# Mephisto405/WCMC

Measured on AMD Instinct MI355X. Metric: 128x128 MC patches/sec (train step), KPCN-Manifold, higher is better.
Workload: dtype bf16x321h

## Files before the change

### include/wcmc_hip.h

```cpp
#ifndef WCMC_HIP_H
#define WCMC_HIP_H

#include <stddef.h>
#include <stdint.h>

#ifdef __cplusplus
extern "C" {
#endif

#define WCMC_ABI_VERSION 2

enum wcmc_status {
  WCMC_OK = 0,
  WCMC_ERR_BAD_ARG = -1,
  WCMC_ERR_ALIGNMENT = -2,
  WCMC_ERR_WORKSPACE = -3,
  WCMC_ERR_LAUNCH = -4
};

enum wcmc_act { WCMC_ACT_LINEAR = 0, WCMC_ACT_RELU = 1, WCMC_ACT_LEAKY_RELU = 2 };

int wcmc_abi_version(void);
const char* wcmc_last_error(void);

int wcmc_to_nhwc(const float* src, int64_t ssn, int64_t ssc, int64_t ssh, int64_t ssw,
                 float* dst, int64_t dsn, int64_t dsh, int64_t dsw,
                 int N, int C, int H, int W, void* stream);
int wcmc_from_nhwc(const float* src, int64_t ssn, int64_t ssh, int64_t ssw,
                   float* dst, int64_t dsn, int64_t dsc, int64_t dsh, int64_t dsw,
                   int N, int C, int H, int W, void* stream);

size_t wcmc_conv2d_packed_elems(int rows, int kchan, int ks);
int wcmc_conv2d_pack_weight(const float* w_oihw, float* wp, int Cout, int Cin, int ks, int mode,
                            void* stream);

int wcmc_conv2d_igemm(const float* x, int64_t xsn, int64_t xsh, int64_t xsw,
                      int N, int H, int W, int Cin,
                      const float* wp, const float* bias,
                      float* y, int64_t ysn, int64_t ysh, int64_t ysw, int Cout,
                      int ks, int pad, int act, float slope,
                      const float* gate, int64_t gsn, int64_t gsh, int64_t gsw,
                      int gate_act, float gate_slope, void* stream);

size_t wcmc_conv2d_wgrad_workspace_bytes(int N, int Ho, int Wo, int Cout, int Cin, int ks);
int wcmc_conv2d_wgrad(const float* x, int64_t xsn, int64_t xsh, int64_t xsw,
                      int N, int H, int W, int Cin,
                      const float* dy, int64_t dsn, int64_t dsh, int64_t dsw, int Cout,
                      int ks, int pad, float* dw_oihw, float* db,
                      void* workspace, size_t workspace_bytes, void* stream);

int wcmc_split_from_nchw(const float* src, int64_t ssn, int64_t ssc, int64_t ssh, int64_t ssw, void* out_split, int N,
                         int C, int H, int W, void* stream);

size_t wcmc_split_elems(int N, int H, int W, int C);
int wcmc_split_bf16(const float* x, int64_t xsn, int64_t xsh, int64_t xsw, void* out_split,
                    int N, int H, int W, int C, void* stream);
int wcmc_split_gated_bf16(const float* dy, int64_t dsn, int64_t dsh, int64_t dsw, const float* post, int64_t psn,
                          int64_t psh, int64_t psw, int act, float slope, void* out_split, int N, int H, int W, int C,
                          void* stream);
int wcmc_cat_broadcast_split(const float* flat, int64_t fsn, int64_t fsh, int64_t fsw,
                             const float* prop, int64_t psn, int64_t psh, int64_t psw,
                             void* out_split, int B, int S, int H, int W, int C1, int C2, void* stream);
int wcmc_cat_upsample_split(const float* deep, int64_t dsn, int64_t dsh, int64_t dsw, const float* skip, int64_t ssn,
                            int64_t ssh, int64_t ssw, void* out_split, int N, int H, int W, int C1, int C2,
                            void* stream);

int wcmc_add_broadcast_split(const float* g, int64_t gsn, int64_t gsh, int64_t gsw,
                             const float* gm, int64_t msn, int64_t msh, int64_t msw, float scale,
                             void* out_split, int B, int S, int H, int W, int C, void* stream);
int wcmc_split_dy_colsum_bf16(const float* dy, int64_t dsn, int64_t dsh, int64_t dsw,
                              const float* post, int64_t psn, int64_t psh, int64_t psw, int act, float slope,
                              const float* gm, int64_t msn, int64_t msh, int64_t msw, int S, float scale,
                              void* out_split, float* colsum_partial, int N, int H, int W, int C, void* stream);
size_t wcmc_conv2d_packed_elems_bf16x3(int rows, int kchan, int ks, int mode);
int wcmc_conv2d_pack_weight_bf16x3(const float* w_oihw, void* wp, int Cout, int Cin, int ks, int mode,
                                   void* stream);
int wcmc_conv2d_pack_chain_bf16x3(int n_entries, const float* const* w, void* const* wp, const int* Cout,
                                  const int* Cin, const int* mode, int ks, void* stream);
int wcmc_conv2d_igemm_bf16x3(const void* x_split, int N, int H, int W, int Cin,
                             const void* wp, const float* bias,
                             float* y, int64_t ysn, int64_t ysh, int64_t ysw, void* y_split, int Cout,
                             int ks, int pad, int act, float slope,
                             const void* gate_split, int gate_act, float gate_slope,
                             float* colsum_partial, const void* gate_mask, void* mask_out, int terms, void* stream);
int wcmc_conv2d_out_f16_supported(int Cin, int Cout, int ks);
size_t wcmc_split_to_f16_elems(int N, int H, int W, int C);
int wcmc_split_to_f16(const void* x_split, int N, int H, int W, int C, void* out_f16, void* stream);
int wcmc_conv2d_out_f16(const void* x_f16, int N, int H, int W, int Cin, const void* wp_f16, const float* bias, float* y,
                        int64_t ysn, int64_t ysh, int64_t ysw, int Cout, int ks, int pad, void* stream);
int wcmc_conv1x1_pair_supported(int Cin, int Cout1, int Cout2);
int wcmc_conv1x1_pair_bf16x3(const void* x_split, int N, int H, int W, int Cin, const void* wp1, const float* bias1,
                             int Cout1, int act1, float slope1, void* y1_split, void* mask1, const void* gate_mask1,
                             int gate_act1, float gate_slope1, float* colsum1, const void* wp2, const float* bias2,
                             int Cout2, int act2, float slope2, float* y2, int64_t y2sn, int64_t y2sh, int64_t y2sw,
                             void* stream);
int wcmc_embed3_supported(int Cin, int C1, int C2, int C3);
size_t wcmc_embed3_bwd_workspace_bytes(void);
int wcmc_embed3_fwd(const void* x_split, int64_t M, int Cin, const void* wp0, const float* b0, const void* wp1,
                    const float* b1, const void* wp2, const float* b2, float* y, void* stream);
int wcmc_embed3_mean_supported(int S, int64_t HW);
int wcmc_embed3_mean_fwd(const void* x_split, int64_t M, int Cin, const void* wp0, const float* b0, const void* wp1,
                         const float* b1, const void* wp2, const float* b2, float* y, float* y_mean, int S, int64_t HW,
                         void* stream);
int wcmc_embed3_bwd(const void* x_split, int64_t M, int Cin, const void* wp0, const float* b0, const void* wp1,
                    const float* b1, const void* wt1, const void* wt2, const float* gy, int gy_pixel_stride,
                    const float* gm, int gm_pixel_stride, int S, int64_t HW, float gm_scale, float* dw0, float* db0,
                    float* dw1, float* db1, float* dw2, float* db2, void* workspace, size_t workspace_bytes, void* stream);
int wcmc_embed3_nchw_supported(int Cin, int64_t N, int64_t H, int64_t W, int64_t sn, int64_t sc, int64_t sh, int64_t sw);
int wcmc_embed3_mean_fwd_nchw(const float* x, int64_t x_sample_stride, int64_t x_channel_stride, int64_t M, int Cin,
                              const void* wp0, const float* b0, const void* wp1, const float* b1, const void* wp2,
                              const float* b2, float* y, float* y_mean, int S, int64_t HW, void* stream);
int wcmc_embed3_bwd_nchw(const float* x, int64_t x_sample_stride, int64_t x_channel_stride, int64_t M, int Cin, const void* wp0,
                         const float* b0, const void* wp1, const float* b1, const void* wt1, const void* wt2, const float* gy,
                         int gy_pixel_stride, const float* gm, int gm_pixel_stride, int S, int64_t HW, float gm_scale, float* dw0,
                         float* db0, float* dw1, float* db1, float* dw2, float* db2, void* workspace, size_t workspace_bytes,
                         void* stream);
int wcmc_final2_supported(int C1, int C2, int Chid, int outc, int64_t HW);
size_t wcmc_final2_bwd_workspace_bytes(void);
int wcmc_final2_fwd(const float* y, int y_pixel_stride, const float* prop, int prop_pixel_stride, int B, int S, int64_t HW,
                    const void* wp0, const float* b0, const void* wp1, const float* b1, int outc, float* out, void* stream);
int wcmc_final2_bwd(const float* y, int y_pixel_stride, const float* prop, int prop_pixel_stride, int B, int S, int64_t HW,
                    const void* wp0, const float* b0, const void* wp1, const float* b1, int outc, const void* wt0,
                    const void* wt1, const float* gout, float* dy, float* dprop, float* dw0, float* db0, float* dw1,
                    float* db1, void* workspace, size_t workspace_bytes, void* stream);
int wcmc_final2_fwd_save(const float* y, int y_pixel_stride, const float* prop, int prop_pixel_stride, int B, int S, int64_t HW,
                         const void* wp0, const float* b0, const void* wp1, const float* b1, int outc, float* out, void* h_hi,
                         void* stream);
int wcmc_final2_bwd_saved(const float* y, int y_pixel_stride, const float* prop, int prop_pixel_stride, int B, int S, int64_t HW,
                          const void* wp0, const float* b0, const void* wp1, const float* b1, int outc, const void* wt0,
                          const void* wt1, const float* gout, const float* out, const void* h_hi, float* dy, float* dprop,
                          float* dw0, float* db0, float* dw1, float* db1, void* workspace, size_t workspace_bytes, void* stream);
size_t wcmc_conv2d_igemm_colsum_elems(int N, int Ho, int Wo, int Cout);
int wcmc_colsum_finish(const float* partial, int N, int Ho, int Wo, int Cout, float* db, void* stream);
int wcmc_conv2d_launch_plan_bf16x3(int N, int H, int W, int Cin, int Cout, int ks, int pad, int terms, int split_out,
                                   int64_t ysn, int64_t ysh, int64_t ysw, int gate_tensor, int out_f16,
                                   char* cls, char* kernel, size_t len);
int wcmc_conv2d_wgrad_launch_plan_bf16x3(int N, int H, int W, int Cin, int Cout, int ks, int pad, int terms,
                                         char* cls, char* kernel, size_t len);
size_t wcmc_conv2d_wgrad_bf16x3_workspace_bytes(int N, int Ho, int Wo, int Cout, int Cin, int ks);
int wcmc_conv2d_wgrad_reduce_multi(int n, void* const* workspace, float* const* dw, float* const* db,
                                   const float* const* dy_colsum_partial, const int* N, const int* Ho, const int* Wo,
                                   const int* Cout, const int* Cin, const int* ks, int terms, void* stream);
int wcmc_conv2d_wgrad_bf16x3(const void* x_split, int N, int H, int W, int Cin,
                             const void* dy_split, int Cout, int ks, int pad, float* dw, float* db,
                             void* workspace, size_t workspace_bytes, int phase, const float* dy_colsum_partial,
                             int terms, void* stream);

int wcmc_act_backward(const float* dy, int64_t dsn, int64_t dsh, int64_t dsw,
                      const float* y, int64_t ysn, int64_t ysh, int64_t ysw,
                      float* dx, int64_t xsn, int64_t xsh, int64_t xsw,
                      int N, int H, int W, int C, int act, float slope, void* stream);

int wcmc_kernel_apply_fwd(const float* logits, int64_t lsn, int64_t lsh, int64_t lsw,
                          const float* data, int64_t dsn, int64_t dsc, int64_t dsh, int64_t dsw,
                          float* out, int64_t osn, int64_t osc, int64_t osh, int64_t osw,
                          float* lse, int N, int C, int h, int w, int k, void* stream);
int wcmc_kernel_apply_bwd(const float* logits, int64_t lsn, int64_t lsh, int64_t lsw,
                          const float* data, int64_t dsn, int64_t dsc, int64_t dsh, int64_t dsw,
                          const float* out, int64_t osn, int64_t osc, int64_t osh, int64_t osw,
                          const float* grad_out, int64_t gsn, int64_t gsc, int64_t gsh, int64_t gsw,
                          const float* lse,
                          float* d_logits, int64_t qsn, int64_t qsh, int64_t qsw,
                          float* d_data, int N, int C, int h, int w, int k, void* stream);

enum wcmc_splat_mode { WCMC_SPLAT_SOFTMAX = 0, WCMC_SPLAT_SHIFT = 1 };
size_t wcmc_kernel_splat_fwd_workspace_bytes(int N, int C, int h, int w, int k2);
int wcmc_kernel_splat_fwd(const float* logits, int64_t lsn, int64_t lsh, int64_t lsw,
                          const float* data, int64_t dsn, int64_t dsc, int64_t dsh, int64_t dsw,
                          float* sum_r, float* sum_w, float* lse, int mode, const float* shift,
                          int accumulate, void* workspace, size_t workspace_bytes,
                          int N, int C, int h, int w, int k2, void* stream);
int wcmc_kernel_splat_bwd(const float* logits, int64_t lsn, int64_t lsh, int64_t lsw,
                          const float* data, int64_t dsn, int64_t dsc, int64_t dsh, int64_t dsw,
                          const float* g_r, int64_t gsn, int64_t gsc, int64_t gsh, int64_t gsw,
                          const float* g_w, int64_t wsn, int64_t wsh, int64_t wsw,
                          const float* lse, int mode, const float* shift,
                          float* d_logits, int64_t qsn, int64_t qsh, int64_t qsw,
                          float* d_data, int N, int C, int h, int w, int k2, void* stream);
size_t wcmc_logit_max_workspace_bytes(int N);
int wcmc_logit_max(const float* logits, int64_t lsn, int64_t lsh, int64_t lsw, float* out,
                   void* workspace, size_t workspace_bytes, int N, int h, int w, int k2, void* stream);

int wcmc_recombine_fwd(const float* albedo, int64_t asn, int64_t asc, int64_t ash, int64_t asw,
                       const float* r_diffuse, int64_t dsn, int64_t dsc, int64_t dsh, int64_t dsw,
                       const float* r_specular, int64_t ssn, int64_t ssc, int64_t ssh, int64_t ssw,
                       float* out, int N, int C, int H, int W, void* stream);
int wcmc_recombine_bwd(const float* grad_out,
                       const float* albedo, int64_t asn, int64_t asc, int64_t ash, int64_t asw,
                       const float* r_specular, int64_t ssn, int64_t ssc, int64_t ssh, int64_t ssw,
                       float* d_diffuse, float* d_specular, int N, int C, int H, int W, void* stream);

size_t wcmc_image_loss_workspace_bytes(void);
int wcmc_image_loss_fwd(const float* x, int64_t xsn, int64_t xsc, int64_t xsh, int64_t xsw,
                        const float* ref, int64_t rsn, int64_t rsc, int64_t rsh, int64_t rsw, float eps,
                        float* l1_mean, float* relative_mse, void* workspace, size_t workspace_bytes,
                        int N, int C, int H, int W, void* stream);
int wcmc_l1_mean_bwd(const float* x, int64_t xsn, int64_t xsc, int64_t xsh, int64_t xsw,
                     const float* ref, int64_t rsn, int64_t rsc, int64_t rsh, int64_t rsw,
                     const float* grad_loss, float* dx, int N, int C, int H, int W, void* stream);

int wcmc_maxpool2_fwd(const float* x, int64_t xsn, int64_t xsh, int64_t xsw,
                      float* y, int64_t ysn, int64_t ysh, int64_t ysw,
                      int N, int H, int W, int C, void* stream);
int wcmc_maxpool2_bwd_add(const float* x, int64_t xsn, int64_t xsh, int64_t xsw, const float* dy, int64_t dsn, int64_t dsh,
                          int64_t dsw, const float* add, int64_t asn, int64_t ash, int64_t asw, float* dx, int64_t gsn,
                          int64_t gsh, int64_t gsw, int N, int H, int W, int C, void* stream);
int wcmc_maxpool2_bwd(const float* x, int64_t xsn, int64_t xsh, int64_t xsw,
                      const float* dy, int64_t dsn, int64_t dsh, int64_t dsw,
                      float* dx, int64_t gsn, int64_t gsh, int64_t gsw,
                      int N, int H, int W, int C, void* stream);
int wcmc_upsample2_fwd(const float* x, int64_t xsn, int64_t xsh, int64_t xsw,
                       float* y, int64_t ysn, int64_t ysh, int64_t ysw,
                       int N, int H, int W, int C, void* stream);
int wcmc_upsample2_bwd(const float* dy, int64_t dsn, int64_t dsh, int64_t dsw,
                       float* dx, int64_t xsn, int64_t xsh, int64_t xsw,
                       int N, int H, int W, int C, void* stream);

int wcmc_spp_reduce(const float* x, int64_t xsn, int64_t xsh, int64_t xsw,
                    float* y, int64_t ysn, int64_t ysh, int64_t ysw,
                    int B, int S, int H, int W, int C, float scale, void* stream);
int wcmc_spp_broadcast(const float* x, int64_t xsn, int64_t xsh, int64_t xsw,
                       float* y, int64_t ysn, int64_t ysh, int64_t ysw,
                       int B, int S, int H, int W, int C, float scale, int accumulate,
                       void* stream);

int wcmc_sample_cat_fwd(const float* feat, int64_t fsb, int64_t fss, int64_t fsc, int64_t fsh, int64_t fsw,
                        const float* p, int64_t psb, int64_t pss, int64_t psc, int64_t psh, int64_t psw, float* out,
                        int B, int S, int C, int Cp, int H, int W, void* stream);

int wcmc_pbuffer_cat_fwd(const float* base, int64_t bsn, int64_t bsc, int64_t bsh, int64_t bsw,
                         const float* p, int64_t psb, int64_t pss, int64_t psc, int64_t psh,
                         int64_t psw,
                         float* out, int64_t osn, int64_t osh, int64_t osw,
                         int B, int S, int Cb, int Cp, int H, int W, void* stream);
int wcmc_pbuffer_cat_bwd(const float* g, int64_t gsn, int64_t gsh, int64_t gsw,
                         float* dp, int64_t psb, int64_t pss, int64_t psc, int64_t psh,
                         int64_t psw,
                         int B, int S, int Cb, int Cp, int H, int W, void* stream);

size_t wcmc_feature_mse_workspace_bytes(int B, int S, int C, int h, int w);
int wcmc_feature_mse_fwd(const float* p, int64_t psb, int64_t pss, int64_t psc, int64_t psh,
                         int64_t psw,
                         const float* ref, int64_t rsb, int64_t rsc, int64_t rsh, int64_t rsw,
                         const int64_t* idx_patch, const int64_t* idx_batch,
                         float* loss, void* workspace, size_t workspace_bytes,
                         int B, int S, int C, int h, int w, void* stream);
int wcmc_feature_mse_bwd(const float* p, int64_t psb, int64_t pss, int64_t psc, int64_t psh,
                         int64_t psw,
                         const int64_t* idx_patch, const int64_t* idx_batch,
                         const float* grad_scale, float* dp,
                         void* workspace, size_t workspace_bytes,
                         int B, int S, int C, int h, int w, void* stream);

int wcmc_grs_fwd(const float* p, int64_t psb, int64_t pss, int64_t psc, int64_t psh, int64_t psw,
                 const float* ref, int64_t rsb, int64_t rsc, int64_t rsh, int64_t rsw,
                 const int64_t* idx_patch, const int64_t* idx_batch, float alpha,
                 float* loss, void* workspace, size_t workspace_bytes,
                 int B, int S, int C, int h, int w, void* stream);
int wcmc_grs_bwd(const float* p, int64_t psb, int64_t pss, int64_t psc, int64_t psh, int64_t psw,
                 const int64_t* idx_patch, const int64_t* idx_batch,
                 const float* grad_scale, float* dp,
                 void* workspace, size_t workspace_bytes,
                 int B, int S, int C, int h, int w, void* stream);

int wcmc_random_permutation(int64_t* out, int64_t n, uint64_t seed, void* stream);
uint64_t wcmc_permutation_key(uint64_t seed, uint64_t counter, int slot);
int wcmc_random_permutation_dev(int64_t* out, int64_t n, const uint64_t* state, int slot, void* stream);
int wcmc_step_counter_advance(uint64_t* state, void* stream);

int wcmc_image_loss2_fwd(int kind, const float* x, int64_t xsn, int64_t xsc, int64_t xsh, int64_t xsw, const float* ref,
                         int64_t rsn, int64_t rsc, int64_t rsh, int64_t rsw, float eps, float* loss, void* workspace,
                         size_t workspace_bytes, int N, int C, int H, int W, void* stream);
int wcmc_image_loss2_bwd(int kind, const float* x, int64_t xsn, int64_t xsc, int64_t xsh, int64_t xsw, const float* ref,
                         int64_t rsn, int64_t rsc, int64_t rsh, int64_t rsw, float eps, const float* grad_loss, float* dx,
                         int N, int C, int H, int W, void* stream);
size_t wcmc_grad_norm_clip_workspace_bytes(int n_tensors, const int64_t* numel);
int wcmc_grad_norm_clip(int n_tensors, float* const* grads, const int64_t* numel, float max_norm, float* norm_and_coef,
                        void* workspace, size_t workspace_bytes, void* stream);

int wcmc_weight_norm_fwd(int n_layers, const float* const* v, const float* const* g, float* const* w,
                         float* const* norm, const int* rows, const int* row_len, void* stream);
int wcmc_weight_norm_bwd(int n_layers, const float* const* dw, const float* const* v, const float* const* g,
                         const float* const* norm, float* const* dv, float* const* dg, const int* rows,
                         const int* row_len, void* stream);

int wcmc_clip_adam(float* param, float* grad, float* exp_avg, float* exp_avg_sq, int64_t n,
                   float clip, double lr, double beta1, double beta2, double eps, int step,
                   float grad_scale, const float* guard, void* stream);
void wcmc_clip_adam_hyper(double lr, double beta1, double beta2, double eps, int step, float* out7);
int wcmc_clip_adam_dev(float* param, float* grad, float* exp_avg, float* exp_avg_sq, int64_t n, float clip,
                       float grad_scale, const float* hyper7, const float* guard, void* stream);
int wcmc_step_guard(const float* const* losses, int n, float* ok, float* sums, float* flags, void* stream);
int wcmc_step_guard_local(const float* const* losses, int n, const float* ok, float* flags, float* flag_slot, void* stream);
int wcmc_step_guard_global(const float* const* losses, int n, const float* flag_slot, float* ok, float* sums, float* flags, void* stream);

int wcmc_preprocess_llpm(const float* raw, int64_t nsamples , int C, int max_depth, float* out,
                         void* stream);
size_t wcmc_preprocess_kpcn_workspace_bytes(int h, int w);
int wcmc_preprocess_kpcn(const float* raw, int h, int w, int s, int C, int max_depth, float* out,
                         void* workspace, size_t workspace_bytes, void* stream);
int wcmc_gradients(const float* buf, int h, int w, int c, float* out, void* stream);
int wcmc_preprocess_kpcn_begin(void* workspace, size_t workspace_bytes, int h, int w, void* stream);
int wcmc_preprocess_kpcn_rows(const float* raw_band, int h, int w, int row0, int rows, int s, int C, int max_depth, float* out,
                              void* workspace, size_t workspace_bytes, void* stream);
int wcmc_preprocess_kpcn_end(float* out, void* workspace, size_t workspace_bytes, int h, int w, int s, void* stream);

int wcmc_assemble_kpcn_patches(const float* kpcn, const float* llpm, const float* gt, const int* origins, int B, int H,
                               int W, int S, int P, float* diffuse_in, float* specular_in, float* diffuse_buffer,
                               float* specular_buffer, float* albedo, float* paths, float* target_diffuse,
                               float* target_specular, float* target_total, void* stream);

int wcmc_reflect_index(int i, int n);
size_t wcmc_importance_map_workspace_bytes(int H, int W, int C);
int wcmc_importance_map(const float* img, int H, int W, int C, float* out, void* workspace, size_t workspace_bytes,
                        void* stream);
size_t wcmc_sampling_prob_workspace_bytes(int H, int W, int patch);
int wcmc_sampling_prob(const float* raw, const float* gt, int H, int W, int S, int C, int max_depth, int patch, float* out,
                       void* workspace, size_t workspace_bytes, void* stream);
int wcmc_sanitize(float* x, int64_t n, void* stream);

int wcmc_preprocess_sbmc(const float* raw, int64_t nsamples , int C, int max_depth, float* out_s, float* out_p,
                         int tiled, void* stream);
int wcmc_assemble_sample_patches(const float* sbmc_s, const float* sbmc_p, const float* llpm, const float* gt,
                                 const int* origins, int B, int H, int W, int S, int P, int use_g_buf, int use_sbmc_buf,
                                 float* radiance, float* features, float* paths, float* target_image, void* stream);

size_t wcmc_preprocess_kpcn_prefix_workspace_bytes(int h, int w, int n_counts);
int wcmc_preprocess_kpcn_prefix(const float* raw, int h, int w, int S, int C, int max_depth, int s_lo, int s_hi, float* out,
                                void* workspace, size_t workspace_bytes, void* stream);
int wcmc_assemble_kpcn_patches_prefix(const float* kpcn, const float* llpm, const float* gt, const int* origins, int B, int H,
                                      int W, int S_total, int s, int P, float* diffuse_in, float* specular_in,
                                      float* diffuse_buffer, float* specular_buffer, float* albedo, float* paths,
                                      float* target_diffuse, float* target_specular, float* target_total, void* stream);
int wcmc_assemble_sample_patches_prefix(const float* sbmc_s, const float* sbmc_p, const float* llpm, const float* gt,
                                        const int* origins, int B, int H, int W, int S_total, int s, int P, int use_g_buf,
                                        int use_sbmc_buf, float* radiance, float* features, float* paths, float* target_image,
                                        void* stream);

int wcmc_assemble_kpcn_patches_aug(const float* kpcn, const float* llpm, const float* gt, const int* origins, const int* transforms,
                                   int B, int H, int W, int S_total, int s, int P, float* diffuse_in, float* specular_in,
                                   float* diffuse_buffer, float* specular_buffer, float* albedo, float* paths,
                                   float* target_diffuse, float* target_specular, float* target_total, void* stream);
int wcmc_assemble_sample_patches_aug(const float* sbmc_s, const float* sbmc_p, const float* llpm, const float* gt,
                                     const int* origins, const int* transforms, int B, int H, int W, int S_total, int s, int P,
                                     int use_g_buf, int use_sbmc_buf, float* radiance, float* features, float* paths,
                                     float* target_image, void* stream);

size_t wcmc_image_eval_workspace_bytes(int H, int W);
int wcmc_image_eval(const float* out, int64_t osh, int64_t osw, int64_t osc, const float* ipt, int64_t ish, int64_t isw,
                    int64_t isc, const float* tgt, int64_t tsh, int64_t tsw, int64_t tsc, const float* has_hit, int64_t hsh,
                    int64_t hsw, int64_t hsc, int H, int W, double eps, double* result, void* workspace,
                    size_t workspace_bytes, void* stream);
int wcmc_stitch_tiles(const float* rad, int64_t rsb, int64_t rsc, int64_t rsh, int64_t rsw, int ho, int wo,
                      const float* pbuf_a, const float* pbuf_b, int S, int C, int P, const int* coords, int B, int H, int W,
                      float* out_rad, float* out_pbuf_a, float* out_pbuf_b, void* stream);

int wcmc_assemble_kpcn_tiles(const float* kpcn, const float* llpm, const int* origins, int B, int H, int W, int S, int P, int pad,
                             float* diffuse_in, float* specular_in, float* diffuse_buffer, float* specular_buffer, float* albedo,
                             float* paths, void* stream);
int wcmc_finish_frame(const float* out_rad, const float* kpcn, const float* llpm, int H, int W, int S, float* out, float* ipt,
                      float* has_hit, unsigned char* preview_out, unsigned char* preview_ipt, void* stream);

int wcmc_assemble_sample_tiles(const float* sbmc_s, const float* sbmc_p, const float* llpm, const int* origins, int B, int H, int W,
                               int S, int P, int pad, int use_g_buf, int use_sbmc_buf, float* radiance, float* features,
                               float* paths, void* stream);
int wcmc_finish_sample_frame(const float* out_rad, const float* sbmc_s, const float* llpm, int H, int W, int S, float* out,
                             float* ipt, float* has_hit, unsigned char* preview_out, unsigned char* preview_ipt, void* stream);

size_t wcmc_pbuffer_filter_workspace_bytes(int S, int C, int H, int W);
int wcmc_pbuffer_filter(const float* image, int64_t ish, int64_t isw, int64_t isc,
                        const float* p_buffer, int64_t pss, int64_t psc, int64_t psh, int64_t psw,
                        const void* mask, int mask_bytes, float* out, float* wsum, void* workspace, size_t workspace_bytes,
                        int H, int W, int S, int C, int Cr, int R, int f, float bandwidth, float eps, int passes, void* stream);

#ifdef __cplusplus
}
#endif
#endif
```

### wcmc_amd/_lib.py

```python
import ctypes
import os

_HERE = os.path.dirname(os.path.abspath(__file__))
LIB_PATH = os.path.join(_HERE, "libwcmc_hip.so")
if os.environ.get("WCMC_DEBUG_LIB") == "1":
    LIB_PATH = os.path.join(_HERE, "libwcmc_hip_debug.so")
if os.environ.get("WCMC_LIB_AB"):
    LIB_PATH = os.path.join(_HERE, os.path.basename(os.environ["WCMC_LIB_AB"]))

_c = ctypes
P, I, L, F, D, Z = _c.c_void_p, _c.c_int, _c.c_int64, _c.c_float, _c.c_double, _c.c_size_t

SIGNATURES = {
    "wcmc_abi_version": (I, []),
    "wcmc_last_error": (_c.c_char_p, []),
    "wcmc_to_nhwc": (I, [P, L, L, L, L, P, L, L, L, I, I, I, I, P]),
    "wcmc_from_nhwc": (I, [P, L, L, L, P, L, L, L, L, I, I, I, I, P]),
    "wcmc_conv2d_packed_elems": (Z, [I, I, I]),
    "wcmc_conv2d_pack_weight": (I, [P, P, I, I, I, I, P]),
    "wcmc_conv2d_igemm": (I, [P, L, L, L, I, I, I, I, P, P, P, L, L, L, I, I, I, I, F,
                              P, L, L, L, I, F, P]),
    "wcmc_conv2d_wgrad_workspace_bytes": (Z, [I, I, I, I, I, I]),
    "wcmc_conv2d_wgrad": (I, [P, L, L, L, I, I, I, I, P, L, L, L, I, I, I, P, P, P, Z, P]),
    "wcmc_split_elems": (Z, [I, I, I, I]),
    "wcmc_split_bf16": (I, [P, L, L, L, P, I, I, I, I, P]),
    "wcmc_split_from_nchw": (I, [P, L, L, L, L, P, I, I, I, I, P]),
    "wcmc_split_gated_bf16": (I, [P, L, L, L, P, L, L, L, I, F, P, I, I, I, I, P]),
    "wcmc_cat_broadcast_split": (I, [P, L, L, L, P, L, L, L, P, I, I, I, I, I, I, P]),
    "wcmc_cat_upsample_split": (I, [P, L, L, L, P, L, L, L, P, I, I, I, I, I, P]),
    "wcmc_add_broadcast_split": (I, [P, L, L, L, P, L, L, L, F, P, I, I, I, I, I, P]),
    "wcmc_split_dy_colsum_bf16": (I, [P, L, L, L, P, L, L, L, I, F, P, L, L, L, I, F, P, P, I, I, I, I, P]),
    "wcmc_conv2d_packed_elems_bf16x3": (Z, [I, I, I, I]),
    "wcmc_conv2d_pack_weight_bf16x3": (I, [P, P, I, I, I, I, P]),
    "wcmc_conv2d_pack_chain_bf16x3": (I, [I, P, P, P, P, P, I, P]),
    "wcmc_conv2d_igemm_bf16x3": (I, [P, I, I, I, I, P, P, P, L, L, L, P, I, I, I, I, F, P, I, F, P, P, P, I, P]),
    "wcmc_conv2d_out_f16_supported": (I, [I, I, I]),
    "wcmc_split_to_f16_elems": (Z, [I, I, I, I]),
    "wcmc_split_to_f16": (I, [P, I, I, I, I, P, P]),
    "wcmc_conv2d_out_f16": (I, [P, I, I, I, I, P, P, P, L, L, L, I, I, I, P]),
    "wcmc_conv1x1_pair_supported": (I, [I, I, I]),
    "wcmc_conv1x1_pair_bf16x3": (I, [P, I, I, I, I, P, P, I, I, F, P, P, P, I, F, P, P, P, I, I, F, P, L, L, L, P]),
    "wcmc_conv2d_igemm_colsum_elems": (Z, [I, I, I, I]),
    "wcmc_colsum_finish": (I, [P, I, I, I, I, P, P]),
    "wcmc_conv2d_launch_plan_bf16x3": (I, [I, I, I, I, I, I, I, I, I, L, L, L, I, I, _c.c_char_p, _c.c_char_p, Z]),
    "wcmc_conv2d_wgrad_launch_plan_bf16x3": (I, [I, I, I, I, I, I, I, I, _c.c_char_p, _c.c_char_p, Z]),
    "wcmc_conv2d_wgrad_bf16x3_workspace_bytes": (Z, [I, I, I, I, I, I]),
    "wcmc_conv2d_wgrad_reduce_multi": (I, [I, P, P, P, P, P, P, P, P, P, P, I, P]),
    "wcmc_conv2d_wgrad_bf16x3": (I, [P, I, I, I, I, P, I, I, I, P, P, P, Z, I, P, I, P]),
    "wcmc_act_backward": (I, [P, L, L, L, P, L, L, L, P, L, L, L, I, I, I, I, I, F, P]),
    "wcmc_kernel_apply_fwd": (I, [P, L, L, L, P, L, L, L, L, P, L, L, L, L, P, I, I, I, I, I, P]),
    "wcmc_kernel_apply_bwd": (I, [P, L, L, L, P, L, L, L, L, P, L, L, L, L, P, L, L, L, L, P,
                                  P, L, L, L, P, I, I, I, I, I, P]),
    "wcmc_kernel_splat_fwd_workspace_bytes": (Z, [I, I, I, I, I]),
    "wcmc_kernel_splat_fwd": (I, [P, L, L, L, P, L, L, L, L, P, P, P, I, P, I, P, Z, I, I, I, I, I, P]),
    "wcmc_kernel_splat_bwd": (I, [P, L, L, L, P, L, L, L, L, P, L, L, L, L, P, L, L, L, P, I, P,
                                  P, L, L, L, P, I, I, I, I, I, P]),
    "wcmc_logit_max_workspace_bytes": (Z, [I]),
    "wcmc_logit_max": (I, [P, L, L, L, P, P, Z, I, I, I, I, P]),
    "wcmc_recombine_fwd": (I, [P, L, L, L, L, P, L, L, L, L, P, L, L, L, L, P, I, I, I, I, P]),
    "wcmc_image_loss_workspace_bytes": (Z, []),
    "wcmc_image_loss_fwd": (I, [P, L, L, L, L, P, L, L, L, L, F, P, P, P, Z, I, I, I, I, P]),
    "wcmc_l1_mean_bwd": (I, [P, L, L, L, L, P, L, L, L, L, P, P, I, I, I, I, P]),
    "wcmc_recombine_bwd": (I, [P, P, L, L, L, L, P, L, L, L, L, P, P, I, I, I, I, P]),
    "wcmc_maxpool2_fwd": (I, [P, L, L, L, P, L, L, L, I, I, I, I, P]),
    "wcmc_maxpool2_bwd": (I, [P, L, L, L, P, L, L, L, P, L, L, L, I, I, I, I, P]),
    "wcmc_maxpool2_bwd_add": (I, [P, L, L, L, P, L, L, L, P, L, L, L, P, L, L, L, I, I, I, I, P]),
    "wcmc_upsample2_fwd": (I, [P, L, L, L, P, L, L, L, I, I, I, I, P]),
    "wcmc_upsample2_bwd": (I, [P, L, L, L, P, L, L, L, I, I, I, I, P]),
    "wcmc_sample_cat_fwd": (I, [P, L, L, L, L, L, P, L, L, L, L, L, P, I, I, I, I, I, I, P]),
    "wcmc_spp_reduce": (I, [P, L, L, L, P, L, L, L, I, I, I, I, I, F, P]),
    "wcmc_spp_broadcast": (I, [P, L, L, L, P, L, L, L, I, I, I, I, I, F, I, P]),
    "wcmc_pbuffer_cat_fwd": (I, [P, L, L, L, L, P, L, L, L, L, L, P, L, L, L, I, I, I, I, I, I, P]),
    "wcmc_pbuffer_cat_bwd": (I, [P, L, L, L, P, L, L, L, L, L, I, I, I, I, I, I, P]),
    "wcmc_feature_mse_workspace_bytes": (Z, [I, I, I, I, I]),
    "wcmc_feature_mse_fwd": (I, [P, L, L, L, L, L, P, L, L, L, L, P, P, P, P, Z, I, I, I, I, I, P]),
    "wcmc_feature_mse_bwd": (I, [P, L, L, L, L, L, P, P, P, P, P, Z, I, I, I, I, I, P]),
    "wcmc_grs_fwd": (I, [P, L, L, L, L, L, P, L, L, L, L, P, P, F, P, P, Z, I, I, I, I, I, P]),
    "wcmc_grs_bwd": (I, [P, L, L, L, L, L, P, P, P, P, P, Z, I, I, I, I, I, P]),
    "wcmc_random_permutation": (I, [P, L, ctypes.c_uint64, P]),
    "wcmc_permutation_key": (ctypes.c_uint64, [ctypes.c_uint64, ctypes.c_uint64, I]),
    "wcmc_random_permutation_dev": (I, [P, L, P, I, P]),
    "wcmc_step_counter_advance": (I, [P, P]),
    "wcmc_final2_supported": (I, [I, I, I, I, L]),
    "wcmc_final2_bwd_workspace_bytes": (Z, []),
    "wcmc_final2_fwd": (I, [P, I, P, I, I, I, L, P, P, P, P, I, P, P]),
    "wcmc_final2_bwd": (I, [P, I, P, I, I, I, L, P, P, P, P, I, P, P, P, P, P, P, P, P, P, P, Z, P]),
    "wcmc_final2_fwd_save": (I, [P, I, P, I, I, I, L, P, P, P, P, I, P, P, P]),
    "wcmc_final2_bwd_saved": (I, [P, I, P, I, I, I, L, P, P, P, P, I, P, P, P, P, P, P, P, P, P, P, P, P, Z, P]),
    "wcmc_embed3_supported": (I, [I, I, I, I]),
    "wcmc_embed3_bwd_workspace_bytes": (Z, []),
    "wcmc_embed3_fwd": (I, [P, L, I, P, P, P, P, P, P, P, P]),
    "wcmc_embed3_mean_supported": (I, [I, L]),
    "wcmc_embed3_mean_fwd": (I, [P, L, I, P, P, P, P, P, P, P, P, I, L, P]),
    "wcmc_embed3_bwd": (I, [P, L, I, P, P, P, P, P, P, P, I, P, I, I, L, F, P, P, P, P, P, P, P, Z, P]),
    "wcmc_embed3_nchw_supported": (I, [I, L, L, L, L, L, L, L]),
    "wcmc_embed3_mean_fwd_nchw": (I, [P, L, L, L, I, P, P, P, P, P, P, P, P, I, L, P]),
    "wcmc_embed3_bwd_nchw": (I, [P, L, L, L, I, P, P, P, P, P, P, P, I, P, I, I, L, F, P, P, P, P, P, P, P, Z, P]),
    "wcmc_image_loss2_fwd": (I, [I, P, L, L, L, L, P, L, L, L, L, F, P, P, Z, I, I, I, I, P]),
    "wcmc_image_loss2_bwd": (I, [I, P, L, L, L, L, P, L, L, L, L, F, P, P, I, I, I, I, P]),
    "wcmc_grad_norm_clip_workspace_bytes": (Z, [I, P]),
    "wcmc_grad_norm_clip": (I, [I, P, P, F, P, P, Z, P]),
    "wcmc_weight_norm_fwd": (I, [I, P, P, P, P, P, P, P]),
    "wcmc_weight_norm_bwd": (I, [I, P, P, P, P, P, P, P, P, P]),
    "wcmc_clip_adam": (I, [P, P, P, P, L, F, D, D, D, D, I, F, P, P]),
    "wcmc_clip_adam_hyper": (None, [D, D, D, D, I, P]),
    "wcmc_clip_adam_dev": (I, [P, P, P, P, L, F, F, P, P, P]),
    "wcmc_step_guard": (I, [P, I, P, P, P, P]),
    "wcmc_step_guard_local": (I, [P, I, P, P, P, P]),
    "wcmc_step_guard_global": (I, [P, I, P, P, P, P, P]),
    "wcmc_preprocess_llpm": (I, [P, L, I, I, P, P]),
    "wcmc_preprocess_kpcn_workspace_bytes": (Z, [I, I]),
    "wcmc_preprocess_kpcn": (I, [P, I, I, I, I, I, P, P, Z, P]),
    "wcmc_preprocess_kpcn_begin": (I, [P, Z, I, I, P]),
    "wcmc_preprocess_kpcn_rows": (I, [P, I, I, I, I, I, I, I, P, P, Z, P]),
    "wcmc_preprocess_kpcn_end": (I, [P, P, Z, I, I, I, P]),
    "wcmc_gradients": (I, [P, I, I, I, P, P]),
    "wcmc_assemble_kpcn_patches": (I, [P, P, P, P, I, I, I, I, I, P, P, P, P, P, P, P, P, P, P]),
    "wcmc_reflect_index": (I, [I, I]),
    "wcmc_importance_map_workspace_bytes": (Z, [I, I, I]),
    "wcmc_importance_map": (I, [P, I, I, I, P, P, Z, P]),
    "wcmc_sampling_prob_workspace_bytes": (Z, [I, I, I]),
    "wcmc_sampling_prob": (I, [P, P, I, I, I, I, I, I, P, P, Z, P]),
    "wcmc_sanitize": (I, [P, L, P]),
    "wcmc_preprocess_sbmc": (I, [P, L, I, I, P, P, I, P]),
    "wcmc_assemble_sample_patches": (I, [P, P, P, P, P, I, I, I, I, I, I, I, P, P, P, P, P]),
    "wcmc_preprocess_kpcn_prefix_workspace_bytes": (Z, [I, I, I]),
    "wcmc_preprocess_kpcn_prefix": (I, [P, I, I, I, I, I, I, I, P, P, Z, P]),
    "wcmc_assemble_kpcn_patches_prefix": (I, [P, P, P, P, I, I, I, I, I, I, P, P, P, P, P, P, P, P, P, P]),
    "wcmc_assemble_sample_patches_prefix": (I, [P, P, P, P, P, I, I, I, I, I, I, I, I, P, P, P, P, P]),
    "wcmc_assemble_kpcn_patches_aug": (I, [P, P, P, P, P, I, I, I, I, I, I, P, P, P, P, P, P, P, P, P, P]),
    "wcmc_assemble_sample_patches_aug": (I, [P, P, P, P, P, P, I, I, I, I, I, I, I, I, P, P, P, P, P]),
    "wcmc_image_eval_workspace_bytes": (Z, [I, I]),
    "wcmc_image_eval": (I, [P, L, L, L, P, L, L, L, P, L, L, L, P, L, L, L, I, I, D, P, P, Z, P]),
    "wcmc_stitch_tiles": (I, [P, L, L, L, L, I, I, P, P, I, I, I, P, I, I, I, P, P, P, P]),
    "wcmc_assemble_kpcn_tiles": (I, [P, P, P, I, I, I, I, I, I, P, P, P, P, P, P, P]),
    "wcmc_finish_frame": (I, [P, P, P, I, I, I, P, P, P, P, P, P]),
    "wcmc_assemble_sample_tiles": (I, [P, P, P, P, I, I, I, I, I, I, I, I, P, P, P, P]),
    "wcmc_finish_sample_frame": (I, [P, P, P, I, I, I, P, P, P, P, P, P]),
    "wcmc_pbuffer_filter_workspace_bytes": (Z, [I, I, I, I]),
    "wcmc_pbuffer_filter": (I, [P, L, L, L, P, L, L, L, L, P, I, P, P, P, Z, I, I, I, I, I, I, I, F, F, I, P]),
}

_lib = None


def lib():
    global _lib
    if _lib is None:
        if not os.path.isfile(LIB_PATH):
            raise RuntimeError(
                "wcmc_amd: %s is missing -- the HIP hot path has not been built "
                "(make -C wcmc_amd/csrc). There is no CPU fallback." % LIB_PATH)
        h = ctypes.CDLL(LIB_PATH)
        for name, (res, args) in SIGNATURES.items():
            fn = getattr(h, name)
            fn.restype, fn.argtypes = res, args
        if h.wcmc_abi_version() != 2:
            raise RuntimeError("wcmc_amd: ABI version mismatch in %s" % LIB_PATH)
        _lib = h
    return _lib


def check(rc, what=""):
    if rc != 0:
        msg = lib().wcmc_last_error().decode("utf-8", "replace")
        raise RuntimeError("wcmc_hip %s failed (%d): %s" % (what, rc, msg))
```

### wcmc_amd/csrc/bf16x3_common.h

```cpp
#pragma once
#include "common.h"

namespace wcmc {

typedef __bf16 bf16x8 __attribute__((ext_vector_type(8)));
typedef unsigned short u16;
typedef short s16x4 __attribute__((ext_vector_type(4)));

__device__ __forceinline__ u16 f2bf(float x) { return __builtin_bit_cast(u16, (__bf16)x); }
__device__ __forceinline__ float bf2f(u16 h) { return __builtin_bit_cast(float, (unsigned)h << 16); }
__device__ __forceinline__ void split1(float x, u16& hi, u16& lo) {
  hi = f2bf(x);
  lo = f2bf(x - bf2f(hi));
}

typedef _Float16 xf16x8 __attribute__((ext_vector_type(8)));

constexpr int XBM = 128;
constexpr int XKC = 32;
constexpr int XROW = 32;
constexpr unsigned XOOB = 0x80000000u;

typedef unsigned int u32x4 __attribute__((ext_vector_type(4)));
typedef unsigned u32x2 __attribute__((ext_vector_type(2)));

typedef short xs16x2 __attribute__((ext_vector_type(2)));
__device__ __forceinline__ unsigned positive_pair(unsigned w) {
  const xs16x2 z = {0, 0};
  const xs16x2 c = __builtin_elementwise_max(__builtin_bit_cast(xs16x2, w), z);
  return ((__builtin_bit_cast(unsigned, c) + 0x7fff7fffu) >> 15) & 0x00010001u;
}
__device__ __forceinline__ unsigned char positive_mask8(const u32x4 v) {
  const unsigned x = positive_pair(v[0]) | (positive_pair(v[1]) << 2) | (positive_pair(v[2]) << 4) | (positive_pair(v[3]) << 6);
  return (unsigned char)((x | (x >> 15)) & 0xffu);
}

typedef __bf16 xbf16x2 __attribute__((ext_vector_type(2)));
typedef float xf32x2 __attribute__((ext_vector_type(2)));
__device__ __forceinline__ void x_split2(float a, float b, unsigned& hi2, unsigned& lo2) {
  const xf32x2 v = {a, b};
  hi2 = __builtin_bit_cast(unsigned, __builtin_convertvector(v, xbf16x2));
  const xf32x2 back = {__builtin_bit_cast(float, hi2 << 16), __builtin_bit_cast(float, hi2 & 0xffff0000u)};
  lo2 = __builtin_bit_cast(unsigned, __builtin_convertvector(v - back, xbf16x2));
}
struct XAct { float ns; bool zero; };
__device__ __forceinline__ XAct x_act(int act, float slope) {
  return XAct{act == WCMC_ACT_LEAKY_RELU ? slope : 1.f, act == WCMC_ACT_RELU};
}
__device__ __forceinline__ float x_act_apply(float v, XAct a) { return v > 0.f ? v : (a.zero ? 0.f : v * a.ns); }

__device__ __forceinline__ void x_epi_quad(const f32x4 a4, const float (&b)[4], bool ok, XAct ak, int gkind, u32x2 g2, int co,
                                           float gate_off, float (&v)[4]) {
#pragma unroll
  for (int e = 0; e < 4; ++e) {
    const float t = a4[e] + b[e];
    const float neg = ak.zero ? 0.f : t * ak.ns;
    const float r = t > 0.f ? t : neg;
    v[e] = ok ? r : 0.f;
  }
  if (gkind == 1) {
    const unsigned g[4] = {g2.x << 16, g2.x & 0xffff0000u, g2.y << 16, g2.y & 0xffff0000u};
#pragma unroll
    for (int e = 0; e < 4; ++e) v[e] = __builtin_bit_cast(float, g[e]) > 0.f ? v[e] : v[e] * gate_off;
  } else if (gkind == 2) {
    const unsigned bits = g2.x >> (co & 7);
#pragma unroll
    for (int e = 0; e < 4; ++e) v[e] = ((bits >> e) & 1u) ? v[e] : v[e] * gate_off;
  }
}

struct XIgemmParams {
  const u16* x; int N, H, W, Cin, Cpi;
  const u16* wp; const float* bias;
  float* yf; int64_t ysn, ysh, ysw;
  u16* ys; int Cpo;
  int Ho, Wo, Cout;
  const u16* gate; int gate_act; float gate_slope;
  const unsigned char* gate_mask;
  unsigned char* mask_out;
  int ks, pad, act; float slope;
  int Kp, Kt, Np;
  int64_t M;
  unsigned x_bytes, wp_bytes;
  float* colsum;
  int G;
  int CS, nslabs, SPS, PXS, tilesX, tilesY;
  int CSl, SPSl;
  int rows16;
  int stripX, stripY;
  int ap;
  int wplanes;
  int f16;
  unsigned y_bytes, m_bytes;
  const u16* wp2; const float* bias2; float* y2; int64_t y2sn, y2sh, y2sw;
  int Cout2, act2, Kt2; float slope2; unsigned wp2_bytes, y2_bytes;
};

struct XWgradParams {
  const u16* x; int N, H, W, Cin, Cpi;
  const u16* dy; int Ho, Wo, Cout, Cpo;
  int ks, pad;
  float* slabs; int S; int64_t M, pix_per_split;
  int Np, Cq, coBlocks, ciBlocks;
  unsigned x_bytes, dy_bytes;
  int xps, yps;
};
struct XWRowsParams {
  const u16* x; int N, H, W, Cpi;
  const u16* dy; int Ho, Wo, Cpo;
  int pad;
  float* slabs; int S, rps, R;
  float* dbg;
  int prio;
  int Np, Cq, coBlocks, ciBlocks;
  unsigned x_bytes, dy_bytes;
  int xps, yps;
};
constexpr int xwr_stride(int ch) { return ((ch / 16) | 1) * 16; }
static size_t xwr_lds_bytes_rt(int ks, int tm, int nw, int pl = 2) {
  const int nvec = pl * 64 * (xwr_stride(tm * 16) / 8) + pl * (64 + ks - 1) * (xwr_stride(nw * 16) / 8);
  const int ni = (nvec + nw * 64 - 1) / (nw * 64);
  const size_t stage = (size_t)2 * ni * nw * 64 * 16, red = (size_t)tm * 16 * (nw * 16 + 4) * sizeof(float);
  return stage > red ? stage : red;
}

__device__ __forceinline__ void pw_barrier() {
  asm volatile("s_waitcnt lgkmcnt(0)" ::: "memory");
  __builtin_amdgcn_s_barrier();
  asm volatile("" ::: "memory");
}

int x_env_on(const char* name);

struct XIgemmPlan { int nt, padded, dbuf; };
struct XHaloPlan { int nt, th, nb, ap, tilesY; size_t lds; };
struct XHalo64Plan { int nt, nb, pt, pxst, ap, wp, f16;
                     int tilesX, tilesY, rows16, stripX, stripY; size_t lds; };
struct XHalo3Plan { int ap, spt; };
struct XPwPlan { int ntw, u; };
struct XWRowsPlan { int ks, tm, nw, pl, rows8, xe; };
XIgemmPlan x_plan_igemm(int nt, const XIgemmParams& p);
int launch_xigemm(const XIgemmPlan& g, const XIgemmParams& p, hipStream_t stream);
bool x_halo_is64(const XIgemmParams& p);
int x_plan_halo(int nt, const XIgemmParams& p, XHaloPlan* h);
int launch_xhalo(const XHaloPlan& h, const XIgemmParams& p, hipStream_t stream);
XHalo64Plan x_plan_halo64(int nt, const XIgemmParams& p);
int launch_xhalo64(const XHalo64Plan& h, const XIgemmParams& p, hipStream_t stream);
bool x_halo3_ok(const XIgemmParams& p);
XHalo3Plan x_plan_halo3(const XIgemmParams& p);
int launch_xhalo3(const XHalo3Plan& h, const XIgemmParams& p, hipStream_t stream);
bool x_plan_pw(const XIgemmParams& p, XPwPlan* w);
int launch_xpw(XIgemmParams& p, const XPwPlan& w, hipStream_t stream);
int launch_xpw_pair(int kind, const XIgemmParams& p, hipStream_t stream);
int launch_xwgrad(int tm, int planes, const XWgradParams& p, hipStream_t stream);
XWRowsPlan x_plan_wgrad_rows(int ks, int tm, int nw, int planes);
int launch_xwgrad_rows(const XWRowsPlan& r, const XWRowsParams& p, hipStream_t stream);

}
```

### wcmc_amd/csrc/bf16x3_halo64.hip

```cpp
#include "bf16x3_common.h"

namespace wcmc {

template <int NT, int NB, int PT = 4, int DBG = 0, int PXST = 0, int AP = 2, int WP = 2, int F16 = 0>
__global__ __launch_bounds__(256, 2) void conv_halo64_bf16x3_kernel(XIgemmParams p0) {
  static_assert(WP == 2 || AP == 1, "one weight plane only together with one pixel plane");
  static_assert(!F16 || (AP == 1 && WP == 1), "fp16 operands: one plane each");
  XIgemmParams p = p0;
  if (PXST) { p.PXS = PXST; p.ks = 5; }
  constexpr int BN = NT * 16, TH = 4 * PT, TW = 16, NTHR = 256, NWV = 4;
  constexpr int NG = (PT + 1) / 2;
  extern __shared__ __attribute__((aligned(16))) u16 smem16[];
  constexpr int B_LO = BN * XROW + 32, B_ELEMS = 2 * BN * XROW + 64;
  const int HWd = TW + p.ks - 1, HHt = TH + p.ks - 1, HP = HWd * HHt;
  char* const halo = reinterpret_cast<char*>(smem16);
  u16* const bsm = smem16 + ((HP * p.PXS + 127) & ~127) / 2;

  const int tid = threadIdx.x, lane = tid & 63, wave = __builtin_amdgcn_readfirstlane(tid >> 6);
  unsigned long long st_rt[7] = {0, 0, 0, 0, 0, 0, 0};
  auto rstamp = [&](int i) {
    if (DBG & 64) {
      unsigned long long t;
      __builtin_amdgcn_sched_barrier(0);
      asm volatile("s_memrealtime %0\n\ts_waitcnt lgkmcnt(0)" : "=s"(t)::"memory");
      __builtin_amdgcn_sched_barrier(0);
      st_rt[i] = t;
    }
  };
  rstamp(0);
  int tile;
  {
    const int nb = gridDim.x, q = nb >> 3, r = nb & 7, xcd = blockIdx.x & 7, k = blockIdx.x >> 3;
    tile = (xcd < r ? xcd * (q + 1) : r * (q + 1) + (xcd - r) * q) + k;
  }
  const int nmain = p.tilesX * p.tilesY;
  const int tpi = nmain + (PT == 4 ? p.stripX * p.stripY : 0);
  const int img = tile / tpi, trem0 = tile - img * tpi;
  const bool tr = PT == 4 && trem0 >= nmain;
  const int trem = tr ? trem0 - nmain : trem0;
  const int tcols = tr ? p.stripX : p.tilesX;
  const int trow = trem / tcols;
  const int ptc = tr ? 3 : (PT == 4 && trow >= p.rows16) ? 3 : PT;
  const int oy0 = tr ? trow * 16 : PT == 4 ? (trow < p.rows16 ? trow * 16 : p.rows16 * 16 + (trow - p.rows16) * 12) : trow * TH;
  const int ox0 = tr ? p.tilesX * TW + (trem - trow * tcols) * 12 : (trem - trow * tcols) * TW;
  const int n0 = blockIdx.y * BN;

  const __amdgpu_buffer_rsrc_t xr = __builtin_amdgcn_make_buffer_rsrc((void*)p.x, 0, (int)p.x_bytes, 0x00020000);
  const __amdgpu_buffer_rsrc_t wr = __builtin_amdgcn_make_buffer_rsrc((void*)p.wp, 0, (int)p.wp_bytes, 0x00020000);
  const int pixb = (F16 ? 2 : 4) * p.Cpi;

  const int VP = p.PXS / 16;
  const int hvecs = HWd * (4 * ptc + p.ks - 1) * VP;
  const float invVP = 1.0f / (float)VP, invHW = 1.0f / (float)HWd;
  constexpr int NHV = PXST ? (((TH + 4) * (TW + 4) * (PXST / 16) + 63) / 64 + NWV - 1) / NWV : 0;
  const int CSlh = p.CSl < 8 ? 8 : p.CSl;
  unsigned hoff[NHV ? NHV : 1], hoffl[NHV ? NHV : 1];
  if (PXST) {
#pragma unroll
    for (int kq = 0; kq < NHV; ++kq) {
      const int v = (wave + NWV * kq) * 64 + lane;
      hoff[kq] = XOOB; hoffl[kq] = XOOB;
      if (v < hvecs) {
        const int px = (int)(((float)v + 0.5f) * invVP), part = v - px * VP;
        const int hy = (int)(((float)px + 0.5f) * invHW), hx = px - hy * HWd;
        const int iy = oy0 - p.pad + (tr ? hx : hy), ix = ox0 - p.pad + (tr ? hy : hx);
        if ((unsigned)iy < (unsigned)p.H && (unsigned)ix < (unsigned)p.W) {
          const unsigned pbase = (unsigned)(((img * p.H + iy) * p.W + ix) * pixb);
          if (AP == 1) {
            if (part < p.CS / 8 && (p.nslabs - 2) * p.CS + part * 8 < p.Cpi) hoff[kq] = pbase + (unsigned)(part * 16);
            if (part < CSlh / 8 && (p.nslabs - 1) * p.CS + part * 8 < p.Cpi) hoffl[kq] = pbase + (unsigned)(part * 16);
          } else {
          {
            const int V = p.CS / 4, plane = part >= (V >> 1), vec = part - plane * (V >> 1);
            if (part < V && (p.nslabs - 2) * p.CS + vec * 8 < p.Cpi) hoff[kq] = pbase + (unsigned)(plane * 2 * p.Cpi + vec * 16);
          }
          {
            const int V = CSlh / 4, plane = part >= (V >> 1), vec = part - plane * (V >> 1);
            if (part < V && (p.nslabs - 1) * p.CS + vec * 8 < p.Cpi) hoffl[kq] = pbase + (unsigned)(plane * 2 * p.Cpi + vec * 16);
          }
          }
        }
      }
    }
  }
  auto dma_halo = [&](int slab) {
    if (PXST) {
      const unsigned so = (unsigned)(slab * p.CS * 2);
      const bool lastslab = slab == p.nslabs - 1;
#pragma unroll
      for (int kq = 0; kq < NHV; ++kq) {
        const int ii = wave + NWV * kq;
        if (ii * 64 < hvecs) {
          const unsigned off = (lastslab ? hoffl[kq] : hoff[kq]) + so;
          if (ii * 64 + lane < hvecs)
            __builtin_amdgcn_raw_ptr_buffer_load_lds(xr, (__attribute__((address_space(3))) void*)(halo + ii * 1024), 16, off, 0, 0, 0);
        }
      }
      return;
    }
    const int V = (slab == p.nslabs - 1 ? CSlh : p.CS) / (AP == 1 ? 8 : 4);
    for (int ii = wave; ii * 64 < hvecs; ii += NWV) {
      const int v = ii * 64 + lane;
      if (v < hvecs) {
        const int px = (int)(((float)v + 0.5f) * invVP), part = v - px * VP;
        const int hy = (int)(((float)px + 0.5f) * invHW), hx = px - hy * HWd;
        const int iy = oy0 - p.pad + (tr ? hx : hy), ix = ox0 - p.pad + (tr ? hy : hx);
        const int plane = AP == 1 ? 0 : part >= (V >> 1), vec = part - plane * (V >> 1);
        const int ch = slab * p.CS + vec * 8;
        unsigned off = XOOB;
        if (part < V && (unsigned)iy < (unsigned)p.H && (unsigned)ix < (unsigned)p.W && ch < p.Cpi)
          off = (unsigned)(((img * p.H + iy) * p.W + ix) * pixb + plane * 2 * p.Cpi + ch * 2);
        __builtin_amdgcn_raw_ptr_buffer_load_lds(xr, (__attribute__((address_space(3))) void*)(halo + ii * 1024), 16, off, 0, 0, 0);
      }
    }
  };

  const int nstages = p.Kt / XKC;
  constexpr int NGMAX = (NT + NWV - 1) / NWV;
  const int ngroups = wave < NT ? (NT - wave + NWV - 1) / NWV : 0;
  unsigned dbase[NGMAX], dbase2[NGMAX];
#pragma unroll
  for (int q = 0; q < NGMAX; ++q) {
    const int drow = 16 * (wave + q * NWV) + (lane >> 2);
    const int dvq = (lane & 3) ^ ((drow >> 1) & 3);
    dbase[q] = (q < ngroups && n0 + drow < p.Np) ? (unsigned)(((n0 + drow) * 2 * p.Kt + dvq * 8) * 2) : XOOB;
    dbase2[q] = dbase[q] >= XOOB ? XOOB : dbase[q] + (unsigned)(p.Kt * 2);
  }
  auto dma_b = [&](int g, int buf) {
    const unsigned sg = g < nstages ? (unsigned)(g * XKC * 2) : 0x40000000u;
#pragma unroll
    for (int q = 0; q < NGMAX; ++q) {
      if (q < ngroups) {
        const unsigned off = dbase[q] + sg;
        const unsigned off2 = dbase2[q] + sg;
        u16* d = bsm + buf * B_ELEMS + 16 * (wave + q * NWV) * XROW;
        __builtin_amdgcn_raw_ptr_buffer_load_lds(wr, (__attribute__((address_space(3))) void*)d, 16, off, 0, 0, 0);
        if (WP == 2) __builtin_amdgcn_raw_ptr_buffer_load_lds(wr, (__attribute__((address_space(3))) void*)(d + B_LO), 16, off2, 0, 0, 0);
      }
    }
  };

  f32x4 acc[NT][PT];
#pragma unroll
  for (int j = 0; j < NT; ++j)
#pragma unroll
    for (int i = 0; i < PT; ++i) acc[j][i] = f32x4{0.f, 0.f, 0.f, 0.f};

  const int frow = lane & 15, kg = lane >> 4;
  const int fslot = (kg ^ ((frow >> 1) & 3)) * 8;
  const int abase0 = (wave * HWd + frow) * p.PXS, dA = NWV * HWd * p.PXS;
  int cs_cur, sps_cur, lo_off, tps, coff, tdx, tdy;
  bool cs4 = false;
  const int sMx = tr ? HWd * p.PXS : p.PXS, sMy = tr ? p.PXS : HWd * p.PXS;
  int toff = 0, dstep = 0;
  const int wrapc = sMy - p.ks * sMx;
  auto slab_begin = [&](int slab) {
    cs_cur = slab == p.nslabs - 1 ? p.CSl : p.CS;
    sps_cur = slab == p.nslabs - 1 ? p.SPSl : (p.SPS & 0xff);
    cs4 = cs_cur == 4;
    lo_off = (cs4 ? 8 : cs_cur) * 2;
    tps = 32 / cs_cur;
    coff = cs4 ? 0 : ((kg * 8) & (cs_cur - 1)) * 2;
    tdy = 0; tdx = cs_cur == 32 ? 0 : cs_cur == 16 ? (kg >> 1) : cs4 ? 2 * kg : kg;
    if (tdx >= p.ks) { tdx -= p.ks; ++tdy; }
    toff = tdy * sMy + tdx * sMx + coff;
    dstep = tps * sMx;
  };
  bf16x8 ah[PT], al[PT], wh[NT], wl[NT];
  auto a_off = [&]() { return tdy < p.ks ? toff : coff; };
  auto a_off2 = [&]() {
    const bool wrap = tdx + 1 >= p.ks;
    const int y = tdy + (wrap ? 1 : 0);
    return y < p.ks ? toff + sMx + (wrap ? wrapc : 0) : 0;
  };
  auto a_advance = [&]() {
    tdx += tps; toff += dstep;
    if (tdx >= p.ks) { tdx -= p.ks; ++tdy; toff += wrapc; }
    if (cs4 && tdx >= p.ks) { tdx -= p.ks; ++tdy; toff += wrapc; }
  };
  auto read_a1 = [&](int i, int aoff, int aoff2) {
    const char* pa = halo + abase0 + aoff;
    if (cs4) {
      const char* pb = halo + abase0 + aoff2;
      const u32x2 a0 = *reinterpret_cast<const u32x2*>(pa + i * dA), a1 = *reinterpret_cast<const u32x2*>(pb + i * dA);
      ah[i] = __builtin_bit_cast(bf16x8, u32x4{a0.x, a0.y, a1.x, a1.y});
      if (AP == 2) {
        const u32x2 l0 = *reinterpret_cast<const u32x2*>(pa + lo_off + i * dA), l1 = *reinterpret_cast<const u32x2*>(pb + lo_off + i * dA);
        al[i] = __builtin_bit_cast(bf16x8, u32x4{l0.x, l0.y, l1.x, l1.y});
      }
      return;
    }
    ah[i] = *reinterpret_cast<const bf16x8*>(pa + i * dA);
    if (AP == 2) al[i] = *reinterpret_cast<const bf16x8*>(pa + lo_off + i * dA);
  };
  const u16* const bfrag = bsm + frow * XROW + fslot;
  auto read_b = [&](int buf, int j) {
    wh[j] = *reinterpret_cast<const bf16x8*>(bfrag + buf * B_ELEMS + j * 16 * XROW);
    if (WP == 2) wl[j] = *reinterpret_cast<const bf16x8*>(bfrag + buf * B_ELEMS + B_LO + j * 16 * XROW);
  };

#pragma unroll
  for (int b = 0; b < NB; ++b) dma_b(b, b);
  dma_halo(0);
  slab_begin(0);
  asm volatile("s_waitcnt vmcnt(0)" ::: "memory");
  __syncthreads();
  {
    const int aoff = a_off(), aoff2 = cs4 ? a_off2() : 0;
#pragma unroll
    for (int i = 0; i < PT; ++i)
      if (i < ptc) read_a1(i, aoff, aoff2);
    a_advance();
  }
#pragma unroll
  for (int j = 0; j < NT; ++j) read_b(0, j);
  int s_in = 0, slab = 0, bcur = 0;
  const int wgpar = (blockIdx.x >> 8) & 1;
  const bool prio_on = p.SPS & 0x100;
  rstamp(1);
  for (int g = 0; g < nstages; ++g) {
    const int b1 = bcur + 1 == NB ? 0 : bcur + 1;
    if (NGMAX == 1 || ngroups < 2) asm volatile("s_waitcnt vmcnt(%0)" ::"n"(WP * (NB - 2)) : "memory");
    else asm volatile("s_waitcnt vmcnt(%0)" ::"n"(2 * WP * (NB - 2)) : "memory");
    pw_barrier();
    if (prio_on) { if ((g ^ wgpar) & 1) __builtin_amdgcn_s_setprio(1); else __builtin_amdgcn_s_setprio(0); }
    if (!(DBG & 2)) dma_b(g + NB, bcur);
    bcur = b1;
    const bool last_of_slab = (s_in + 1 == sps_cur);
    if (last_of_slab && slab + 1 < p.nslabs && !(DBG & 4)) dma_halo(slab + 1);
    const int aoff = a_off(), aoff2 = cs4 ? a_off2() : 0;
    __builtin_amdgcn_sched_barrier(0);
#pragma unroll
    for (int j = 0; j < NT; ++j) {
#pragma unroll
      for (int i = 0; i < PT; ++i) {
        if (i >= ptc) continue;
        if (!(DBG & 1)) {
          if (WP == 2) acc[j][i] = __builtin_amdgcn_mfma_f32_16x16x32_bf16(wl[j], ah[i], acc[j][i], 0, 0, 0);
          if (AP == 2) acc[j][i] = __builtin_amdgcn_mfma_f32_16x16x32_bf16(wh[j], al[i], acc[j][i], 0, 0, 0);
          if (F16) acc[j][i] = __builtin_amdgcn_mfma_f32_16x16x32_f16(__builtin_bit_cast(xf16x8, wh[j]), __builtin_bit_cast(xf16x8, ah[i]), acc[j][i], 0, 0, 0);
          else acc[j][i] = __builtin_amdgcn_mfma_f32_16x16x32_bf16(wh[j], ah[i], acc[j][i], 0, 0, 0);
        }
        if (j == NT - 1 && !last_of_slab && !(DBG & 8)) read_a1(i, aoff, aoff2);
      }
      if (!(DBG & 8)) read_b(b1, j);
      __builtin_amdgcn_sched_barrier(0);
    }
    if (!last_of_slab) {
      a_advance();
      ++s_in;
    } else {
      s_in = 0;
      ++slab;
      slab_begin(slab < p.nslabs ? slab : p.nslabs - 1);
      asm volatile("s_waitcnt vmcnt(0)" ::: "memory");
      __syncthreads();
      const int a2 = a_off(), a22 = cs4 ? a_off2() : 0;
#pragma unroll
      for (int i = 0; i < PT; ++i)
        if (i < ptc) read_a1(i, a2, a22);
      a_advance();
    }
  }
  __builtin_amdgcn_s_setprio(0);
  rstamp(2);
  if ((DBG & 32) && !(DBG & 64)) {
    float keep = 0.f;
#pragma unroll
    for (int j = 0; j < NT; ++j)
#pragma unroll
      for (int i = 0; i < PT; ++i) keep += acc[j][i][0] + acc[j][i][1] + acc[j][i][2] + acc[j][i][3];
    if (keep == 12345.678f && p.ys) p.ys[0] = 1;
    return;
  }
  const int fq = kg * 4;
  float bv[NT][4];
  {
    const __amdgpu_buffer_rsrc_t brs =
        __builtin_amdgcn_make_buffer_rsrc((void*)(p.bias ? (const void*)p.bias : (const void*)p.wp), 0, p.bias ? p.Cout * 4 : 0, 0x00020000);
#pragma unroll
    for (int j = 0; j < NT; ++j)
#pragma unroll
      for (int e = 0; e < 4; ++e)
        bv[j][e] = __builtin_bit_cast(float, __builtin_amdgcn_raw_buffer_load_b32(brs, (n0 + j * 16 + fq + e) * 4, 0, 0));
  }
  const bool use_gate = p.ys && p.gate, use_mask = p.ys && !p.gate && p.gate_mask && p.gate_act != WCMC_ACT_LINEAR;
  u32x2 gv[PT][NT];
  bool okp[PT]; int64_t mp[PT];
#pragma unroll
  for (int i = 0; i < PT; ++i) {
    const int oy = tr ? oy0 + frow : oy0 + wave + NWV * i, ox = tr ? ox0 + wave + NWV * i : ox0 + frow;
    okp[i] = i < ptc && oy < p.Ho && ox < p.Wo;
    mp[i] = ((int64_t)img * p.Ho + oy) * p.Wo + ox;
  }
  if (use_gate) {
    const int64_t gbytes = (int64_t)p.N * p.Ho * p.Wo * 4 * p.Cpo;
    const __amdgpu_buffer_rsrc_t grs = __builtin_amdgcn_make_buffer_rsrc((void*)p.gate, 0, (int)(gbytes < 0x7fffffff ? gbytes : 0x7fffffff), 0x00020000);
#pragma unroll
    for (int i = 0; i < PT; ++i)
#pragma unroll
      for (int j = 0; j < NT; ++j) {
        const int co = n0 + j * 16 + fq;
        gv[i][j] = __builtin_amdgcn_raw_buffer_load_b64(grs, (okp[i] && co < p.Cpo) ? (unsigned)((mp[i] * 2 * p.Cpo + co) * 2) : XOOB, 0, 0);
      }
  } else if (use_mask) {
    const int64_t mbytes = (int64_t)p.N * p.Ho * p.Wo * (p.Cpo >> 3);
    const __amdgpu_buffer_rsrc_t mrs = __builtin_amdgcn_make_buffer_rsrc((void*)p.gate_mask, 0, (int)mbytes, 0x00020000);
#pragma unroll
    for (int i = 0; i < PT; ++i)
#pragma unroll
      for (int j = 0; j < NT; ++j) {
        const int co = n0 + j * 16 + fq;
        gv[i][j].x = (unsigned)__builtin_amdgcn_raw_buffer_load_b8(mrs, (okp[i] && co < p.Cpo) ? (unsigned)(mp[i] * (p.Cpo >> 3) + (co >> 3)) : XOOB, 0, 0);
      }
  }
  const XAct ak = x_act(p.act, p.slope);
  const float gate_off = p.gate_act == WCMC_ACT_RELU ? 0.f : p.gate_act == WCMC_ACT_LEAKY_RELU ? p.gate_slope : 1.f;
  const int gkind = use_gate ? 1 : use_mask ? 2 : 0;
  asm volatile("s_waitcnt vmcnt(0)" ::: "memory");
  __syncthreads();
  rstamp(3);

  auto pix_of = [&](int h, int pr, int& oy, int& ox) {
    const int i = 2 * h + ((pr >> 4) & 1);
    if (tr) { oy = oy0 + (pr & 15); ox = ox0 + (pr >> 5) + NWV * i; }
    else { oy = oy0 + (pr >> 5) + NWV * i; ox = ox0 + (pr & 15); }
    return i < ptc && oy < p.Ho && ox < p.Wo;
  };
  if (p.ys) {
    constexpr int OLD = 2 * BN + 8;
    u16* so = smem16;
    constexpr int CW = BN <= 16 ? 16 : BN <= 32 ? 32 : BN <= 64 ? 64 : 128, RG = NTHR / CW;
    const int cc = tid % CW, rg = tid / CW;
    float csum = 0.f;
#pragma unroll
    for (int h = 0; h < NG; ++h) {
      if (h) __syncthreads();
#pragma unroll
      for (int il = 0; il < 2; ++il) {
        const int pr = wave * 32 + il * 16 + frow;
#pragma unroll
        for (int j = 0; j < NT; ++j) {
          const int co = n0 + j * 16 + fq;
          unsigned h01 = 0, l01 = 0, h23 = 0, l23 = 0;
          if (2 * h + il < PT) {
            constexpr int dummy = 0; (void)dummy;
            float v[4];
            const int ti = 2 * h + il < PT ? 2 * h + il : 0;
            x_epi_quad(acc[j][ti], bv[j], okp[ti], ak, gkind, gv[ti][j], co, gate_off, v);
            x_split2(v[0], v[1], h01, l01);
            x_split2(v[2], v[3], h23, l23);
          }
          *reinterpret_cast<uint2*>(so + pr * OLD + j * 16 + fq) = make_uint2(h01, h23);
          *reinterpret_cast<uint2*>(so + pr * OLD + BN + j * 16 + fq) = make_uint2(l01, l23);
        }
      }
      __syncthreads();
      if (h == 0) rstamp(4);
      constexpr int VPP = BN / 8;
      for (int v = tid; v < 128 * 2 * VPP; v += NTHR) {
        const int pr = v / (2 * VPP), q = v - pr * (2 * VPP);
        const int plane = q >= VPP, vec = q - plane * VPP;
        const int co = n0 + vec * 8;
        int oy, ox;
        if (pix_of(h, pr, oy, ox) && co < p.Cpo) {
          const int64_t m = ((int64_t)img * p.Ho + oy) * p.Wo + ox;
          const u32x4 hv = *reinterpret_cast<const u32x4*>(so + pr * OLD + plane * BN + vec * 8);
          *reinterpret_cast<u32x4*>(p.ys + m * 2 * p.Cpo + plane * p.Cpo + co) = hv;
          if (p.mask_out && plane == 0) p.mask_out[m * (p.Cpo >> 3) + (co >> 3)] = positive_mask8(hv);
        }
      }
      if (h == 0) rstamp(5);
      if (p.colsum && cc < BN)
        for (int r = rg; r < 128; r += RG) csum += bf2f(so[r * OLD + cc]) + bf2f(so[r * OLD + BN + cc]);
    }
    if (p.colsum && !(DBG & 64)) {
      __syncthreads();
      float* red = reinterpret_cast<float*>(so);
      if (rg > 0 && cc < BN) red[(rg - 1) * BN + cc] = csum;
      __syncthreads();
      if (rg == 0 && cc < BN && n0 + cc < p.Np) {
        for (int q = 0; q < RG - 1; ++q) csum += red[q * BN + cc];
        p.colsum[(int64_t)tile * p.Np + n0 + cc] = csum;
        if (tile == 0 && n0 + cc == 0) reinterpret_cast<int*>(p.colsum)[(int64_t)p.G * p.Np] = (int)gridDim.x;
      }
    }
  } else {
    constexpr int OLD = BN + 4;
    float* so = reinterpret_cast<float*>(smem16);
#pragma unroll
    for (int h = 0; h < NG; ++h) {
      if (h) __syncthreads();
#pragma unroll
      for (int il = 0; il < 2; ++il) {
        const int pr = wave * 32 + il * 16 + frow;
#pragma unroll
        for (int j = 0; j < NT; ++j) {
          const int co = n0 + j * 16 + fq;
          const f32x4 a4 = acc[j][2 * h + il < PT ? 2 * h + il : 0];
          float v[4];
          x_epi_quad(a4, bv[j], true, ak, 0, u32x2{0u, 0u}, co, 1.f, v);
          *reinterpret_cast<float4*>(so + pr * OLD + j * 16 + fq) = make_float4(v[0], v[1], v[2], v[3]);
        }
      }
      __syncthreads();
      constexpr int VPP = BN / 4;
      for (int v = tid; v < 128 * VPP; v += NTHR) {
        const int pr = v / VPP, vec = v - pr * VPP;
        const int co = n0 + vec * 4;
        int oy, ox;
        if (pix_of(h, pr, oy, ox) && co < p.Cpo)
          *reinterpret_cast<float4*>(p.yf + (int64_t)img * p.ysn + (int64_t)oy * p.ysh + (int64_t)ox * p.ysw + co) =
              *reinterpret_cast<const float4*>(so + pr * OLD + vec * 4);
      }
    }
  }
  if (DBG & 64) {
    asm volatile("s_waitcnt vmcnt(0)" ::: "memory");
    rstamp(6);
    if (lane == 0) {
      unsigned long long* o = reinterpret_cast<unsigned long long*>(p.colsum) + ((int64_t)tile * NWV + wave) * 14;
      for (int i = 0; i < 7; ++i) o[6 + i] = st_rt[i];
      unsigned hw, xcc;
      asm volatile("s_getreg_b32 %0, hwreg(HW_REG_HW_ID)" : "=s"(hw));
      asm volatile("s_getreg_b32 %0, hwreg(HW_REG_XCC_ID)" : "=s"(xcc));
      o[13] = hw | ((unsigned long long)xcc << 32);
    }
  }
}

static size_t xh64_halo_bytes(int th, const XIgemmParams& p) { return (size_t)(((th + p.ks - 1) * (16 + p.ks - 1) * p.PXS + 127) & ~127); }
static size_t xh64_bstage_bytes(int nt) { return (size_t)(2 * nt * 16 * XROW + 64) * sizeof(u16); }

XHalo64Plan x_plan_halo64(int nt, const XIgemmParams& p) {
  XHalo64Plan h;
  h.nt = nt;
  const int gy = (p.Np / 16 + nt - 1) / nt;
  auto rounds = [&](int th) { return ((int64_t)p.N * p.tilesX * ((p.Ho + th - 1) / th) * gy + 511) / 512 * th; };
  bool pt3 = p.PXS == 160 || (x_env_on("WCMC_HALO64_PT3") && rounds(12) < rounds(16));
  h.rows16 = 1 << 20; h.stripX = h.stripY = 0; h.tilesX = p.tilesX;
  const char* mixe = ab_env("WCMC_HALO64_MIX");
  const bool mix12 = !(mixe && mixe[0] == '1');
  const char* nomix = ab_env("WCMC_HALO64_NOMIX");
  if (p.PXS != 160 && p.Ho % 16 != 0 && (p.Ho % 12 != 0 || mix12) && x_env_on("WCMC_HALO64_MIX") && !(nomix && atoi(nomix) == p.Ho)) {
    for (int b = 1; 12 * b < p.Ho; ++b)
      if ((p.Ho - 12 * b) % 16 == 0) { h.rows16 = (p.Ho - 12 * b) / 16; pt3 = false; break; }
  }
  const bool mixed = h.rows16 != (1 << 20);
  const int th = pt3 ? 12 : 16;
  h.tilesY = mixed ? h.rows16 + (p.Ho - 16 * h.rows16) / 12 : (p.Ho + th - 1) / th;
  const size_t halo = xh64_halo_bytes(th, p), bstage = xh64_bstage_bytes(nt);
  const size_t out = p.ys ? (size_t)128 * (2 * nt * 16 + 8) * sizeof(u16) : (size_t)128 * (nt * 16 + 4) * sizeof(float);
  const char* nbe = ab_env("WCMC_HALO_NB");
  h.nb = (p.ap == 1 || (!(nbe && nbe[0] == '2') && halo + 3 * bstage <= 80 * 1024)) ? 3 : 2;
  h.pt = pt3 ? 3 : 4;
  if (!pt3 && p.ks == 5 && p.Wo % 16 != 0 && p.Wo % 4 == 0 && x_env_on("WCMC_HALO64_STRIP")) {
    for (int b = 1; b <= 3; ++b)
      if (12 * b < p.Wo && (p.Wo - 12 * b) % 16 == 0) { h.stripX = b; h.tilesX = (p.Wo - 12 * b) / 16; h.stripY = (p.Ho + 15) / 16; break; }
  }
  const size_t main_ = halo + h.nb * bstage;
  h.lds = main_ > out ? main_ : out;
  const bool hi = h.nb == 3 && p.ap == 1;
  h.wp = (hi && nt == 7 && p.wplanes == 1) ? 1 : 2;
  h.f16 = (h.wp == 1 && p.f16) ? 1 : 0;
  h.ap = (hi && (nt == 7 || nt == 1)) ? 1 : 2;
  h.pxst = h.ap == 1 ? 80 : (p.ks == 5 && p.PXS == 80 && h.nb == 3) ? 80 : (p.ks == 5 && p.PXS == 160 && h.nb == 2 && pt3) ? 160 : 0;
  return h;
}

template <int NT, int NB, int PT, int PXST, int AP = 2, int WP = 2, int F16 = 0>
static int launch_xhalo64c(const XHalo64Plan& h, const XIgemmParams& p, hipStream_t stream) {
  WCMC_REQUIRE(h.nt == NT && h.nb == NB && h.pt == PT && h.pxst == PXST && h.ap == AP && h.wp == WP && h.f16 == F16, WCMC_ERR_LAUNCH,
               "conv2d_igemm_bf16x3(halo, 64 pixels per wave): no instance for the plan");
  static LdsAttr attr;
  if (set_max_lds(reinterpret_cast<const void*>(&conv_halo64_bf16x3_kernel<NT, NB, PT, 0, PXST, AP, WP, F16>), h.lds, attr) != hipSuccess) return WCMC_ERR_LAUNCH;
  const dim3 grid((unsigned)(p.N * (p.tilesX * p.tilesY + (PT == 4 ? p.stripX * p.stripY : 0))), (unsigned)((p.Np / 16 + NT - 1) / NT));
  hipLaunchKernelGGL((conv_halo64_bf16x3_kernel<NT, NB, PT, 0, PXST, AP, WP, F16>), grid, dim3(256), h.lds, stream, p);
  return check_launch("conv2d_igemm_bf16x3(halo, 64 pixels per wave)");
}
template <int NT, int NB, int PT>
static int launch_xhalo64b(const XHalo64Plan& h, const XIgemmParams& p, hipStream_t stream) {
  if constexpr (NT == 7 && NB == 3) {
    if (h.f16) return launch_xhalo64c<NT, NB, PT, 80, 1, 1, 1>(h, p, stream);
    if (h.wp == 1) return launch_xhalo64c<NT, NB, PT, 80, 1, 1>(h, p, stream);
  }
  if constexpr ((NT == 7 || NT == 1) && NB == 3) {
    if (h.ap == 1) return launch_xhalo64c<NT, NB, PT, 80, 1>(h, p, stream);
  }
  if (h.pxst == 80) return launch_xhalo64c<NT, NB, PT, NB == 3 ? 80 : 0>(h, p, stream);
  if (h.pxst == 160) return launch_xhalo64c<NT, NB, PT, (NB == 2 && PT == 3) ? 160 : 0>(h, p, stream);
  return launch_xhalo64c<NT, NB, PT, 0>(h, p, stream);
}
template <int NT>
static int launch_xhalo64(const XHalo64Plan& h, const XIgemmParams& p0, hipStream_t stream) {
  XIgemmParams p = p0;
  p.SPS |= 0x100;
  p.rows16 = h.rows16; p.tilesY = h.tilesY; p.stripX = p.stripY = 0;
#ifdef WCMC_DEBUG_BUILD
  if (NT == 7 && h.pt == 4 && p.PXS == 80 && p.ks == 5) {
    const char* e = ab_env("WCMC_DEBUG_ABLATE");
    const int ab = e ? atoi(e) : 0;
    if (ab) {
      auto kfn = ab == 1 ? &conv_halo64_bf16x3_kernel<7, 3, 4, 1, 80> : ab == 2 ? &conv_halo64_bf16x3_kernel<7, 3, 4, 2, 80>
                 : ab == 4 ? &conv_halo64_bf16x3_kernel<7, 3, 4, 4, 80> : ab == 8 ? &conv_halo64_bf16x3_kernel<7, 3, 4, 8, 80>
                 : ab == 10 ? &conv_halo64_bf16x3_kernel<7, 3, 4, 10, 80> : ab == 14 ? &conv_halo64_bf16x3_kernel<7, 3, 4, 14, 80>
                 : ab == 32 ? &conv_halo64_bf16x3_kernel<7, 3, 4, 32, 80> : ab == 46 ? &conv_halo64_bf16x3_kernel<7, 3, 4, 46, 80>
                 : &conv_halo64_bf16x3_kernel<7, 3, 4, 64, 80>;
      (void)hipFuncSetAttribute(reinterpret_cast<const void*>(kfn), hipFuncAttributeMaxDynamicSharedMemorySize, 80 * 1024);
      const dim3 grid((unsigned)(p.N * p.tilesX * p.tilesY), (unsigned)((p.Np / 16 + NT - 1) / NT));
      hipLaunchKernelGGL(kfn, grid, dim3(256), xh64_halo_bytes(16, p) + 3 * xh64_bstage_bytes(NT), stream, p);
      return check_launch("conv2d_igemm_bf16x3(halo64, debug)");
    }
  }
#endif
  p.tilesX = h.tilesX; p.stripX = h.stripX; p.stripY = h.stripY;
  if (h.pt == 3) return h.nb == 3 ? launch_xhalo64b<NT, 3, 3>(h, p, stream) : launch_xhalo64b<NT, 2, 3>(h, p, stream);
  return h.nb == 3 ? launch_xhalo64b<NT, 3, 4>(h, p, stream) : launch_xhalo64b<NT, 2, 4>(h, p, stream);
}
int launch_xhalo64(const XHalo64Plan& h, const XIgemmParams& p, hipStream_t stream) {
  switch (h.nt) {
    case 7: return launch_xhalo64<7>(h, p, stream);
    case 4: return launch_xhalo64<4>(h, p, stream);
    case 2: return launch_xhalo64<2>(h, p, stream);
    default: return launch_xhalo64<1>(h, p, stream);
  }
}

}
```

### wcmc_amd/csrc/conv_bf16x3.hip

```cpp
#include <stdlib.h>

#include "bf16x3_common.h"
#include "conv_common.h"

namespace wcmc {

__global__ void split_kernel(const float* __restrict__ x, int64_t xsn, int64_t xsh, int64_t xsw,
                             u16* __restrict__ out, int H, int W, int C, int Cp, int64_t total,
                             const float* __restrict__ post = nullptr, int64_t psn = 0, int64_t psh = 0, int64_t psw = 0,
                             int act = 0, float slope = 0.f) {
  const int V = Cp / 8;
  for (int64_t idx = (int64_t)blockIdx.x * blockDim.x + threadIdx.x; idx < total;
       idx += (int64_t)gridDim.x * blockDim.x) {
    const NhwvIndex ix_ = decode_nhwv(idx, total, H, W, V);
    const int v = ix_.v, xx = ix_.x, y = ix_.y, n = ix_.n;
    const float* src = x + n * xsn + y * xsh + xx * xsw + v * 8;
    float f[8];
    const int c0 = v * 8;
    if (c0 + 8 <= C) {
      const float4 a = *reinterpret_cast<const float4*>(src), b = *reinterpret_cast<const float4*>(src + 4);
      f[0] = a.x; f[1] = a.y; f[2] = a.z; f[3] = a.w; f[4] = b.x; f[5] = b.y; f[6] = b.z; f[7] = b.w;
    } else {
#pragma unroll
      for (int e = 0; e < 8; ++e) f[e] = (c0 + e < C) ? src[e] : 0.f;
    }
    if (post) {
      const float* ps = post + n * psn + y * psh + xx * psw + c0;
#pragma unroll
      for (int e = 0; e < 8; ++e)
        if (c0 + e < C) f[e] *= act_gate(ps[e], act, slope);
    }
    u16 hi[8], lo[8];
#pragma unroll
    for (int e = 0; e < 8; ++e) split1(f[e], hi[e], lo[e]);
    u16* o = out + (((int64_t)n * H + y) * W + xx) * 2 * Cp + c0;
    *reinterpret_cast<uint4*>(o) = *reinterpret_cast<const uint4*>(hi);
    *reinterpret_cast<uint4*>(o + Cp) = *reinterpret_cast<const uint4*>(lo);
  }
}

__device__ __forceinline__ u16 f2h_sat(float v) {
  v = v > 65504.f ? 65504.f : (v < -65504.f ? -65504.f : v);
  return __builtin_bit_cast(u16, (_Float16)v);
}
__global__ __launch_bounds__(256) void split_to_f16_kernel(const u16* __restrict__ xs, u16* __restrict__ out, int Cp, int64_t total) {
  const int V = Cp / 8;
  for (int64_t idx = (int64_t)blockIdx.x * blockDim.x + threadIdx.x; idx < total; idx += (int64_t)gridDim.x * blockDim.x) {
    const int v = (int)(idx % V); const int64_t px = idx / V;
    const uint4 h = *reinterpret_cast<const uint4*>(xs + px * 2 * Cp + v * 8), l = *reinterpret_cast<const uint4*>(xs + px * 2 * Cp + Cp + v * 8);
    const unsigned hw[4] = {h.x, h.y, h.z, h.w}, lw[4] = {l.x, l.y, l.z, l.w};
    u16 o[8];
#pragma unroll
    for (int e = 0; e < 4; ++e) {
      const float a = __builtin_bit_cast(float, hw[e] << 16) + __builtin_bit_cast(float, lw[e] << 16);
      const float b = __builtin_bit_cast(float, hw[e] & 0xffff0000u) + __builtin_bit_cast(float, lw[e] & 0xffff0000u);
      o[2 * e] = f2h_sat(a); o[2 * e + 1] = f2h_sat(b);
    }
    *reinterpret_cast<uint4*>(out + px * Cp + v * 8) = *reinterpret_cast<const uint4*>(o);
  }
}

__global__ __launch_bounds__(256) void nchw_split_kernel(const float* __restrict__ src, int64_t ssn, int64_t ssc, int64_t ssh,
                                                         int64_t ssw, u16* __restrict__ out, int C, int Cp, int H, int W) {
  __shared__ float tile[64][65];
  const int xt = blockIdx.x * 64, y = blockIdx.y % H, n = blockIdx.y / H;
  const int lane = threadIdx.x & 63, grp = threadIdx.x >> 6;
  for (int c = grp; c < Cp; c += 4) {
    const int x = xt + lane;
    tile[c][lane] = (c < C && x < W) ? src[(int64_t)n * ssn + (int64_t)c * ssc + (int64_t)y * ssh + (int64_t)x * ssw] : 0.f;
  }
  __syncthreads();
  const int V = Cp / 8;
  for (int i = threadIdx.x; i < 64 * V; i += 256) {
    const int px = i / V, v = i - px * V, x = xt + px;
    if (x >= W) continue;
    u16 hi[8], lo[8];
#pragma unroll
    for (int e = 0; e < 8; ++e) split1(tile[v * 8 + e][px], hi[e], lo[e]);
    u16* o = out + (((int64_t)n * H + y) * W + x) * 2 * Cp + v * 8;
    *reinterpret_cast<uint4*>(o) = *reinterpret_cast<const uint4*>(hi);
    *reinterpret_cast<uint4*>(o + Cp) = *reinterpret_cast<const uint4*>(lo);
  }
}

__global__ void cat_broadcast_split_kernel(const float* __restrict__ flat, int64_t fsn, int64_t fsh, int64_t fsw,
                                           const float* __restrict__ prop, int64_t psn, int64_t psh, int64_t psw,
                                           u16* __restrict__ out, int S, int H, int W, int C1, int C2, int Cp,
                                           int64_t total, int up = 0) {
  const int V = Cp / 8;
  for (int64_t idx = (int64_t)blockIdx.x * blockDim.x + threadIdx.x; idx < total;
       idx += (int64_t)gridDim.x * blockDim.x) {
    const NhwvIndex ix_ = decode_nhwv(idx, total, H, W, V);
    const int v = ix_.v, xx = ix_.x, y = ix_.y, n = ix_.n;
    const int c0 = v * 8;
    float f[8];
    if (c0 < C1 && up) {
      const int hh = H >> 1, wh = W >> 1, iy = y >> 1, ix = xx >> 1;
      const int ny = (y & 1) ? min(iy + 1, hh - 1) : max(iy - 1, 0);
      const int nx = (xx & 1) ? min(ix + 1, wh - 1) : max(ix - 1, 0);
      const float* b0 = flat + n * fsn + c0;
      const float* p00 = b0 + iy * fsh + ix * fsw;
      const float* p01 = b0 + iy * fsh + nx * fsw;
      const float* p10 = b0 + ny * fsh + ix * fsw;
      const float* p11 = b0 + ny * fsh + nx * fsw;
      __attribute__((aligned(16))) float t00[8], t01[8], t10[8], t11[8];
      *reinterpret_cast<float4*>(t00) = *reinterpret_cast<const float4*>(p00); *reinterpret_cast<float4*>(t00 + 4) = *reinterpret_cast<const float4*>(p00 + 4);
      *reinterpret_cast<float4*>(t01) = *reinterpret_cast<const float4*>(p01); *reinterpret_cast<float4*>(t01 + 4) = *reinterpret_cast<const float4*>(p01 + 4);
      *reinterpret_cast<float4*>(t10) = *reinterpret_cast<const float4*>(p10); *reinterpret_cast<float4*>(t10 + 4) = *reinterpret_cast<const float4*>(p10 + 4);
      *reinterpret_cast<float4*>(t11) = *reinterpret_cast<const float4*>(p11); *reinterpret_cast<float4*>(t11 + 4) = *reinterpret_cast<const float4*>(p11 + 4);
#pragma unroll
      for (int e = 0; e < 8; ++e) {
        float r = 0.5625f * t00[e];
        r = fmaf(0.1875f, t01[e], r);
        r = fmaf(0.1875f, t10[e], r);
        r = fmaf(0.0625f, t11[e], r);
        f[e] = r;
      }
    } else if (c0 < C1) {
      const float* src = flat + n * fsn + y * fsh + xx * fsw + c0;
      const float4 a = *reinterpret_cast<const float4*>(src), b = *reinterpret_cast<const float4*>(src + 4);
      f[0] = a.x; f[1] = a.y; f[2] = a.z; f[3] = a.w; f[4] = b.x; f[5] = b.y; f[6] = b.z; f[7] = b.w;
    } else {
      const float* src = prop + (n / S) * psn + y * psh + xx * psw + (c0 - C1);
      if (c0 - C1 + 8 <= C2) {
        const float4 a = *reinterpret_cast<const float4*>(src), b = *reinterpret_cast<const float4*>(src + 4);
        f[0] = a.x; f[1] = a.y; f[2] = a.z; f[3] = a.w; f[4] = b.x; f[5] = b.y; f[6] = b.z; f[7] = b.w;
      } else {
#pragma unroll
        for (int e = 0; e < 8; ++e) f[e] = (c0 - C1 + e < C2) ? src[e] : 0.f;
      }
    }
    u16 hi[8], lo[8];
#pragma unroll
    for (int e = 0; e < 8; ++e) split1(f[e], hi[e], lo[e]);
    u16* o = out + (((int64_t)n * H + y) * W + xx) * 2 * Cp + c0;
    *reinterpret_cast<uint4*>(o) = *reinterpret_cast<const uint4*>(hi);
    *reinterpret_cast<uint4*>(o + Cp) = *reinterpret_cast<const uint4*>(lo);
  }
}

__global__ void add_broadcast_split_kernel(const float* __restrict__ g, int64_t gsn, int64_t gsh, int64_t gsw,
                                           const float* __restrict__ gm, int64_t msn, int64_t msh, int64_t msw,
                                           float scale, u16* __restrict__ out, int S, int H, int W, int C, int Cp,
                                           int64_t total) {
  const int V = Cp / 8;
  for (int64_t idx = (int64_t)blockIdx.x * blockDim.x + threadIdx.x; idx < total;
       idx += (int64_t)gridDim.x * blockDim.x) {
    const NhwvIndex ix_ = decode_nhwv(idx, total, H, W, V);
    const int v = ix_.v, xx = ix_.x, y = ix_.y, n = ix_.n;
    const int c0 = v * 8;
    float f[8];
    if (c0 + 8 <= C) {
#pragma unroll
      for (int e = 0; e < 8; ++e) f[e] = 0.f;
      if (g) {
        const float* q = g + n * gsn + y * gsh + xx * gsw + c0;
        const float4 a = *reinterpret_cast<const float4*>(q), b = *reinterpret_cast<const float4*>(q + 4);
        f[0] = a.x; f[1] = a.y; f[2] = a.z; f[3] = a.w; f[4] = b.x; f[5] = b.y; f[6] = b.z; f[7] = b.w;
      }
      if (gm) {
        const float* q = gm + (n / S) * msn + y * msh + xx * msw + c0;
        const float4 a = *reinterpret_cast<const float4*>(q), b = *reinterpret_cast<const float4*>(q + 4);
        f[0] += a.x * scale; f[1] += a.y * scale; f[2] += a.z * scale; f[3] += a.w * scale;
        f[4] += b.x * scale; f[5] += b.y * scale; f[6] += b.z * scale; f[7] += b.w * scale;
      }
    } else {
#pragma unroll
      for (int e = 0; e < 8; ++e) {
        float a = 0.f;
        if (c0 + e < C) {
          if (g) a = g[n * gsn + y * gsh + xx * gsw + c0 + e];
          if (gm) a += gm[(n / S) * msn + y * msh + xx * msw + c0 + e] * scale;
        }
        f[e] = a;
      }
    }
    u16 hi[8], lo[8];
#pragma unroll
    for (int e = 0; e < 8; ++e) split1(f[e], hi[e], lo[e]);
    u16* o = out + (((int64_t)n * H + y) * W + xx) * 2 * Cp + c0;
    *reinterpret_cast<uint4*>(o) = *reinterpret_cast<const uint4*>(hi);
    *reinterpret_cast<uint4*>(o + Cp) = *reinterpret_cast<const uint4*>(lo);
  }
}

__global__ __launch_bounds__(256) void split_dy_colsum_kernel(const float* __restrict__ dy, int64_t dsn, int64_t dsh, int64_t dsw,
                                                              const float* __restrict__ post, int64_t psn, int64_t psh, int64_t psw,
                                                              int act, float slope, const float* __restrict__ gm, int64_t msn,
                                                              int64_t msh, int64_t msw, int S, float scale, u16* __restrict__ out,
                                                              int H, int W, int C, int Cp, int64_t M, int64_t per_block,
                                                              float* __restrict__ partial, int Np, int Gmax) {
  extern __shared__ __attribute__((aligned(16))) float smem[];
  const int V = Cp / 8, PL = 256 / V;
  const int v = threadIdx.x % V, pl = threadIdx.x / V;
  const int64_t p0 = (int64_t)blockIdx.x * per_block, p1 = min(M, p0 + per_block);
  const int c0 = v * 8;
  float acc[8] = {0.f, 0.f, 0.f, 0.f, 0.f, 0.f, 0.f, 0.f};
  if (pl < PL) {
    int xx, y, n;
    { const int64_t q0 = p0 + pl; xx = (int)(q0 % W); const int64_t t = q0 / W; y = (int)(t % H); n = (int)(t / H); }
    for (int64_t q = p0 + pl; q < p1; q += PL, xx += PL) {
      while (xx >= W) { xx -= W; if (++y == H) { y = 0; ++n; } }
      float f[8];
#pragma unroll
      for (int e = 0; e < 8; ++e) f[e] = 0.f;
      const bool whole = c0 + 8 <= C;
      if (dy) {
        const float* src = dy + n * dsn + y * dsh + xx * dsw + c0;
        if (whole) {
          const float4 a = *reinterpret_cast<const float4*>(src), b = *reinterpret_cast<const float4*>(src + 4);
          f[0] = a.x; f[1] = a.y; f[2] = a.z; f[3] = a.w; f[4] = b.x; f[5] = b.y; f[6] = b.z; f[7] = b.w;
        } else {
#pragma unroll
          for (int e = 0; e < 8; ++e) if (c0 + e < C) f[e] = src[e];
        }
      }
      if (gm) {
        const float* src = gm + (n / S) * msn + y * msh + xx * msw + c0;
        if (whole) {
          const float4 a = *reinterpret_cast<const float4*>(src), b = *reinterpret_cast<const float4*>(src + 4);
          f[0] += a.x * scale; f[1] += a.y * scale; f[2] += a.z * scale; f[3] += a.w * scale;
          f[4] += b.x * scale; f[5] += b.y * scale; f[6] += b.z * scale; f[7] += b.w * scale;
        } else {
#pragma unroll
          for (int e = 0; e < 8; ++e) if (c0 + e < C) f[e] += src[e] * scale;
        }
      }
      if (post) {
        const float* ps = post + n * psn + y * psh + xx * psw + c0;
        if (whole) {
          const float4 a = *reinterpret_cast<const float4*>(ps), b = *reinterpret_cast<const float4*>(ps + 4);
          const float g[8] = {a.x, a.y, a.z, a.w, b.x, b.y, b.z, b.w};
#pragma unroll
          for (int e = 0; e < 8; ++e) f[e] *= act_gate(g[e], act, slope);
        } else {
#pragma unroll
          for (int e = 0; e < 8; ++e)
            if (c0 + e < C) f[e] *= act_gate(ps[e], act, slope);
        }
      }
      u16 hi[8], lo[8];
#pragma unroll
      for (int e = 0; e < 8; ++e) {
        split1(f[e], hi[e], lo[e]);
        acc[e] += bf2f(hi[e]) + bf2f(lo[e]);
      }
      u16* o = out + q * 2 * Cp + c0;
      *reinterpret_cast<uint4*>(o) = *reinterpret_cast<const uint4*>(hi);
      *reinterpret_cast<uint4*>(o + Cp) = *reinterpret_cast<const uint4*>(lo);
    }
#pragma unroll
    for (int e = 0; e < 8; ++e) smem[(pl * V + v) * 8 + e] = acc[e];
  }
  __syncthreads();
  if (pl == 0) {
    for (int q = 1; q < PL; ++q)
#pragma unroll
      for (int e = 0; e < 8; ++e) acc[e] += smem[(q * V + v) * 8 + e];
#pragma unroll
    for (int e = 0; e < 8; ++e)
      if (c0 + e < Np) partial[(int64_t)blockIdx.x * Np + c0 + e] = (c0 + e < C) ? acc[e] : 0.f;
  }
  if (threadIdx.x < Np - Cp) partial[(int64_t)blockIdx.x * Np + Cp + threadIdx.x] = 0.f;
  if (blockIdx.x == 0 && threadIdx.x == 0) reinterpret_cast<int*>(partial)[(int64_t)Gmax * Np] = (int)gridDim.x;
}

__global__ void pack_weight_split_kernel(const float* __restrict__ w, u16* __restrict__ wp, int Cout, int Cin,
                                         int ks, int mode, int rows, int Np, int CS, int Ks, int Kt, int nslabs, int CSl, int f16) {
  const int64_t idx = (int64_t)blockIdx.x * blockDim.x + threadIdx.x;
  if (idx >= (int64_t)Np * Kt) return;
  const int n = (int)(idx / Kt), k = (int)(idx - (int64_t)n * Kt);
  int slab = k / Ks;
  if (slab > nslabs - 1) slab = nslabs - 1;
  const int kk = k - slab * Ks;
  const int cs = slab == nslabs - 1 ? CSl : CS;
  const int tap = kk / cs, cl = kk - tap * cs;
  const int c = slab * CS + cl;
  const int taps = ks * ks;
  const int kchan = mode == 0 ? Cin : Cout;
  float v = 0.f;
  if (n < rows && tap < taps && c < kchan) {
    if (mode == 0) v = w[((int64_t)n * Cin + c) * taps + tap];
    else           v = w[((int64_t)c * Cin + n) * taps + (taps - 1 - tap)];
  }
  u16 hi, lo;
  split1(v, hi, lo);
  if (f16) { hi = f2h_sat(v); lo = 0; }
  wp[((int64_t)n * 2) * Kt + k] = hi;
  wp[((int64_t)n * 2 + 1) * Kt + k] = lo;
}

int x_env_on(const char* name) {
  const char* e = ab_env(name);
  return (e && e[0] == '0') ? 0 : 1;
}
struct XKPlan { bool halo; int Kp, CS, nslabs, Ks, Kt, PXS, CSl, Ksl, ap; };
static int x_pick_nt(int tiles);
static bool x_last4(int kchan, int CS, int nslabs) {
  const int left = kchan - (nslabs - 1) * CS;
  return nslabs >= 2 && left >= 1 && left <= 4 && x_env_on("WCMC_HALO64_L4");
}
static XKPlan x_plan_k(int kchan, int ks, int ap_req = 2, int rows = 0) {
  const int enable = x_env_on("WCMC_IGEMM_HALO");
  XKPlan q;
  q.ap = 2;
  q.Kp = round_up(kchan, 8);
  q.halo = enable && ks >= 3 && ks <= 5 && q.Kp >= 32;
  const int nt_rows = rows > 0 ? x_pick_nt(round_up(rows, 16) / 16) : 0;
  if (ap_req == 1 && q.halo && ks == 5 && x_env_on("WCMC_HALO64") && (nt_rows == 7 || nt_rows == 1) &&
      q.Kp % 32 != 24 && x_env_on("WCMC_DGRAD_AP1")) {
    q.ap = 1;
    q.nslabs = (q.Kp + 31) / 32;
    q.CS = 32; q.CSl = q.Kp - (q.nslabs - 1) * 32;
    if (x_last4(kchan, q.CS, q.nslabs)) q.CSl = 4;
    q.PXS = 80;
    q.Ks = round_up(ks * ks * q.CS, 32); q.Ksl = round_up(ks * ks * q.CSl, 32);
    q.Kt = (q.nslabs - 1) * q.Ks + q.Ksl;
    return q;
  }
  if (ap_req == 1 && q.halo && ks == 3 && rows > 0 && x_pick_nt(round_up(rows, 16) / 16) >= 4 && x_env_on("WCMC_DGRAD_AP1")) {
    q.ap = 1;
    q.nslabs = (q.Kp + 127) / 128;
    q.CS = round_up((q.Kp + q.nslabs - 1) / q.nslabs, 8);
    q.PXS = q.CS <= 112 ? 224 : 288;
    q.Ks = round_up(ks * ks * q.CS, 32);
    q.CSl = q.Kp - (q.nslabs - 1) * q.CS;
    if (q.CSl < 32) q.CSl = q.CS;
    q.Ksl = round_up(ks * ks * q.CSl, 32);
    q.Kt = (q.nslabs - 1) * q.Ks + q.Ksl;
    return q;
  }
  if (q.halo && ks == 5 && x_env_on("WCMC_HALO64")) {
    if (q.Kp >= 256 && q.Kp % 32 == 0 && x_env_on("WCMC_HALO64_CS32")) {
      q.nslabs = q.Kp / 32;
      q.CS = q.CSl = 32;
      q.PXS = 160;
      q.Ks = q.Ksl = round_up(ks * ks * 32, 32);
      q.Kt = q.nslabs * q.Ks;
      return q;
    }
    q.nslabs = (q.Kp + 15) / 16;
    q.CS = 16; q.CSl = q.Kp - (q.nslabs - 1) * 16;
    if (x_last4(kchan, q.CS, q.nslabs)) q.CSl = 4;
    q.PXS = 80;
    q.Ks = round_up(ks * ks * q.CS, 32); q.Ksl = round_up(ks * ks * q.CSl, 32);
    q.Kt = (q.nslabs - 1) * q.Ks + q.Ksl;
    return q;
  }
  const int th8 = x_env_on("WCMC_HALO_TH8_5X5");
  if (q.halo && th8 && ks == 5 && (q.Kp % 32 == 0 || q.Kp % 32 == 8)) {
    q.nslabs = q.Kp / 32;
    q.CS = 32; q.CSl = q.Kp - (q.nslabs - 1) * 32;
    q.PXS = 160;
    q.Ks = round_up(ks * ks * q.CS, 32); q.Ksl = round_up(ks * ks * q.CSl, 32);
    q.Kt = (q.nslabs - 1) * q.Ks + q.Ksl;
    return q;
  }
  if (q.halo) {
    q.nslabs = (q.Kp + 63) / 64;
    q.CS = round_up((q.Kp + q.nslabs - 1) / q.nslabs, 8);
    q.PXS = q.CS <= 56 ? 224 : 288;
    q.Ks = round_up(ks * ks * q.CS, 32);
    q.CSl = q.Kp - (q.nslabs - 1) * q.CS;
    if (q.CSl < 32) q.CSl = q.CS;
    q.Ksl = round_up(ks * ks * q.CSl, 32);
  } else {
    q.nslabs = 1; q.CS = q.Kp; q.PXS = 0;
    q.Ks = round_up(ks * ks * q.Kp, 32);
    q.CSl = q.CS; q.Ksl = q.Ks;
  }
  q.Kt = (q.nslabs - 1) * q.Ks + q.Ksl;
  return q;
}
constexpr int XPACK_MAX = 32;
struct XPackEntry { const float* w; u16* wp; int Cout, Cin, mode, rows, Np, CS, Ks, Kt, nslabs, CSl; unsigned block0; int f16; };
struct XPackTable { XPackEntry e[XPACK_MAX]; int n, ks; };
__global__ __launch_bounds__(256) void pack_weight_split_multi_kernel(XPackTable t) {
  int k = 0;
#pragma unroll 1
  for (int i = 1; i < t.n; ++i)
    if (blockIdx.x >= t.e[i].block0) k = i;
  const XPackEntry& q = t.e[k];
  const int64_t idx = (int64_t)(blockIdx.x - q.block0) * blockDim.x + threadIdx.x;
  if (idx >= (int64_t)q.Np * q.Kt) return;
  const int n = (int)(idx / q.Kt), kk0 = (int)(idx - (int64_t)n * q.Kt);
  int slab = kk0 / q.Ks;
  if (slab > q.nslabs - 1) slab = q.nslabs - 1;
  const int kk = kk0 - slab * q.Ks;
  const int cs = slab == q.nslabs - 1 ? q.CSl : q.CS;
  const int tap = kk / cs, cl = kk - tap * cs;
  const int c = slab * q.CS + cl;
  const int taps = t.ks * t.ks;
  const int kchan = q.mode == 0 ? q.Cin : q.Cout;
  float v = 0.f;
  if (n < q.rows && tap < taps && c < kchan) {
    if (q.mode == 0) v = q.w[((int64_t)n * q.Cin + c) * taps + tap];
    else             v = q.w[((int64_t)c * q.Cin + n) * taps + (taps - 1 - tap)];
  }
  u16 hi, lo;
  split1(v, hi, lo);
  if (q.f16) { hi = f2h_sat(v); lo = 0; }
  q.wp[((int64_t)n * 2) * q.Kt + kk0] = hi;
  q.wp[((int64_t)n * 2 + 1) * q.Kt + kk0] = lo;
}

static int x_colsum_rows(int N, int Ho, int Wo) {
  const int64_t gl = ceil_div64((int64_t)N * Ho * Wo, 128);
  const int64_t gh = (int64_t)N * ((Ho + 7) / 8) * ((Wo + 15) / 16);
  return (int)(gl > gh ? gl : gh);
}

__global__ __launch_bounds__(256) void colsum_split_kernel(const u16* __restrict__ dy, int Cp, int C, int64_t M,
                                                            int64_t per_block, float* __restrict__ partial) {
  extern __shared__ __attribute__((aligned(16))) float smem[];
  const int V = Cp / 8;
  const int PL = 256 / V;
  const int v = threadIdx.x % V, pl = threadIdx.x / V;
  const int64_t p0 = (int64_t)blockIdx.x * per_block, p1 = min(M, p0 + per_block);
  float acc[8] = {0.f, 0.f, 0.f, 0.f, 0.f, 0.f, 0.f, 0.f};
  if (pl < PL) {
    for (int64_t q = p0 + pl; q < p1; q += PL) {
      const u16* r = dy + q * 2 * Cp + v * 8;
      const uint4 h = *reinterpret_cast<const uint4*>(r), l = *reinterpret_cast<const uint4*>(r + Cp);
      const unsigned hw[4] = {h.x, h.y, h.z, h.w}, lw[4] = {l.x, l.y, l.z, l.w};
#pragma unroll
      for (int e = 0; e < 4; ++e) {
        acc[2 * e] += __builtin_bit_cast(float, hw[e] << 16) + __builtin_bit_cast(float, lw[e] << 16);
        acc[2 * e + 1] += __builtin_bit_cast(float, hw[e] & 0xffff0000u) + __builtin_bit_cast(float, lw[e] & 0xffff0000u);
      }
    }
#pragma unroll
    for (int e = 0; e < 8; ++e) smem[(pl * V + v) * 8 + e] = acc[e];
  }
  __syncthreads();
  if (pl == 0) {
    for (int q = 1; q < PL; ++q)
#pragma unroll
      for (int e = 0; e < 8; ++e) acc[e] += smem[(q * V + v) * 8 + e];
#pragma unroll
    for (int e = 0; e < 8; ++e)
      if (v * 8 + e < C) partial[(int64_t)blockIdx.x * C + v * 8 + e] = acc[e];
  }
}

static int x_pick_nt(int tiles) {
  const int cand[4] = {7, 4, 2, 1};
  int best = 1, best_cost = 1 << 30;
  for (int i = 0; i < 4; ++i) {
    const int nt = cand[i];
    const int cost = ((tiles + nt - 1) / nt) * (nt + 2);
    if (cost < best_cost) { best_cost = cost; best = nt; }
  }
  return best;
}

struct XWgradPlan { int rows, rps, R, rTM, rNW; int TM, coBlocks, ciBlocks, S, Np, Cq, G; int64_t pix_per_split, per_block; size_t slab_elems, bytes; };
static XWgradPlan x_plan_wgrad(int N, int Ho, int Wo, int Cout, int Cin, int ks, int terms = 3) {
  XWgradPlan pl;
  pl.Np = round_up(Cout, 16); pl.Cq = round_up(Cin, 16);
  const int coT = pl.Np / 16, ciT = pl.Cq / 16;
  pl.TM = (coT % 7 == 0) ? 7 : 4;
  pl.coBlocks = (coT + pl.TM - 1) / pl.TM;
  pl.ciBlocks = (ciT + 3) / 4;
  const int64_t M = (int64_t)N * Ho * Wo;
  const int taps = ks * ks;
  const int rows_on = x_env_on("WCMC_WGRAD_ROWS");
  pl.R = N * Ho; pl.rps = 0; pl.rows = 0; pl.rTM = pl.rNW = 0;
  if (rows_on && (ks == 5 || ks == 3 || (ks == 1 && x_env_on("WCMC_WGRAD_ROWS_1X1"))) && (int64_t)N * Ho >= 64) {
    int tm = 0, nw = 0;
    if (ks == 5) { tm = coT % 7 == 0 ? 7 : 0; nw = ciT % 7 == 0 ? 7 : ciT == 3 ? 3 : 0; }
    else if (ks == 1) {
      if (coT == 8 && ciT == 8) { tm = 8; nw = 8; }
    }
    else if (ks == 3) {
      const int wide = x_env_on("WCMC_WGRAD_ROWS_3X3");
      const char* e44 = ab_env("WCMC_WGRAD_44");
      if (coT % 8 == 0 && ciT % 8 == 0 && (ciT >= 16 || wide) && !(e44 && e44[0] == '1')) { tm = 8; nw = 8; }
      else if (wide && coT % 4 == 0 && ciT % 4 == 0) { tm = 4; nw = 4; }
    }
    if (tm && nw) {
      pl.rows = 1; pl.rTM = tm; pl.rNW = nw;
      pl.coBlocks = coT / tm; pl.ciBlocks = ciT / nw;
      const size_t lds = xwr_lds_bytes_rt(ks, tm, nw, terms == 1 ? 1 : 2);
      int wpc = (int)((160 * 1024) / lds);
      int wcap = nw <= 4 ? 2 : 1;
      { const char* e = ab_env("WCMC_WGRAD_WCAP"); if (e && nw <= 4) wcap = atoi(e); }
      int sdiv = 1;
      { const char* e = ab_env("WCMC_WGRAD_SDIV"); if (e) sdiv = atoi(e); }
      if (wpc > wcap) wpc = wcap;
      if (wpc < 1) wpc = 1;
      int S = 8 * ((32 * wpc) / ks) / (pl.coBlocks * pl.ciBlocks) / sdiv;
      if (S > pl.R / 4) S = pl.R / 4;
      if (S < 1) S = 1;
      pl.rps = (pl.R + S - 1) / S;
      pl.S = (pl.R + pl.rps - 1) / pl.rps;
      pl.pix_per_split = 0;
    }
  }
  const int64_t tiles = (int64_t)taps * pl.coBlocks * pl.ciBlocks;
  int64_t S = (ks == 1 ? 512 : 1024) / tiles;
  const int64_t maxS = M / 512 > 0 ? M / 512 : 1;
  if (S > maxS) S = maxS;
  if (S < 1) S = 1;
  if (!pl.rows) {
    pl.pix_per_split = ceil_div64(ceil_div64(M, S), 64) * 64;
    pl.S = (int)ceil_div64(M, pl.pix_per_split);
  }
  pl.slab_elems = (size_t)pl.S * taps * pl.Np * pl.Cq;
  pl.G = (int)(M / 64 > 0 ? (M / 64 < 1024 ? M / 64 : 1024) : 1);
  pl.per_block = ceil_div64(M, pl.G);
  pl.G = (int)ceil_div64(M, pl.per_block);
  pl.bytes = (pl.slab_elems + (size_t)pl.G * Cout) * sizeof(float);
  return pl;
}

}

using namespace wcmc;

extern "C" size_t wcmc_split_elems(int N, int H, int W, int C) {
  if (N <= 0 || H <= 0 || W <= 0 || C <= 0) return 0;
  return (size_t)N * H * W * 2 * round_up(C, 8);
}

extern "C" int wcmc_split_bf16(const float* x, int64_t xsn, int64_t xsh, int64_t xsw, void* out, int N, int H, int W,
                               int C, void* stream) {
  WCMC_REQUIRE(N > 0 && H > 0 && W > 0 && C > 0 && out, WCMC_ERR_BAD_ARG, "split_bf16: bad argument");
  WCMC_REQUIRE(nhwc_view_ok(x, xsn, xsh, xsw, C) && aligned16(out), WCMC_ERR_ALIGNMENT,
               "split_bf16: x violates the NHWC-view contract (or out unaligned)");
  const int Cp = round_up(C, 8);
  const int64_t total = (int64_t)N * H * W * (Cp / 8);
  const int64_t blocks = ceil_div64(total, 256);
  hipLaunchKernelGGL(split_kernel, dim3((unsigned)(blocks < 16384 ? blocks : 16384)), dim3(256), 0, (hipStream_t)stream,
                     x, xsn, xsh, xsw, (u16*)out, H, W, C, Cp, total, (const float*)nullptr, (int64_t)0, (int64_t)0,
                     (int64_t)0, 0, 0.f);
  return check_launch("split_bf16");
}

extern "C" int wcmc_split_gated_bf16(const float* dy, int64_t xsn, int64_t xsh, int64_t xsw, const float* post, int64_t psn,
                                     int64_t psh, int64_t psw, int act, float slope, void* out, int N, int H, int W, int C,
                                     void* stream) {
  WCMC_REQUIRE(N > 0 && H > 0 && W > 0 && C > 0 && out, WCMC_ERR_BAD_ARG, "split_gated_bf16: bad argument");
  WCMC_REQUIRE(nhwc_view_ok(dy, xsn, xsh, xsw, C) && nhwc_view_ok(post, psn, psh, psw, C) && aligned16(out),
               WCMC_ERR_ALIGNMENT, "split_gated_bf16: dy / post violate the NHWC-view contract (or out unaligned)");
  const int Cp = round_up(C, 8);
  const int64_t total = (int64_t)N * H * W * (Cp / 8);
  const int64_t blocks = ceil_div64(total, 256);
  hipLaunchKernelGGL(split_kernel, dim3((unsigned)(blocks < 16384 ? blocks : 16384)), dim3(256), 0, (hipStream_t)stream,
                     dy, xsn, xsh, xsw, (u16*)out, H, W, C, Cp, total, post, psn, psh, psw, act, slope);
  return check_launch("split_gated_bf16");
}

extern "C" int wcmc_split_from_nchw(const float* src, int64_t ssn, int64_t ssc, int64_t ssh, int64_t ssw, void* out_split,
                                    int N, int C, int H, int W, void* stream) {
  WCMC_REQUIRE(src && out_split && N > 0 && C > 0 && C <= 64 && H > 0 && W > 0, WCMC_ERR_BAD_ARG,
               "split_from_nchw: bad argument (at most 64 channels)");
  WCMC_REQUIRE(aligned16(out_split), WCMC_ERR_ALIGNMENT, "split_from_nchw: out must be 16-byte aligned");
  WCMC_REQUIRE((int64_t)N * H <= 65535, WCMC_ERR_BAD_ARG, "split_from_nchw: N*H > 65535");
  hipLaunchKernelGGL(nchw_split_kernel, dim3((unsigned)((W + 63) / 64), (unsigned)(N * H)), dim3(256), 0,
                     (hipStream_t)stream, src, ssn, ssc, ssh, ssw, (u16*)out_split, C, round_up(C, 8), H, W);
  return check_launch("split_from_nchw");
}

extern "C" int wcmc_cat_broadcast_split(const float* flat, int64_t fsn, int64_t fsh, int64_t fsw, const float* prop,
                                       int64_t psn, int64_t psh, int64_t psw, void* out_split, int B, int S, int H,
                                       int W, int C1, int C2, void* stream) {
  WCMC_REQUIRE(flat && prop && out_split && B > 0 && S > 0 && H > 0 && W > 0 && C1 > 0 && C2 > 0, WCMC_ERR_BAD_ARG,
               "cat_broadcast_split: bad argument");
  WCMC_REQUIRE(C1 % 8 == 0, WCMC_ERR_BAD_ARG, "cat_broadcast_split: the first operand needs a multiple of 8 channels");
  WCMC_REQUIRE(nhwc_view_ok(flat, fsn, fsh, fsw, C1) && nhwc_view_ok(prop, psn, psh, psw, C2) && aligned16(out_split),
               WCMC_ERR_ALIGNMENT, "cat_broadcast_split: a view violates the NHWC-view contract");
  const int Cp = round_up(C1 + C2, 8);
  const int64_t total = (int64_t)B * S * H * W * (Cp / 8);
  const int64_t blocks = ceil_div64(total, 256);
  hipLaunchKernelGGL(cat_broadcast_split_kernel, dim3((unsigned)(blocks > 65535 ? 65535 : blocks)), dim3(256), 0,
                     (hipStream_t)stream, flat, fsn, fsh, fsw, prop, psn, psh, psw, (u16*)out_split, S, H, W, C1, C2, Cp,
                     total, 0);
  return check_launch("cat_broadcast_split");
}

extern "C" int wcmc_cat_upsample_split(const float* deep, int64_t dsn, int64_t dsh, int64_t dsw, const float* skip,
                                       int64_t ssn, int64_t ssh, int64_t ssw, void* out_split, int N, int H, int W, int C1,
                                       int C2, void* stream) {
  WCMC_REQUIRE(deep && skip && out_split && N > 0 && H > 1 && W > 1 && (H % 2) == 0 && (W % 2) == 0 && C1 > 0 && C2 > 0,
               WCMC_ERR_BAD_ARG, "cat_upsample_split: bad argument (H and W are the fine, even, geometry)");
  WCMC_REQUIRE(C1 % 8 == 0, WCMC_ERR_BAD_ARG, "cat_upsample_split: the upsampled operand needs a multiple of 8 channels");
  WCMC_REQUIRE(nhwc_view_ok(deep, dsn, dsh, dsw, C1) && nhwc_view_ok(skip, ssn, ssh, ssw, C2) && aligned16(out_split),
               WCMC_ERR_ALIGNMENT, "cat_upsample_split: a view violates the NHWC-view contract");
  const int Cp = round_up(C1 + C2, 8);
  const int64_t total = (int64_t)N * H * W * (Cp / 8);
  const int64_t blocks = ceil_div64(total, 256);
  hipLaunchKernelGGL(cat_broadcast_split_kernel, dim3((unsigned)(blocks > 65535 ? 65535 : blocks)), dim3(256), 0,
                     (hipStream_t)stream, deep, dsn, dsh, dsw, skip, ssn, ssh, ssw, (u16*)out_split, 1, H, W, C1, C2, Cp,
                     total, 1);
  return check_launch("cat_upsample_split");
}

extern "C" int wcmc_add_broadcast_split(const float* g, int64_t gsn, int64_t gsh, int64_t gsw, const float* gm,
                                       int64_t msn, int64_t msh, int64_t msw, float scale, void* out_split, int B,
                                       int S, int H, int W, int C, void* stream) {
  WCMC_REQUIRE((g || gm) && out_split && B > 0 && S > 0 && H > 0 && W > 0 && C > 0, WCMC_ERR_BAD_ARG,
               "add_broadcast_split: bad argument");
  WCMC_REQUIRE((!g || nhwc_view_ok(g, gsn, gsh, gsw, C)) && (!gm || nhwc_view_ok(gm, msn, msh, msw, C)) &&
                   aligned16(out_split),
               WCMC_ERR_ALIGNMENT, "add_broadcast_split: a view violates the NHWC-view contract");
  const int Cp = round_up(C, 8);
  const int64_t total = (int64_t)B * S * H * W * (Cp / 8);
  const int64_t blocks = ceil_div64(total, 256);
  hipLaunchKernelGGL(add_broadcast_split_kernel, dim3((unsigned)(blocks > 65535 ? 65535 : blocks)), dim3(256), 0,
                     (hipStream_t)stream, g, gsn, gsh, gsw, gm, msn, msh, msw, scale, (u16*)out_split, S, H, W, C, Cp,
                     total);
  return check_launch("add_broadcast_split");
}

extern "C" int wcmc_split_dy_colsum_bf16(const float* dy, int64_t dsn, int64_t dsh, int64_t dsw, const float* post, int64_t psn,
                                         int64_t psh, int64_t psw, int act, float slope, const float* gm, int64_t msn,
                                         int64_t msh, int64_t msw, int S, float scale, void* out_split, float* colsum_partial,
                                         int N, int H, int W, int C, void* stream) {
  WCMC_REQUIRE((dy || gm) && out_split && colsum_partial && N > 0 && S > 0 && H > 0 && W > 0 && C > 0 && C <= 2048,
               WCMC_ERR_BAD_ARG, "split_dy_colsum_bf16: bad argument");
  WCMC_REQUIRE(!gm || N % S == 0, WCMC_ERR_BAD_ARG, "split_dy_colsum_bf16: N must be a multiple of S");
  WCMC_REQUIRE((!dy || nhwc_view_ok(dy, dsn, dsh, dsw, C)) && (!post || nhwc_view_ok(post, psn, psh, psw, C)) &&
                   (!gm || nhwc_view_ok(gm, msn, msh, msw, C)) && aligned16(out_split),
               WCMC_ERR_ALIGNMENT, "split_dy_colsum_bf16: a view violates the NHWC-view contract (or out unaligned)");
  const int Cp = round_up(C, 8), Np = round_up(C, 16);
  const int64_t M = (int64_t)N * H * W;
  const int Gmax = x_colsum_rows(N, H, W);
  int blocks = Gmax < 1024 ? Gmax : 1024;
  const int64_t per_block = ceil_div64(M, blocks);
  blocks = (int)ceil_div64(M, per_block);
  hipLaunchKernelGGL(split_dy_colsum_kernel, dim3((unsigned)blocks), dim3(256), (size_t)256 * 8 * sizeof(float),
                     (hipStream_t)stream, dy, dsn, dsh, dsw, post, psn, psh, psw, act, slope, gm, msn, msh, msw, S, scale,
                     (u16*)out_split, H, W, C, Cp, M, per_block, colsum_partial, Np, Gmax);
  return check_launch("split_dy_colsum_bf16");
}

static inline int x_mode_ap(int mode) { return mode >= 2 ? 1 : 2; }
static inline bool x_mode_fwd(int mode) { return mode == 0 || mode == 3 || mode == 4; }
extern "C" size_t wcmc_conv2d_packed_elems_bf16x3(int rows, int kchan, int ks, int mode) {
  if (rows <= 0 || kchan <= 0 || ks <= 0 || mode < 0 || mode > 4) return 0;
  return (size_t)round_up(rows, 16) * 2 * x_plan_k(kchan, ks, x_mode_ap(mode), rows).Kt;
}

extern "C" int wcmc_conv2d_pack_weight_bf16x3(const float* w, void* wp, int Cout, int Cin, int ks, int mode,
                                              void* stream) {
  WCMC_REQUIRE(w && wp && Cout > 0 && Cin > 0 && ks > 0 && mode >= 0 && mode <= 4, WCMC_ERR_BAD_ARG,
               "conv2d_pack_weight_bf16x3: bad argument");
  const int rows = x_mode_fwd(mode) ? Cout : Cin, kchan = x_mode_fwd(mode) ? Cin : Cout;
  const int Np = round_up(rows, 16);
  const XKPlan q = x_plan_k(kchan, ks, x_mode_ap(mode), rows);
  const int64_t total = (int64_t)Np * q.Kt;
  hipLaunchKernelGGL(pack_weight_split_kernel, dim3((unsigned)ceil_div64(total, 256)), dim3(256), 0,
                     (hipStream_t)stream, w, (u16*)wp, Cout, Cin, ks, x_mode_fwd(mode) ? 0 : 1, rows, Np, q.CS, q.Ks, q.Kt, q.nslabs, q.CSl, mode == 4 ? 1 : 0);
  return check_launch("conv2d_pack_weight_bf16x3");
}

extern "C" int wcmc_conv2d_pack_chain_bf16x3(int n_entries, const float* const* w, void* const* wp, const int* Cout,
                                             const int* Cin, const int* mode, int ks, void* stream) {
  WCMC_REQUIRE(n_entries > 0 && n_entries <= XPACK_MAX && w && wp && Cout && Cin && mode && ks > 0, WCMC_ERR_BAD_ARG,
               "conv2d_pack_chain_bf16x3: bad argument (at most %d entries)", XPACK_MAX);
  XPackTable t;
  t.n = n_entries; t.ks = ks;
  unsigned blocks = 0;
  for (int i = 0; i < n_entries; ++i) {
    WCMC_REQUIRE(w[i] && wp[i] && Cout[i] > 0 && Cin[i] > 0 && mode[i] >= 0 && mode[i] <= 4, WCMC_ERR_BAD_ARG,
                 "conv2d_pack_chain_bf16x3: bad entry %d", i);
    XPackEntry& e = t.e[i];
    e.w = w[i]; e.wp = (u16*)wp[i]; e.Cout = Cout[i]; e.Cin = Cin[i]; e.mode = x_mode_fwd(mode[i]) ? 0 : 1;
    e.f16 = mode[i] == 4 ? 1 : 0;
    e.rows = x_mode_fwd(mode[i]) ? Cout[i] : Cin[i];
    const int kchan = x_mode_fwd(mode[i]) ? Cin[i] : Cout[i];
    e.Np = round_up(e.rows, 16);
    const XKPlan q = x_plan_k(kchan, ks, x_mode_ap(mode[i]), e.rows);
    e.CS = q.CS; e.Ks = q.Ks; e.Kt = q.Kt; e.nslabs = q.nslabs; e.CSl = q.CSl;
    e.block0 = blocks;
    blocks += (unsigned)ceil_div64((int64_t)e.Np * q.Kt, 256);
  }
  hipLaunchKernelGGL(pack_weight_split_multi_kernel, dim3(blocks), dim3(256), 0, (hipStream_t)stream, t);
  return check_launch("conv2d_pack_chain_bf16x3");
}

extern "C" int wcmc_conv2d_wgrad_reduce_multi(int n, void* const* workspace, float* const* dw, float* const* db,
                                              const float* const* dy_colsum_partial, const int* N, const int* Ho, const int* Wo,
                                              const int* Cout, const int* Cin, const int* ks, int terms, void* stream) {
  WCMC_REQUIRE(n > 0 && n <= WRM_MAX && workspace && dw && db && dy_colsum_partial && N && Ho && Wo && Cout && Cin && ks &&
               (terms == 1 || terms == 3), WCMC_ERR_BAD_ARG, "conv2d_wgrad_reduce_multi: bad argument (1..%d layers)", WRM_MAX);
  WRMTable t;
  t.n = n;
  unsigned blocks = 0;
  size_t lds = 0;
  for (int i = 0; i < n; ++i) {
    WCMC_REQUIRE(workspace[i] && dw[i] && N[i] > 0 && Ho[i] > 0 && Wo[i] > 0 && Cout[i] > 0 && Cin[i] > 0 && ks[i] > 0 && ks[i] <= 7,
                 WCMC_ERR_BAD_ARG, "conv2d_wgrad_reduce_multi: bad layer %d", i);
    WCMC_REQUIRE(!db[i] || dy_colsum_partial[i], WCMC_ERR_BAD_ARG,
                 "conv2d_wgrad_reduce_multi: layer %d wants a bias gradient without the column sums of dy", i);
    const XWgradPlan pl = x_plan_wgrad(N[i], Ho[i], Wo[i], Cout[i], Cin[i], ks[i], terms);
    WRMEntry& e = t.e[i];
    const bool fuse_db = db[i] != nullptr;
    e.slabs = (const float*)workspace[i]; e.dw = dw[i]; e.cs_partial = fuse_db ? dy_colsum_partial[i] : nullptr; e.db = db[i];
    e.S = pl.S; e.taps = ks[i] * ks[i]; e.Cout = Cout[i]; e.Cin = Cin[i]; e.Np = pl.Np; e.Cq = pl.Cq;
    e.cs_gmax = x_colsum_rows(N[i], Ho[i], Wo[i]); e.cs_ld = round_up(Cout[i], 16);
    e.gx = (Cin[i] + WR_CI - 1) / WR_CI;
    e.block0 = blocks;
    blocks += (unsigned)e.gx * (unsigned)(Cout[i] + (fuse_db ? (Cout[i] + 63) / 64 : 0));
    size_t l = (size_t)WR_CI * (e.taps + 1) * sizeof(float) + 256 * sizeof(float);
    if (fuse_db && l < (size_t)16 * 64 * sizeof(float)) l = (size_t)16 * 64 * sizeof(float);
    if (l > lds) lds = l;
  }
  hipLaunchKernelGGL(wgrad_reduce_multi_kernel, dim3(blocks), dim3(256), lds, (hipStream_t)stream, t);
  return check_launch("conv2d_wgrad_reduce_multi");
}

static bool x_out_f16_plan(int Cin, int Cout, int ks, XKPlan* q) {
  if (ks != 5 || Cin <= 0 || Cout <= 0) return false;
  *q = x_plan_k(Cin, ks, 1, Cout);
  return q->ap == 1 && q->halo && q->PXS == 80 && x_pick_nt(round_up(Cout, 16) / 16) == 7;
}
extern "C" int wcmc_conv2d_out_f16_supported(int Cin, int Cout, int ks) {
  XKPlan q;
  return x_out_f16_plan(Cin, Cout, ks, &q) ? 1 : 0;
}
extern "C" size_t wcmc_split_to_f16_elems(int N, int H, int W, int C) {
  return (N > 0 && H > 0 && W > 0 && C > 0) ? (size_t)N * H * W * round_up(C, 8) : 0;
}
extern "C" int wcmc_split_to_f16(const void* x_split, int N, int H, int W, int C, void* out_f16, void* stream) {
  WCMC_REQUIRE(x_split && out_f16 && N > 0 && H > 0 && W > 0 && C > 0, WCMC_ERR_BAD_ARG, "split_to_f16: bad argument");
  WCMC_REQUIRE(aligned16(x_split) && aligned16(out_f16), WCMC_ERR_ALIGNMENT, "split_to_f16: buffers must be 16-byte aligned");
  const int Cp = round_up(C, 8);
  const int64_t total = (int64_t)N * H * W * (Cp / 8);
  const int64_t blocks = ceil_div64(total, 256);
  hipLaunchKernelGGL(split_to_f16_kernel, dim3((unsigned)(blocks < 16384 ? blocks : 16384)), dim3(256), 0, (hipStream_t)stream,
                     (const u16*)x_split, (u16*)out_f16, Cp, total);
  return check_launch("split_to_f16");
}

static int x_igemm_shape(XIgemmParams& p, const char* who, int N, int H, int W, int Cin, int Cout, int ks, int pad, int terms,
                         bool split_out, int64_t ysn, int64_t ysh, int64_t ysw, bool gated, bool f16) {
  WCMC_REQUIRE(N > 0 && H > 0 && W > 0 && Cin > 0 && Cout > 0 && ks > 0 && pad >= 0, WCMC_ERR_BAD_ARG, "%s: bad argument", who);
  WCMC_REQUIRE(terms >= 1 && terms <= 3, WCMC_ERR_BAD_ARG,
               "%s: terms must be 3, 2 (x hi plane only; wp packed with mode 2 / 3) or 1 (hi planes of x and W only)", who);
  const int Ho = H + 2 * pad - ks + 1, Wo = W + 2 * pad - ks + 1;
  WCMC_REQUIRE(Ho > 0 && Wo > 0, WCMC_ERR_BAD_ARG, "%s: empty output", who);
  WCMC_REQUIRE(!gated || split_out, WCMC_ERR_BAD_ARG, "%s: a gate / a mask requires the split output geometry", who);
  XKPlan q;
  if (f16)
    WCMC_REQUIRE(x_out_f16_plan(Cin, Cout, ks, &q), WCMC_ERR_BAD_ARG,
                 "%s: no fp16 instance for this shape (ask wcmc_conv2d_out_f16_supported; 5x5, cout blocks of seven tiles)", who);
  else
    q = x_plan_k(Cin, ks, terms <= 2 ? 1 : 2, Cout);
  p = XIgemmParams{};
  p.N = N; p.H = H; p.W = W; p.Cin = Cin; p.Cpi = round_up(Cin, 8);
  p.ysn = ysn; p.ysh = ysh; p.ysw = ysw;
  p.Cpo = split_out ? round_up(Cout, 8) : round_up(Cout, 4);
  p.Ho = Ho; p.Wo = Wo; p.Cout = Cout;
  p.ks = ks; p.pad = pad;
  p.ap = f16 ? 1 : q.ap;
  p.wplanes = (f16 || (terms == 1 && q.ap == 1 && ks == 5 && q.PXS == 80 && x_pick_nt(round_up(Cout, 16) / 16) == 7)) ? 1 : 2;
  p.f16 = f16 ? 1 : 0;
  p.Kp = p.Cpi; p.Kt = q.Kt; p.Np = round_up(Cout, 16);
  p.CS = q.CS; p.nslabs = q.nslabs; p.SPS = q.Ks / 32; p.PXS = q.halo ? q.PXS : 0;
  p.CSl = q.CSl; p.SPSl = q.Ksl / 32;
  p.tilesY = (Ho + 15) / 16; p.tilesX = (Wo + 15) / 16;
  p.G = x_colsum_rows(N, Ho, Wo);
  p.M = (int64_t)N * Ho * Wo;
  const size_t xb = (f16 ? (size_t)N * H * W * p.Cpi : wcmc_split_elems(N, H, W, Cin)) * sizeof(u16), wb = (size_t)p.Np * 2 * p.Kt * sizeof(u16);
  WCMC_REQUIRE(xb < 0x7ff00000u && wb < 0x7ff00000u, WCMC_ERR_BAD_ARG, "%s: operand larger than 2 GiB (split the batch)", who);
  WCMC_REQUIRE(!q.halo || wb < 0x40000000u, WCMC_ERR_BAD_ARG, "%s: packed weights of 1 GiB or more", who);
  p.x_bytes = (unsigned)xb; p.wp_bytes = (unsigned)wb;
  return 0;
}
struct XConvPlan {
  enum { PW, HALO3, IGEMM, HALO, HALO64 } family;
  XPwPlan pw; XHalo3Plan h3; XIgemmPlan ig; XHaloPlan halo; XHalo64Plan h64;
};
static int x_plan_conv(const XIgemmParams& p, XConvPlan* c) {
  const int nt = x_pick_nt(p.Np / 16);
  if (x_plan_pw(p, &c->pw)) c->family = XConvPlan::PW;
  else if (x_halo3_ok(p)) { c->family = XConvPlan::HALO3; c->h3 = x_plan_halo3(p); }
  else if (!p.PXS) { c->family = XConvPlan::IGEMM; c->ig = x_plan_igemm(nt, p); }
  else if (x_halo_is64(p)) { c->family = XConvPlan::HALO64; c->h64 = x_plan_halo64(nt, p); }
  else { c->family = XConvPlan::HALO; return x_plan_halo(nt, p, &c->halo); }
  return 0;
}
static int x_launch_conv(const XConvPlan& c, XIgemmParams& p, hipStream_t st) {
  switch (c.family) {
    case XConvPlan::PW: return launch_xpw(p, c.pw, st);
    case XConvPlan::HALO3: return launch_xhalo3(c.h3, p, st);
    case XConvPlan::IGEMM: return launch_xigemm(c.ig, p, st);
    case XConvPlan::HALO64: return launch_xhalo64(c.h64, p, st);
    default: return launch_xhalo(c.halo, p, st);
  }
}
static int x_name_conv(const XConvPlan& c, const XIgemmParams& p, char* cls, char* kernel, size_t len) {
  const char* k = "conv_igemm";
  int kn = 0, cn = 0;
  switch (c.family) {
    case XConvPlan::PW:
      k = "conv_pw";
      kn = snprintf(kernel, len, "conv_pw_bf16x3_kernel<%d, %d, %s, 0>", c.pw.ntw, c.pw.u, p.ys ? "true" : "false");
      break;
    case XConvPlan::HALO3:
      k = c.h3.ap == 2 ? "conv_halo3" : "conv_halo3_x2";
      kn = snprintf(kernel, len, "conv_halo3_bf16x3_kernel<%d, %d, 2, 0>", c.h3.ap, c.h3.spt);
      break;
    case XConvPlan::IGEMM:
      kn = snprintf(kernel, len, "conv_igemm_bf16x3_kernel<%d, %s, %s, 0>", c.ig.nt, c.ig.padded ? "true" : "false", c.ig.dbuf ? "true" : "false");
      break;
    case XConvPlan::HALO:
      if (c.halo.nt == 7 && c.halo.th == 8 && c.halo.ap == 2) k = "conv_halo7";
      kn = snprintf(kernel, len, "conv_halo_bf16x3_kernel<%d, %d, 16, 0, %d, %d>", c.halo.nt, c.halo.th, c.halo.nb, c.halo.ap);
      break;
    case XConvPlan::HALO64: {
      const XHalo64Plan& h = c.h64;
      if (h.nt == 7 && h.nb == 2 && h.pt == 3 && h.pxst == 160) k = "conv_halo64_cs32";
      else if (h.nt == 7 && h.nb == 3 && h.pxst == 80) {
        cn = snprintf(cls, len, "conv_halo64_pt%d%s", h.pt, h.f16 ? "_h1" : h.wp == 1 ? "_x1" : h.ap == 1 ? "_x2" : "");
        k = nullptr;
      }
      kn = snprintf(kernel, len, "conv_halo64_bf16x3_kernel<%d, %d, %d, 0, %d, %d, %d, %d>", h.nt, h.nb, h.pt, h.pxst, h.ap, h.wp, h.f16);
      break;
    }
  }
  if (k) cn = snprintf(cls, len, "%s", k);
  return cn > kn ? cn : kn;
}

extern "C" int wcmc_conv2d_launch_plan_bf16x3(int N, int H, int W, int Cin, int Cout, int ks, int pad, int terms, int split_out,
                                              int64_t ysn, int64_t ysh, int64_t ysw, int gate_tensor, int out_f16,
                                              char* cls, char* kernel, size_t len) {
  const char* who = "conv2d_launch_plan_bf16x3";
  WCMC_REQUIRE(cls && kernel && len > 0, WCMC_ERR_BAD_ARG, "%s: bad argument", who);
  WCMC_REQUIRE(!out_f16 || (!split_out && !gate_tensor), WCMC_ERR_BAD_ARG, "%s: the fp16 launch writes an fp32 view, un-gated", who);
  XIgemmParams p;
  if (const int rc = x_igemm_shape(p, who, N, H, W, Cin, Cout, ks, pad, out_f16 ? 1 : terms, split_out != 0, ysn, ysh, ysw,
                                   gate_tensor != 0, out_f16 != 0)) return rc;
  static const u16 given = 0;
  if (split_out) p.ys = const_cast<u16*>(&given); else p.yf = reinterpret_cast<float*>(const_cast<u16*>(&given));
  if (gate_tensor) p.gate = &given;
  XConvPlan c;
  if (const int rc = x_plan_conv(p, &c)) return rc;
  WCMC_REQUIRE((size_t)x_name_conv(c, p, cls, kernel, len) < len, WCMC_ERR_BAD_ARG, "%s: buffers of %zu bytes are too short", who, len);
  return 0;
}

extern "C" int wcmc_conv2d_igemm_bf16x3(const void* x_split, int N, int H, int W, int Cin, const void* wp,
                                        const float* bias, float* y, int64_t ysn, int64_t ysh, int64_t ysw,
                                        void* y_split, int Cout, int ks, int pad, int act, float slope,
                                        const void* gate_split, int gate_act, float gate_slope,
                                        float* colsum_partial, const void* gate_mask, void* mask_out,
                                        int terms, void* stream) {
  const char* who = "conv2d_igemm_bf16x3";
  WCMC_REQUIRE(x_split && wp, WCMC_ERR_BAD_ARG, "%s: bad argument", who);
  WCMC_REQUIRE(!colsum_partial || y_split, WCMC_ERR_BAD_ARG,
               "conv2d_igemm_bf16x3: column sums are produced with the split output only");
  WCMC_REQUIRE((y != nullptr) != (y_split != nullptr), WCMC_ERR_BAD_ARG,
               "conv2d_igemm_bf16x3: exactly one of y (fp32 view) and y_split must be given");
  XIgemmParams p;
  if (const int rc = x_igemm_shape(p, who, N, H, W, Cin, Cout, ks, pad, terms, y_split != nullptr, ysn, ysh, ysw,
                                   gate_split || gate_mask || mask_out, false)) return rc;
  WCMC_REQUIRE(aligned16(x_split) && aligned16(wp) && (!y_split || aligned16(y_split)) &&
                   (!gate_split || aligned16(gate_split)),
               WCMC_ERR_ALIGNMENT, "conv2d_igemm_bf16x3: split buffers must be 16-byte aligned");
  WCMC_REQUIRE(!y || nhwc_view_ok(y, ysn, ysh, ysw, Cout), WCMC_ERR_ALIGNMENT,
               "conv2d_igemm_bf16x3: y violates the NHWC-view contract");
  WCMC_REQUIRE(!(gate_split && gate_mask), WCMC_ERR_BAD_ARG, "conv2d_igemm_bf16x3: gate_split and gate_mask are exclusive");
  p.x = (const u16*)x_split; p.wp = (const u16*)wp; p.bias = bias;
  p.yf = y; p.ys = (u16*)y_split;
  p.gate = (const u16*)gate_split; p.gate_act = gate_act; p.gate_slope = gate_slope;
  p.gate_mask = (const unsigned char*)gate_mask; p.mask_out = (unsigned char*)mask_out;
  p.act = act; p.slope = slope;
  p.colsum = colsum_partial;
#ifdef WCMC_DEBUG_BUILD
  {
    static int dbg = -1;
    if (dbg < 0) { const char* e = ab_env("WCMC_DEBUG_DROP"); dbg = e ? atoi(e) : 0; }
    if (dbg & 1) p.x_bytes = 0;
    if (dbg & 2) p.wp_bytes = 0;
  }
#endif
  XConvPlan c;
  if (const int rc = x_plan_conv(p, &c)) return rc;
  return x_launch_conv(c, p, (hipStream_t)stream);
}

extern "C" int wcmc_conv2d_out_f16(const void* x_f16, int N, int H, int W, int Cin, const void* wp_f16, const float* bias, float* y,
                                   int64_t ysn, int64_t ysh, int64_t ysw, int Cout, int ks, int pad, void* stream) {
  const char* who = "conv2d_out_f16";
  WCMC_REQUIRE(x_f16 && wp_f16 && y, WCMC_ERR_BAD_ARG, "%s: bad argument", who);
  XIgemmParams p;
  if (const int rc = x_igemm_shape(p, who, N, H, W, Cin, Cout, ks, pad, 1, false, ysn, ysh, ysw, false, true)) return rc;
  WCMC_REQUIRE(aligned16(x_f16) && aligned16(wp_f16) && nhwc_view_ok(y, ysn, ysh, ysw, Cout), WCMC_ERR_ALIGNMENT,
               "conv2d_out_f16: unaligned operand or y violates the NHWC-view contract");
  p.x = (const u16*)x_f16; p.wp = (const u16*)wp_f16; p.bias = bias; p.yf = y;
  p.gate_act = WCMC_ACT_LINEAR; p.act = WCMC_ACT_LINEAR;
  XConvPlan c;
  if (const int rc = x_plan_conv(p, &c)) return rc;
  return x_launch_conv(c, p, (hipStream_t)stream);
}

static bool x_pair_enabled() {
  const char* e = ab_env("WCMC_IGEMM_PW");
  const char* t = ab_env("WCMC_PW_TAIL");
  return !(e && e[0] == '0') && !(t && t[0] == '0');
}
static int x_pair_kind(int Cin, int Cout1, int Cout2) {
  const int cpi = round_up(Cin, 8);
  if (cpi == 128 && Cout1 == 128 && Cout2 >= 1 && Cout2 <= 4) return 1;
  if (cpi == 8 && Cout1 == 128 && Cout2 == 128) return 2;
  if (cpi == 64 && Cout1 == 64 && Cout2 == 64) return 3;
  return 0;
}

extern "C" int wcmc_conv1x1_pair_supported(int Cin, int Cout1, int Cout2) {
  return x_pair_enabled() && x_pair_kind(Cin, Cout1, Cout2) != 0;
}

extern "C" int wcmc_conv1x1_pair_bf16x3(const void* x_split, int N, int H, int W, int Cin, const void* wp1,
                                        const float* bias1, int Cout1, int act1, float slope1, void* y1_split,
                                        void* mask1, const void* gate_mask1, int gate_act1, float gate_slope1,
                                        float* colsum1, const void* wp2, const float* bias2, int Cout2, int act2,
                                        float slope2, float* y2, int64_t y2sn, int64_t y2sh, int64_t y2sw, void* stream) {
  WCMC_REQUIRE(N > 0 && H > 0 && W > 0 && x_split && wp1 && wp2 && y1_split && y2, WCMC_ERR_BAD_ARG,
               "conv1x1_pair_bf16x3: bad argument");
  const int kind = x_pair_enabled() ? x_pair_kind(Cin, Cout1, Cout2) : 0;
  WCMC_REQUIRE(kind != 0, WCMC_ERR_BAD_ARG, "conv1x1_pair_bf16x3: no fused instance for %d -> %d -> %d channels", Cin,
               Cout1, Cout2);
  WCMC_REQUIRE(aligned16(x_split) && aligned16(wp1) && aligned16(wp2) && aligned16(y1_split), WCMC_ERR_ALIGNMENT,
               "conv1x1_pair_bf16x3: split buffers must be 16-byte aligned");
  WCMC_REQUIRE(nhwc_view_ok(y2, y2sn, y2sh, y2sw, Cout2), WCMC_ERR_ALIGNMENT, "conv1x1_pair_bf16x3: y2 violates the NHWC-view contract");
  XIgemmParams p;
  p.x = (const u16*)x_split; p.N = N; p.H = H; p.W = W; p.Cin = Cin; p.Cpi = round_up(Cin, 8);
  p.wp = (const u16*)wp1; p.bias = bias1;
  p.yf = nullptr; p.ysn = p.ysh = p.ysw = 0;
  p.ys = (u16*)y1_split; p.Cpo = round_up(Cout1, 8);
  p.Ho = H; p.Wo = W; p.Cout = Cout1;
  p.gate = nullptr; p.gate_act = gate_act1; p.gate_slope = gate_slope1; p.gate_mask = (const unsigned char*)gate_mask1;
  p.mask_out = (unsigned char*)mask1;
  p.ks = 1; p.pad = 0; p.act = act1; p.slope = slope1;
  p.Kp = p.Cpi; p.Kt = round_up(p.Cpi, 32); p.Np = round_up(Cout1, 16);
  p.CS = p.Kp; p.nslabs = 1; p.SPS = p.Kt / 32; p.PXS = 0; p.CSl = p.CS; p.SPSl = p.SPS; p.ap = 2; p.wplanes = 2; p.f16 = 0;
  p.tilesY = p.tilesX = 0; p.G = x_colsum_rows(N, H, W); p.colsum = colsum1;
  p.M = (int64_t)N * H * W;
  const int cp2 = round_up(Cout2, 4);
  const int64_t xb = p.M * 4 * p.Cpi, yb = p.M * 4 * p.Np;
  const int64_t y2b = ((int64_t)(N - 1) * y2sn + (int64_t)(H - 1) * y2sh + (int64_t)(W - 1) * y2sw + cp2) * 4;
  WCMC_REQUIRE(xb < 0x7ff00000LL && yb < 0x7ff00000LL && y2b < 0x7ff00000LL && y2sn >= 0 && y2sh >= 0 && y2sw >= cp2,
               WCMC_ERR_BAD_ARG, "conv1x1_pair_bf16x3: operand larger than 2 GiB (split the batch)");
  p.x_bytes = (unsigned)xb; p.wp_bytes = (unsigned)((size_t)p.Np * 2 * p.Kt * sizeof(u16));
  p.y_bytes = (unsigned)yb; p.m_bytes = (unsigned)(p.M * (p.Np / 8));
  p.wp2 = (const u16*)wp2; p.bias2 = bias2; p.y2 = y2; p.y2sn = y2sn; p.y2sh = y2sh; p.y2sw = y2sw;
  p.Cout2 = Cout2; p.act2 = act2; p.slope2 = slope2; p.Kt2 = p.Np;
  p.wp2_bytes = (unsigned)((size_t)round_up(Cout2, 16) * 2 * p.Kt2 * sizeof(u16)); p.y2_bytes = (unsigned)y2b;
  hipStream_t st = (hipStream_t)stream;
  return launch_xpw_pair(kind, p, st);
}

extern "C" size_t wcmc_conv2d_igemm_colsum_elems(int N, int Ho, int Wo, int Cout) {
  if (N <= 0 || Ho <= 0 || Wo <= 0 || Cout <= 0) return 0;
  return (size_t)x_colsum_rows(N, Ho, Wo) * round_up(Cout, 16) + 4;
}

extern "C" int wcmc_colsum_finish(const float* partial, int N, int Ho, int Wo, int Cout, float* db, void* stream) {
  WCMC_REQUIRE(partial && db && N > 0 && Ho > 0 && Wo > 0 && Cout > 0, WCMC_ERR_BAD_ARG, "colsum_finish: bad argument");
  const int G = x_colsum_rows(N, Ho, Wo), Np = round_up(Cout, 16);
  hipLaunchKernelGGL(colsum_final_strided_kernel, dim3((unsigned)((Cout + 63) / 64)), dim3(1024), 0,
                     (hipStream_t)stream, partial, G, Np, Cout, db);
  return check_launch("colsum_finish");
}

extern "C" size_t wcmc_conv2d_wgrad_bf16x3_workspace_bytes(int N, int Ho, int Wo, int Cout, int Cin, int ks) {
  if (N <= 0 || Ho <= 0 || Wo <= 0 || Cout <= 0 || Cin <= 0 || ks <= 0) return 0;
  const size_t b3 = x_plan_wgrad(N, Ho, Wo, Cout, Cin, ks, 3).bytes, b1 = x_plan_wgrad(N, Ho, Wo, Cout, Cin, ks, 1).bytes;
  return b3 > b1 ? b3 : b1;
}

static int x_wgrad_shape(XWgradParams& p, XWgradPlan& pl, const char* who, int N, int H, int W, int Cin, int Cout, int ks, int pad, int terms) {
  WCMC_REQUIRE(N > 0 && H > 0 && W > 0 && Cin > 0 && Cout > 0 && ks > 0 && pad >= 0, WCMC_ERR_BAD_ARG, "%s: bad argument", who);
  WCMC_REQUIRE(terms == 3 || terms == 1, WCMC_ERR_BAD_ARG, "%s: terms must be 3 (hi*hi + hi*lo + lo*hi) or 1 (the hi planes only)", who);
  const int Ho = H + 2 * pad - ks + 1, Wo = W + 2 * pad - ks + 1;
  WCMC_REQUIRE(Ho > 0 && Wo > 0, WCMC_ERR_BAD_ARG, "%s: empty output", who);
  pl = x_plan_wgrad(N, Ho, Wo, Cout, Cin, ks, terms);
  p = XWgradParams{};
  p.N = N; p.H = H; p.W = W; p.Cin = Cin; p.Cpi = round_up(Cin, 8);
  p.Ho = Ho; p.Wo = Wo; p.Cout = Cout; p.Cpo = round_up(Cout, 8);
  p.ks = ks; p.pad = pad; p.S = pl.S; p.M = (int64_t)N * Ho * Wo;
  p.pix_per_split = pl.pix_per_split; p.Np = pl.Np; p.Cq = pl.Cq; p.coBlocks = pl.coBlocks; p.ciBlocks = pl.ciBlocks;
  const size_t xb = wcmc_split_elems(N, H, W, Cin) * sizeof(u16), yb = wcmc_split_elems(N, Ho, Wo, Cout) * sizeof(u16);
  WCMC_REQUIRE(xb < 0x7ff00000u && yb < 0x7ff00000u, WCMC_ERR_BAD_ARG, "%s: operand larger than 2 GiB (split the batch)", who);
  p.x_bytes = (unsigned)xb; p.dy_bytes = (unsigned)yb;
  p.xps = 4 * p.Cpi; p.yps = 4 * p.Cpo;
  return 0;
}

extern "C" int wcmc_conv2d_wgrad_launch_plan_bf16x3(int N, int H, int W, int Cin, int Cout, int ks, int pad, int terms,
                                                    char* cls, char* kernel, size_t len) {
  const char* who = "conv2d_wgrad_launch_plan_bf16x3";
  WCMC_REQUIRE(cls && kernel && len > 0, WCMC_ERR_BAD_ARG, "%s: bad argument", who);
  XWgradParams p;
  XWgradPlan pl;
  if (const int rc = x_wgrad_shape(p, pl, who, N, H, W, Cin, Cout, ks, pad, terms)) return rc;
  const XWRowsPlan r = x_plan_wgrad_rows(ks, pl.rTM, pl.rNW, terms == 1 ? 1 : 2);
  const int cn = snprintf(cls, len, "%s", (pl.rows && ks == 5 && pl.rTM == 7 && pl.rNW == 7) ? "conv_wgrad_rows" : "conv_wgrad");
  const int kn = pl.rows && r.rows8 ? snprintf(kernel, len, "conv_wgrad_rows8_bf16x3_kernel<0, %d, %d>", r.xe, r.pl)
                 : pl.rows ? snprintf(kernel, len, "conv_wgrad_rows_bf16x3_kernel<%d, %d, %d, 0, %d>", r.ks, r.tm, r.nw, r.pl)
                           : snprintf(kernel, len, "conv_wgrad_bf16x3_kernel<%d, %d>", pl.TM, r.pl);
  WCMC_REQUIRE((size_t)(cn > kn ? cn : kn) < len, WCMC_ERR_BAD_ARG, "%s: buffers of %zu bytes are too short", who, len);
  return 0;
}

extern "C" int wcmc_conv2d_wgrad_bf16x3(const void* x_split, int N, int H, int W, int Cin, const void* dy_split,
                                        int Cout, int ks, int pad, float* dw, float* db, void* workspace,
                                        size_t workspace_bytes, int phase, const float* dy_colsum_partial, int terms,
                                        void* stream) {
  const char* who = "conv2d_wgrad_bf16x3";
  WCMC_REQUIRE(dw && workspace && x_split && dy_split, WCMC_ERR_BAD_ARG, "%s: bad argument", who);
  XWgradParams p;
  XWgradPlan pl;
  if (const int rc = x_wgrad_shape(p, pl, who, N, H, W, Cin, Cout, ks, pad, terms)) return rc;
  const int Ho = p.Ho, Wo = p.Wo;
  WCMC_REQUIRE(aligned16(x_split) && aligned16(dy_split), WCMC_ERR_ALIGNMENT,
               "conv2d_wgrad_bf16x3: split buffers must be 16-byte aligned");
  WCMC_REQUIRE(workspace_bytes >= pl.bytes && aligned16(workspace), WCMC_ERR_WORKSPACE,
               "conv2d_wgrad_bf16x3: workspace %zu < %zu bytes (or unaligned)", workspace_bytes, pl.bytes);
  WCMC_REQUIRE(phase >= 0 && phase <= 2, WCMC_ERR_BAD_ARG, "conv2d_wgrad_bf16x3: phase must be 0, 1 or 2");
  hipStream_t st = (hipStream_t)stream;
  p.x = (const u16*)x_split; p.dy = (const u16*)dy_split; p.slabs = (float*)workspace;
  int rc = 0;
  if (phase != 2 && pl.rows) {
    XWRowsParams q;
    q.x = p.x; q.N = N; q.H = H; q.W = W; q.Cpi = p.Cpi; q.dy = p.dy; q.Ho = Ho; q.Wo = Wo; q.Cpo = p.Cpo;
    q.dbg = (float*)workspace + pl.slab_elems;
    { const char* e = ab_env("WCMC_WGRAD_ROWS8_PRIO"); q.prio = e ? atoi(e) : 8; if (q.prio < 0 || q.prio > 13) q.prio = 0; }
    q.pad = pad; q.slabs = p.slabs; q.S = pl.S; q.rps = pl.rps; q.R = pl.R; q.Np = pl.Np; q.Cq = pl.Cq;
    q.coBlocks = pl.coBlocks; q.ciBlocks = pl.ciBlocks; q.x_bytes = p.x_bytes; q.dy_bytes = p.dy_bytes;
    q.xps = p.xps; q.yps = p.yps;
    rc = launch_xwgrad_rows(x_plan_wgrad_rows(ks, pl.rTM, pl.rNW, terms == 1 ? 1 : 2), q, st);
  } else if (phase != 2) {
    rc = launch_xwgrad(pl.TM, terms == 1 ? 1 : 2, p, st);
  }
  if (rc || phase == 1) return rc;
  const bool fuse_db = db && dy_colsum_partial;
  const int cs_rows = fuse_db ? (Cout + 63) / 64 : 0;
  size_t red_lds = (size_t)WR_CI * (ks * ks + 1) * sizeof(float) + 256 * sizeof(float);
  if (fuse_db && red_lds < (size_t)16 * 64 * sizeof(float)) red_lds = (size_t)16 * 64 * sizeof(float);
  hipLaunchKernelGGL(wgrad_reduce_kernel, dim3((unsigned)((Cin + WR_CI - 1) / WR_CI), (unsigned)(Cout + cs_rows)), dim3(256),
                     red_lds, st, p.slabs, dw, pl.S, ks * ks, Cout, Cin, pl.Np, pl.Cq, fuse_db ? dy_colsum_partial : nullptr,
                     x_colsum_rows(N, Ho, Wo), round_up(Cout, 16), db);
  rc = check_launch("conv2d_wgrad_bf16x3_reduce");
  if (rc || !db || fuse_db) return rc;
  float* partial = (float*)workspace + pl.slab_elems;
  WCMC_REQUIRE(p.Cpo / 8 <= 256, WCMC_ERR_BAD_ARG, "conv2d_wgrad_bf16x3: Cout > 2048 unsupported");
  hipLaunchKernelGGL(colsum_split_kernel, dim3((unsigned)pl.G), dim3(256), (size_t)256 * 8 * sizeof(float), st, p.dy,
                     p.Cpo, Cout, p.M, pl.per_block, partial);
  hipLaunchKernelGGL(colsum_final_kernel, dim3((unsigned)((Cout + 63) / 64)), dim3(1024), 0, st, partial, pl.G, Cout,
                     db);
  return check_launch("conv2d_bias_grad_bf16x3");
}
```

### wcmc_amd/ops/__init__.py

```python
import os

import torch
import weakref

from .._lib import check, lib

MODES = ("bf16x321h", "bf16x321", "bf16x321o", "bf16x3", "fp32")


PRECISION = os.environ.get("WCMC_PRECISION", MODES[0])
assert PRECISION in MODES, PRECISION


def _side_stream_default(mode):
    return os.environ.get("WCMC_SIDE_STREAM") == "1"


USE_SIDE_STREAM = _side_stream_default(PRECISION)

USE_BRANCH_STREAM = os.environ.get("WCMC_BRANCH_STREAM", "1") != "0"

FUSE_EMBED = os.environ.get("WCMC_FUSE_EMBED", "1") != "0"

EMBED_IN_PLACE = os.environ.get("WCMC_EMBED_IN_PLACE", "1") != "0"

FUSE_FINAL = os.environ.get("WCMC_FUSE_FINAL", "1") != "0"

SAVE_FINAL_HIDDEN = True

TERMS_BY_KS = {}

EMULATE_HIDDEN = None

DEBUG_ACTS = None

DEFER_MAX_BYTES = 24 << 20

_PROFILER = None
_DEFERRED = None


def reduced_backward(mode=None):
    return (PRECISION if mode is None else mode) in ("bf16x321h", "bf16x321o", "bf16x321")


def set_precision(mode):
    global PRECISION, USE_SIDE_STREAM
    assert mode in MODES, mode
    PRECISION = mode
    USE_SIDE_STREAM = _side_stream_default(mode)


def split_path():
    return PRECISION != "fp32"


def wgrad_terms():
    return 1 if reduced_backward() else 3


def dgrad_terms():
    return 2 if reduced_backward() else 3


def chain_terms(ks, cin=None):
    return TERMS_BY_KS.get((ks, cin), TERMS_BY_KS.get(ks, (wgrad_terms(), dgrad_terms())))


def out_layer_terms(ks, act):
    if PRECISION == "bf16x321h" and ks == 5 and act == "linear":
        return "h"
    if not (PRECISION == "bf16x321o" and ks == 5 and act == "linear"):
        return 3
    return 1


from ._base import (ACT, LEAKY_SLOPE, set_profiler, _Timed, _ptr, _stream, _need_cuda, nhwc_empty, is_nhwc_view, _v,
                    to_nhwc_raw, from_nhwc_raw, _ToNHWC, as_nhwc, _as_nhwc_nograd, conv_launch_plan, wgrad_launch_plan, _timed_conv)
from .streams import (_SIDE_STREAMS, _side_stream, _BRANCH_STREAMS, branch_stream, _step_streams, fork_all_streams,
                      join_all_streams, _STREAM_PAIRS, _spin_ms, concurrent_stream_pair, on_branch)
from .conv_fp32 import (_pack, conv2d_raw, conv2d_wgrad_raw, act_backward_raw, _ConvChain)
from .grads import (_GRAD_SINK, register_grad_sinks, release_grad_sinks, _sink_ex, _sink, _param_ptr, _flushed_by_consumer,
                    _WeightNormMulti, WEIGHT_NORM_MAX_LAYERS, weight_norm_multi, deferred_wgrad_reduce, flush_wgrad_reduce,
                    _on_side_stream, _reduce_multi)
from .elementwise import (_MaxPool2, _MaxPool2Skip, maxpool2_skip, _Upsample2, maxpool2, upsample2, _CatChannels, cat_channels,
                          _SppMean, spp_mean, _CatBroadcast, cat_broadcast, _PBufferCat, pbuffer_cat, _SampleCat,
                          sample_features_cat)
from .conv_split import (_split_empty, split_raw, split_from_nchw_raw, presplit_shared, split_gated_raw, split_dy_colsum_raw,
                         unsplit_debug, _dgrad_mode, _pack_x, _fwd_pack_mode, PACK_MAX_ENTRIES, _pack_chains_x, _pack_chain_x,
                         _chain_out_terms, conv2d_x_raw, conv2d_out_f16_raw, conv1x1_pair_x_raw, colsum_finish_raw,
                         conv2d_wgrad_x_raw, _chainx_forward, _chainx_backward, _ConvChainX, _split_shared, _ChainSppMeanX,
                         _CatBroadcastChainX, _CatUpsampleChainX, conv_chain)
from .pathnet_fused import (_dense_pixel_stride, _EmbedSppMeanFusedX, _FinalFusedX, cat_upsample_chain, _UNFUSED_NOTED,
                            _note_unfused, conv_chain_spp_mean, cat_broadcast_chain, embed_in_place, embed_in_place_supported,
                            _reads_in_place)
from .image import (_KernelApply, kernel_apply, chain_kernel_apply, _Recombine, recombine, _image_loss_raw, _L1Mean, l1_mean,
                    image_metrics, relative_mse, LOSS2_KINDS, _ImageLoss2, image_loss2, image_eval)
from .splat import (SPLAT_SOFTMAX, SPLAT_SHIFT, _splat_dims, _KernelSplat, kernel_splat, logit_max)
from .filter import (PBF_STATS, PBF_FILTER, PBF_MAX_RADIUS, PBF_MAX_PATCH_RADIUS, PBF_MAX_CHANNELS,
                     PBF_MAX_IMAGE_CHANNELS, _pbuffer_filter_check, pbuffer_filter)
from .manifold import (_FeatureMSE, _GRS, grs_loss, feature_mse)
from .optim import (clip_grad_norm_, clip_adam_, clip_adam_hyper, clip_adam_dev_, step_guard_, step_guard_local_,
                    step_guard_global_)
from .data import (_need_dense, preprocess_llpm, preprocess_kpcn, assemble_kpcn_patches, gradients, reflect_index,
                   preprocess_kpcn_begin, preprocess_kpcn_rows, preprocess_kpcn_end,
                   importance_map, sampling_prob, sanitize_, random_permutation, random_permutation_dev, step_counter_advance,
                   permutation_key, check_tile_coords, stitch_tiles, preprocess_sbmc, check_patch_origins, sample_feature_size,
                   assemble_sample_patches, preprocess_kpcn_prefix, check_tile_origins, assemble_kpcn_tiles, finish_frame,
                   assemble_sample_tiles, finish_sample_frame, check_patch_transforms)
```

### wcmc_amd/ops/conv_split.py

```python
import ctypes

import torch

from .. import ops as _sw
from .._lib import check, lib
from ._base import (ACT, LEAKY_SLOPE, _Timed, _as_nhwc_nograd, _need_cuda, _ptr, _stream, _timed_conv, _v, wgrad_launch_plan,
                    as_nhwc, nhwc_empty)
from .conv_fp32 import _ConvChain
from .grads import _flushed_by_consumer, _on_side_stream, _sink_ex
from .streams import _side_stream


def _split_empty(n, c, h, w, device):
    return torch.empty(lib().wcmc_split_elems(n, h, w, c), device=device, dtype=torch.int16)


def split_raw(x):
    n, c, h, w = x.shape
    out = _split_empty(n, c, h, w, x.device)
    check(lib().wcmc_split_bf16(*_v(x), _ptr(out), n, h, w, c, _stream()), "split_bf16")
    return out


def split_from_nchw_raw(x):
    n, c, h, w = x.shape
    out = _split_empty(n, c, h, w, x.device)
    check(lib().wcmc_split_from_nchw(_ptr(x), *x.stride(), _ptr(out), n, c, h, w, _stream()), "split_from_nchw")
    return out


def presplit_shared(x):
    _need_cuda(x)
    x._wcmc_split = ((x._version, None), split_from_nchw_raw(x))
    return x


def split_gated_raw(dy, post, act):
    n, c, h, w = dy.shape
    out = _split_empty(n, c, h, w, dy.device)
    check(lib().wcmc_split_gated_bf16(*_v(dy), *_v(post), ACT[act], LEAKY_SLOPE, _ptr(out), n, h, w, c, _stream()),
          "split_gated_bf16")
    return out


def split_dy_colsum_raw(dims, dy=None, post=None, act="linear", gm=None, s=1, scale=1.0):
    n, c, h, w = dims
    dev = (dy if dy is not None else gm).device
    out = _split_empty(n, c, h, w, dev)
    part = torch.empty(lib().wcmc_conv2d_igemm_colsum_elems(n, h, w, c), device=dev, dtype=torch.float32)
    z = (_ptr(None), 0, 0, 0)
    check(lib().wcmc_split_dy_colsum_bf16(*(_v(dy) if dy is not None else z), *(_v(post) if post is not None else z), ACT[act],
                                          LEAKY_SLOPE, *(_v(gm) if gm is not None else z), s, float(scale), _ptr(out), _ptr(part),
                                          n, h, w, c, _stream()), "split_dy_colsum_bf16")
    return out, part


def unsplit_debug(t, n, c, h, w):
    cp = (c + 7) // 8 * 8
    v = t.view(torch.bfloat16).view(n, h, w, 2, cp).float()
    return (v[:, :, :, 0] + v[:, :, :, 1])[..., :c].permute(0, 3, 1, 2)


def _dgrad_mode(terms=None):
    return 2 if (_sw.dgrad_terms() if terms is None else terms) == 2 else 1


def _pack_x(weight, mode):
    cout, cin, ks, _ = weight.shape
    rows, kch = (cout, cin) if mode in (0, 3, 4) else (cin, cout)
    wp = torch.empty(lib().wcmc_conv2d_packed_elems_bf16x3(rows, kch, ks, mode), device=weight.device, dtype=torch.int16)
    w = weight.detach()
    if not w.is_contiguous():
        w = w.contiguous()
    check(lib().wcmc_conv2d_pack_weight_bf16x3(_ptr(w), _ptr(wp), cout, cin, ks, mode, _stream()),
          "pack_weight_bf16x3")
    return wp




def _fwd_pack_mode(out_terms):
    return 4 if out_terms == "h" else 0 if out_terms == 3 else 3


PACK_MAX_ENTRIES = 32


def _pack_chains_x(chains, ks):
    assert sum(2 * len(w) for w, _ in chains) <= PACK_MAX_ENTRIES
    dev = chains[0][0][0].device
    ws, outs, couts, cins, modes, keep, res = [], [], [], [], [], [], []
    for weights, out_terms in chains:
        n = len(weights)
        dmode = _dgrad_mode(_sw.chain_terms(ks, weights[0].shape[1])[1])
        per = []
        for li, wt in enumerate(weights):
            w = wt.detach()
            if not w.is_contiguous():
                w = w.contiguous()
            keep.append(w)
            cout, cin = w.shape[0], w.shape[1]
            pair = []
            for mode in (_fwd_pack_mode(out_terms) if li == n - 1 else 0, dmode):
                rows, kch = (cout, cin) if mode in (0, 3, 4) else (cin, cout)
                wp = torch.empty(lib().wcmc_conv2d_packed_elems_bf16x3(rows, kch, ks, mode), device=dev, dtype=torch.int16)
                ws.append(w.data_ptr()); outs.append(wp.data_ptr()); couts.append(cout); cins.append(cin); modes.append(mode)
                pair.append(wp)
            per.append((pair[0], pair[1], (_fwd_pack_mode(out_terms) if li == n - 1 else 0, dmode)))
        res.append(per)
    m = len(ws)
    arr_p, arr_i = ctypes.c_void_p * m, ctypes.c_int * m
    check(lib().wcmc_conv2d_pack_chain_bf16x3(m, arr_p(*ws), arr_p(*outs), arr_i(*couts), arr_i(*cins), arr_i(*modes), ks,
                                              _stream()), "conv2d_pack_chain_bf16x3")
    return res


def _pack_chain_x(weights, ks, out_terms=3):
    return [(a, b) for a, b, _ in _pack_chains_x([(weights, out_terms)], ks)[0]]


def _chain_out_terms(ks, act_last, cin_last, cout_last, pair):
    oterms = 3 if pair else _sw.out_layer_terms(ks, act_last)
    if oterms == "h" and not lib().wcmc_conv2d_out_f16_supported(cin_last, cout_last, ks):
        oterms = 3
    return oterms


def conv2d_x_raw(xs, dims, wp, bias, cout, ks, pad, act, out_split, gate=None, gate_act="linear", colsum=False,
                 gate_mask=None, mask_out=False, terms=3, out=None):
    n, cin, h, w = dims
    ho, wo = h + 2 * pad - ks + 1, w + 2 * pad - ks + 1
    dev = xs.device
    if out_split:
        ysp, yf, yv = _split_empty(n, cout, ho, wo, dev), None, (_ptr(None), 0, 0, 0)
    else:
        yf = nhwc_empty(n, cout, ho, wo, dev) if out is None else out
        assert tuple(yf.shape) == (n, cout, ho, wo)
        ysp, yv = None, _v(yf)
    part = None
    if colsum:
        part = torch.empty(lib().wcmc_conv2d_igemm_colsum_elems(n, ho, wo, cout), device=dev, dtype=torch.float32)
    mask = None
    if mask_out:
        mask = torch.empty(n * ho * wo * ((cout + 7) // 8), device=dev, dtype=torch.uint8)
    with _timed_conv(dims, cout, ks, pad, terms, yf, gate is not None):
        check(lib().wcmc_conv2d_igemm_bf16x3(_ptr(xs), n, h, w, cin, _ptr(wp), _ptr(bias), *yv, _ptr(ysp), cout,
                                             ks, pad, ACT[act], LEAKY_SLOPE, _ptr(gate), ACT[gate_act], LEAKY_SLOPE,
                                             _ptr(part), _ptr(gate_mask), _ptr(mask), terms, _stream()), "conv2d_igemm_bf16x3")
    out = ysp if out_split else yf
    ret = (out,) + ((part,) if colsum else ()) + ((mask,) if mask_out else ())
    return ret if len(ret) > 1 else out


def conv2d_out_f16_raw(xs, dims, wp16, bias, cout, ks, pad):
    n, cin, h, w = dims
    ho, wo = h + 2 * pad - ks + 1, w + 2 * pad - ks + 1
    x16 = torch.empty(lib().wcmc_split_to_f16_elems(n, h, w, cin), device=xs.device, dtype=torch.int16)
    check(lib().wcmc_split_to_f16(_ptr(xs), n, h, w, cin, _ptr(x16), _stream()), "split_to_f16")
    y = nhwc_empty(n, cout, ho, wo, xs.device)
    with _timed_conv(dims, cout, ks, pad, 1, y, False, f16=True):
        check(lib().wcmc_conv2d_out_f16(_ptr(x16), n, h, w, cin, _ptr(wp16), _ptr(bias), *_v(y), cout, ks, pad, _stream()), "conv2d_out_f16")
    return y


def conv1x1_pair_x_raw(xs, dims, wp1, b1, cout1, act1, wp2, b2, cout2, act2, gate_mask=None, gate_act="linear",
                       colsum=False, mask_out=True):
    n, cin, h, w = dims
    dev = xs.device
    ysp = _split_empty(n, cout1, h, w, dev)
    mask = torch.empty(n * h * w * ((cout1 + 7) // 8), device=dev, dtype=torch.uint8) if mask_out else None
    part = None
    if colsum:
        part = torch.empty(lib().wcmc_conv2d_igemm_colsum_elems(n, h, w, cout1), device=dev, dtype=torch.float32)
    y2 = nhwc_empty(n, cout2, h, w, dev)
    with _Timed("conv_pw", 4.0 * n * h * w * ((cin + 7) // 8 * 8 + cout1 + (cout2 + 3) // 4 * 4), "byte"):
        check(lib().wcmc_conv1x1_pair_bf16x3(_ptr(xs), n, h, w, cin, _ptr(wp1), _ptr(b1), cout1, ACT[act1], LEAKY_SLOPE,
                                             _ptr(ysp), _ptr(mask), _ptr(gate_mask), ACT[gate_act], LEAKY_SLOPE,
                                             _ptr(part), _ptr(wp2), _ptr(b2), cout2, ACT[act2], LEAKY_SLOPE,
                                             *_v(y2), _stream()), "conv1x1_pair_bf16x3")
    return ysp, mask, part, y2


def colsum_finish_raw(part, dims):
    n, c, h, w = dims
    db = torch.empty(c, device=part.device, dtype=torch.float32)
    check(lib().wcmc_colsum_finish(_ptr(part), n, h, w, c, _ptr(db), _stream()), "colsum_finish")
    return db


def conv2d_wgrad_x_raw(xs, xdims, dys, cout, ks, pad, weight_shape, want_bias=True, colsum_part=None, terms=None, sinks=(0, 0),
                       dw_flushed=False):
    n, cin, h, w = xdims
    ho, wo = h + 2 * pad - ks + 1, w + 2 * pad - ks + 1
    nbytes = lib().wcmc_conv2d_wgrad_bf16x3_workspace_bytes(n, ho, wo, cout, cin, ks)
    ws = torch.empty((nbytes + 3) // 4, device=xs.device, dtype=torch.float32)
    dw, dw_view = _sink_ex(sinks[0], weight_shape, xs.device)
    db, db_view = _sink_ex(sinks[1], (cout,), xs.device) if (want_bias or colsum_part is not None) else (None, True)
    args = (_ptr(xs), n, h, w, cin, _ptr(dys), cout, ks, pad, _ptr(dw), _ptr(db), _ptr(ws), ws.numel() * 4)
    cs = _ptr(colsum_part)
    terms = _sw.wgrad_terms() if terms is None else terms
    safe = (dw_view or dw_flushed) and db_view
    if (_sw._PROFILER is None and _sw._DEFERRED is not None and safe and nbytes <= _sw.DEFER_MAX_BYTES and (db is None or colsum_part is not None)
            and not _on_side_stream()):
        check(lib().wcmc_conv2d_wgrad_bf16x3(*args, 1, cs, terms, _stream()), "conv2d_wgrad_bf16x3")
        st = torch.cuda.current_stream()
        _sw._DEFERRED.setdefault(st.cuda_stream, (st, []))[1].append((ws, dw.data_ptr() if dw_view else dw, db.data_ptr() if db is not None else 0,
                                                                  colsum_part, n, ho, wo, cout, cin, ks, terms))
    elif _sw._PROFILER is None:
        check(lib().wcmc_conv2d_wgrad_bf16x3(*args, 0, cs, terms, _stream()), "conv2d_wgrad_bf16x3")
    else:
        with _Timed(wgrad_launch_plan(n, h, w, cin, cout, ks, pad, terms)[0], 2.0 * n * ho * wo * cout * cin * ks * ks, "flop"):
            check(lib().wcmc_conv2d_wgrad_bf16x3(*args, 1, cs, terms, _stream()), "conv2d_wgrad_bf16x3")
        with _Timed("conv_wgrad_finish", 0.0, "flop"):
            check(lib().wcmc_conv2d_wgrad_bf16x3(*args, 2, cs, terms, _stream()), "conv2d_wgrad_bf16x3")
    return dw, db




def _chainx_forward(ctx, xs0, dims0, spec, params, extra_saved=None):
    ks, pad, acts = spec[:3]
    ctx.dx_channels = spec[3] if len(spec) > 3 else None
    spec = tuple(spec[:3])
    nl = len(acts)
    n = dims0[0]
    dims = [dims0]
    xs = [xs0]
    masks = []
    y = None
    pair = (ks == 1 and pad == 0 and nl >= 2 and
            lib().wcmc_conv1x1_pair_supported(params[2 * nl - 4].shape[1], params[2 * nl - 4].shape[0],
                                              params[2 * nl - 2].shape[0]))
    ctx.terms = _sw.chain_terms(ks, dims0[1])
    oterms = _chain_out_terms(ks, acts[-1], params[2 * nl - 2].shape[1], params[2 * nl - 2].shape[0], pair)
    packs = _pack_chain_x([params[2 * l] for l in range(nl)], ks, oterms) if 2 * nl <= PACK_MAX_ENTRIES else None
    ctx.wp1 = [pk[1] for pk in packs] if packs is not None else None
    pack0 = (lambda l: packs[l][0]) if packs is not None else (lambda l: _pack_x(params[2 * l], _fwd_pack_mode(oterms) if l == nl - 1 else 0))
    for l in range(nl):
        wt, b = params[2 * l], params[2 * l + 1]
        cout = wt.shape[0]
        if wt.shape[1] != dims[l][1]:
            raise RuntimeError("conv chain layer %d: weight expects %d input channels, got a tensor with %d"
                               % (l, wt.shape[1], dims[l][1]))
        wp = pack0(l)
        hidden = l < nl - 1
        if pair and l == nl - 2:
            xs1, mask1, _, y = conv1x1_pair_x_raw(xs[l], dims[l], wp, b.detach(), cout, acts[l], pack0(l + 1),
                                                  params[2 * l + 3].detach(), params[2 * l + 2].shape[0], acts[l + 1])
            hh, ww = dims[l][2], dims[l][3]
            dims.append((n, cout, hh, ww))
            dims.append((n, params[2 * l + 2].shape[0], hh, ww))
            xs.append(xs1)
            masks.append(mask1)
            break
        if not hidden and oterms == "h":
            out = conv2d_out_f16_raw(xs[l], dims[l], wp, b.detach(), cout, ks, pad)
        else:
            out = conv2d_x_raw(xs[l], dims[l], wp, b.detach(), cout, ks, pad, acts[l], out_split=hidden, mask_out=hidden,
                               terms=3 if hidden else oterms)
        hh, ww = dims[l][2] + 2 * pad - ks + 1, dims[l][3] + 2 * pad - ks + 1
        dims.append((n, cout, hh, ww))
        if hidden:
            xs.append(out[0] if _sw.EMULATE_HIDDEN is None else _sw.EMULATE_HIDDEN(out[0], dims[-1], ks))
            masks.append(out[1])
        else:
            y = out
    ctx.spec, ctx.dims = spec, dims
    ctx.bias_ptrs = [params[2 * l + 1].data_ptr() if isinstance(params[2 * l + 1], torch.nn.Parameter) else 0 for l in range(nl)]
    keep_y = [y] if acts[-1] != "linear" else []
    extra = tuple(extra_saved(y)) if extra_saved is not None else ()
    ctx.n_extra = len(extra)
    ctx.save_for_backward(*xs, *masks, *keep_y, *[params[2 * l] for l in range(nl)], *extra)
    if _sw.DEBUG_ACTS is not None:
        _sw.DEBUG_ACTS.extend(unsplit_debug(xs[l + 1], *dims[l + 1]) for l in range(nl - 1))
        if acts[-1] != "linear":
            _sw.DEBUG_ACTS.append(y)
    return y


def _chainx_backward(ctx, dy, need_dx, dys=None, part=None):
    ks, pad, acts = ctx.spec
    dims = ctx.dims
    nl = len(acts)
    saved = ctx.saved_tensors
    xs = saved[:nl]
    masks = saved[nl:2 * nl - 1]
    off = 2 * nl - 1
    if dys is None:
        dy = _as_nhwc_nograd(dy)
        gated = acts[-1] != "linear"
        dys, part = split_dy_colsum_raw(dims[nl], dy=dy, post=saved[off] if gated else None, act=acts[-1])
        off += 1 if gated else 0
    else:
        assert acts[-1] == "linear"
    ws = saved[off:len(saved) - getattr(ctx, "n_extra", 0)]
    grads = [None] * (2 * nl)
    dx = None
    main = torch.cuda.current_stream()
    side = _side_stream(dys.device)
    keep = []
    wp1 = getattr(ctx, "wp1", None)
    wterms, dterms = ctx.terms
    bptrs = getattr(ctx, "bias_ptrs", None) or [0] * nl
    sink_of = lambda l: (ws[l].data_ptr() if isinstance(ws[l], torch.nn.Parameter) else 0, bptrs[l])
    flushed = [_flushed_by_consumer(w) for w in ws]
    pack1 = (lambda l: wp1[l]) if wp1 is not None else (lambda l: _pack_x(ws[l], _dgrad_mode(dterms)))
    for l in range(nl - 1, -1, -1):
        wt = ws[l]
        cout = wt.shape[0]
        if side is not None:
            side.wait_stream(main)
            with torch.cuda.stream(side):
                dw, db = conv2d_wgrad_x_raw(xs[l], dims[l], dys, cout, ks, pad, wt.shape, want_bias=part is None,
                                            colsum_part=part, terms=wterms, sinks=sink_of(l), dw_flushed=flushed[l])
            dw.record_stream(main)
            db.record_stream(main)
            keep.append(dys)
            keep.append(part)
        else:
            dw, db = conv2d_wgrad_x_raw(xs[l], dims[l], dys, cout, ks, pad, wt.shape, want_bias=part is None,
                                        colsum_part=part, terms=wterms, sinks=sink_of(l), dw_flushed=flushed[l])
        grads[2 * l], grads[2 * l + 1] = dw, db
        if (l == 1 and need_dx and ks == 1 and pad == 0 and
                lib().wcmc_conv1x1_pair_supported(cout, wt.shape[1], ws[0].shape[1])):
            dys, _, part, dx = conv1x1_pair_x_raw(dys, dims[2], pack1(1), None, wt.shape[1], "linear",
                                                  pack1(0), None, ws[0].shape[1], "linear",
                                                  gate_mask=masks[0], gate_act=acts[0], colsum=True, mask_out=False)
        elif l > 0:
            wpt = pack1(l)
            dys, part = conv2d_x_raw(dys, dims[l + 1], wpt, None, wt.shape[1], ks, ks - 1 - pad, "linear",
                                     out_split=True, gate_act=acts[l - 1], colsum=True, terms=dterms, gate_mask=masks[l - 1])
        elif need_dx and dx is None:
            sub = getattr(ctx, "dx_channels", None)
            if sub is not None and (sub[1] + 7) // 8 * 8 - sub[0] // 8 * 8 <= wt.shape[1] // 2:
                a0, a1 = sub[0] // 8 * 8, min((sub[1] + 7) // 8 * 8, wt.shape[1])
                nn_, _, hh_, ww_ = dims[0]
                dx = nhwc_empty(nn_, wt.shape[1], hh_, ww_, dys.device, zero=True)
                wsub = _pack_x(wt.detach()[:, a0:a1].contiguous(), _dgrad_mode(dterms))
                conv2d_x_raw(dys, dims[l + 1], wsub, None, a1 - a0, ks, ks - 1 - pad, "linear", out_split=False, terms=dterms,
                             out=dx[:, a0:a1])
            else:
                wpt = pack1(l)
                dx = conv2d_x_raw(dys, dims[l + 1], wpt, None, wt.shape[1], ks, ks - 1 - pad, "linear",
                                  out_split=False, terms=dterms)
    if side is not None:
        main.wait_stream(side)
    del keep
    return dx, grads


class _ConvChainX(torch.autograd.Function):

    @staticmethod
    def forward(ctx, x, spec, *params):
        _need_cuda(x, *params)
        return _chainx_forward(ctx, split_raw(x), tuple(x.shape), spec, params)

    @staticmethod
    def backward(ctx, dy):
        dx, grads = _chainx_backward(ctx, dy, ctx.needs_input_grad[0])
        return (dx, None, *grads)


def _split_shared(x):
    tag = (x._version, torch.cuda.current_stream().cuda_stream)
    cached = getattr(x, "_wcmc_split", None)
    if cached is not None and cached[0] == tag:
        return cached[1]
    if cached is not None and cached[0] == (x._version, None):
        cached[1].record_stream(torch.cuda.current_stream())
        return cached[1]
    xs = split_raw(x)
    if not x.requires_grad:
        x._wcmc_split = (tag, xs)
    return xs


class _ChainSppMeanX(torch.autograd.Function):

    @staticmethod
    def forward(ctx, x, s, spec, *params):
        _need_cuda(x, *params)
        assert spec[2][-1] == "linear"
        y = _chainx_forward(ctx, _split_shared(x), tuple(x.shape), spec, params)
        bs, c, h, w = y.shape
        m = nhwc_empty(bs // s, c, h, w, y.device)
        check(lib().wcmc_spp_reduce(*_v(y), *_v(m), bs // s, s, h, w, c, 1.0 / s, _stream()), "spp_reduce")
        ctx.s = s
        return y, m

    @staticmethod
    def backward(ctx, gy, gm):
        s = ctx.s
        bs, c, h, w = ctx.dims[-1]
        gy = _as_nhwc_nograd(gy) if gy is not None else None
        gm = _as_nhwc_nograd(gm) if gm is not None else None
        dys, part = split_dy_colsum_raw((bs, c, h, w), dy=gy, gm=gm, s=s, scale=1.0 / s)
        dx, grads = _chainx_backward(ctx, None, ctx.needs_input_grad[0], dys=dys, part=part)
        return (dx, None, None, *grads)


class _CatBroadcastChainX(torch.autograd.Function):

    @staticmethod
    def forward(ctx, flat, prop, s, spec, *params):
        _need_cuda(flat, prop, *params)
        bs, c1, h, w = flat.shape
        b, c2 = prop.shape[0], prop.shape[1]
        assert bs == b * s and c1 % 8 == 0 and prop.shape[2:] == flat.shape[2:]
        xs0 = _split_empty(bs, c1 + c2, h, w, flat.device)
        check(lib().wcmc_cat_broadcast_split(*_v(flat), *_v(prop), _ptr(xs0), b, s, h, w, c1, c2, _stream()),
              "cat_broadcast_split")
        ctx.cat = (b, s, c1, c2)
        return _chainx_forward(ctx, xs0, (bs, c1 + c2, h, w), spec, params)

    @staticmethod
    def backward(ctx, dy):
        b, s, c1, c2 = ctx.cat
        need = ctx.needs_input_grad[0] or ctx.needs_input_grad[1]
        dx, grads = _chainx_backward(ctx, dy, need)
        dflat = dprop = None
        if need:
            _, _, h, w = dx.shape
            dflat = dx[:, :c1]
            if s == 1:
                dprop = dx[:, c1:]
            else:
                dprop = nhwc_empty(b, c2, h, w, dx.device)
                check(lib().wcmc_spp_reduce(*_v(dx[:, c1:]), *_v(dprop), b, s, h, w, c2, 1.0, _stream()), "spp_reduce")
        return (dflat, dprop, None, None, *grads)


class _CatUpsampleChainX(torch.autograd.Function):

    @staticmethod
    def forward(ctx, deep, skip, spec, *params):
        _need_cuda(deep, skip, *params)
        n, c1, hd, wd = deep.shape
        c2, h, w = skip.shape[1:]
        assert skip.shape[0] == n and h == 2 * hd and w == 2 * wd and c1 % 8 == 0
        xs0 = _split_empty(n, c1 + c2, h, w, deep.device)
        check(lib().wcmc_cat_upsample_split(*_v(deep), *_v(skip), _ptr(xs0), n, h, w, c1, c2, _stream()), "cat_upsample_split")
        ctx.cat = (n, c1, c2, h, w)
        return _chainx_forward(ctx, xs0, (n, c1 + c2, h, w), spec, params)

    @staticmethod
    def backward(ctx, dy):
        n, c1, c2, h, w = ctx.cat
        need = ctx.needs_input_grad[0] or ctx.needs_input_grad[1]
        dx, grads = _chainx_backward(ctx, dy, need)
        ddeep = dskip = None
        if need:
            g = dx[:, :c1]
            ddeep = nhwc_empty(n, c1, h // 2, w // 2, dx.device)
            check(lib().wcmc_upsample2_bwd(*_v(g), *_v(ddeep), n, h // 2, w // 2, c1, _stream()), "upsample2_bwd")
            dskip = dx[:, c1:]
        return (ddeep, dskip, None, *grads)


def conv_chain(x, ksize, pad, acts, params):
    if not _sw.split_path():
        return _ConvChain.apply(as_nhwc(x), (ksize, pad, tuple(acts)), *params)
    hint = getattr(x, "_wcmc_grad_channels", None)
    spec = (ksize, pad, tuple(acts)) + ((tuple(hint),) if hint is not None else ())
    return _ConvChainX.apply(as_nhwc(x), spec, *params)
```

Measured before the change: 736.8.

## Fold low-plane weights into empty rows of a partial last Cout tile

When the last 16-row output-channel tile holds only 1 to 8 real rows, the weight packer puts the low bf16 plane of those rows into the tile's unused upper 8 rows. The halo64 kernel then skips the separate low-weight MFMA for that tile and combines the two halves with a cross-lane ds_bpermute add before the epilogue. This removes one MFMA per pixel tile on the last Cout tile of 7-tile, two-weight-plane layers. It adds a new pack mode, a new entry point and a support query, plus per-layer Python logic that decides when to fold in forward and dgrad chains.

New measurement: 727.3. -1.3%, worse.

```diff
diff --git a/include/wcmc_hip.h b/include/wcmc_hip.h
--- a/include/wcmc_hip.h
+++ b/include/wcmc_hip.h
@@ -72,6 +72,7 @@
                               const float* post, int64_t psn, int64_t psh, int64_t psw, int act, float slope,
                               const float* gm, int64_t msn, int64_t msh, int64_t msw, int S, float scale,
                               void* out_split, float* colsum_partial, int N, int H, int W, int C, void* stream);
+#define WCMC_PACK_FOLD 8
 size_t wcmc_conv2d_packed_elems_bf16x3(int rows, int kchan, int ks, int mode);
 int wcmc_conv2d_pack_weight_bf16x3(const float* w_oihw, void* wp, int Cout, int Cin, int ks, int mode,
                                    void* stream);
@@ -83,6 +84,13 @@
                              int ks, int pad, int act, float slope,
                              const void* gate_split, int gate_act, float gate_slope,
                              float* colsum_partial, const void* gate_mask, void* mask_out, int terms, void* stream);
+int wcmc_conv2d_fold_supported(int N, int H, int W, int Cin, int Cout, int ks, int pad, int terms, int orientation);
+int wcmc_conv2d_igemm_fold_bf16x3(const void* x_split, int N, int H, int W, int Cin,
+                                  const void* wp_folded, const float* bias,
+                                  float* y, int64_t ysn, int64_t ysh, int64_t ysw, void* y_split, int Cout,
+                                  int ks, int pad, int act, float slope,
+                                  const void* gate_split, int gate_act, float gate_slope,
+                                  float* colsum_partial, const void* gate_mask, void* mask_out, int terms, void* stream);
 int wcmc_conv2d_out_f16_supported(int Cin, int Cout, int ks);
 size_t wcmc_split_to_f16_elems(int N, int H, int W, int C);
 int wcmc_split_to_f16(const void* x_split, int N, int H, int W, int C, void* out_f16, void* stream);
diff --git a/wcmc_amd/_lib.py b/wcmc_amd/_lib.py
--- a/wcmc_amd/_lib.py
+++ b/wcmc_amd/_lib.py
@@ -34,6 +34,8 @@
     "wcmc_conv2d_pack_weight_bf16x3": (I, [P, P, I, I, I, I, P]),
     "wcmc_conv2d_pack_chain_bf16x3": (I, [I, P, P, P, P, P, I, P]),
     "wcmc_conv2d_igemm_bf16x3": (I, [P, I, I, I, I, P, P, P, L, L, L, P, I, I, I, I, F, P, I, F, P, P, P, I, P]),
+    "wcmc_conv2d_fold_supported": (I, [I, I, I, I, I, I, I, I, I]),
+    "wcmc_conv2d_igemm_fold_bf16x3": (I, [P, I, I, I, I, P, P, P, L, L, L, P, I, I, I, I, F, P, I, F, P, P, P, I, P]),
     "wcmc_conv2d_out_f16_supported": (I, [I, I, I]),
     "wcmc_split_to_f16_elems": (Z, [I, I, I, I]),
     "wcmc_split_to_f16": (I, [P, I, I, I, I, P, P]),
diff --git a/wcmc_amd/csrc/bf16x3_common.h b/wcmc_amd/csrc/bf16x3_common.h
--- a/wcmc_amd/csrc/bf16x3_common.h
+++ b/wcmc_amd/csrc/bf16x3_common.h
@@ -91,6 +91,7 @@
   int ap;
   int wplanes;
   int f16;
+  int fold;
   unsigned y_bytes, m_bytes;
   const u16* wp2; const float* bias2; float* y2; int64_t y2sn, y2sh, y2sw;
   int Cout2, act2, Kt2; float slope2; unsigned wp2_bytes, y2_bytes;
diff --git a/wcmc_amd/csrc/bf16x3_halo64.hip b/wcmc_amd/csrc/bf16x3_halo64.hip
--- a/wcmc_amd/csrc/bf16x3_halo64.hip
+++ b/wcmc_amd/csrc/bf16x3_halo64.hip
@@ -44,6 +44,7 @@
   const int oy0 = tr ? trow * 16 : PT == 4 ? (trow < p.rows16 ? trow * 16 : p.rows16 * 16 + (trow - p.rows16) * 12) : trow * TH;
   const int ox0 = tr ? p.tilesX * TW + (trem - trow * tcols) * 12 : (trem - trow * tcols) * TW;
   const int n0 = blockIdx.y * BN;
+  const int fold = (NT == 7 && WP == 2 && !F16 && n0 + BN >= p.Cout) ? p.fold : 0;
 
   const __amdgpu_buffer_rsrc_t xr = __builtin_amdgcn_make_buffer_rsrc((void*)p.x, 0, (int)p.x_bytes, 0x00020000);
   const __amdgpu_buffer_rsrc_t wr = __builtin_amdgcn_make_buffer_rsrc((void*)p.wp, 0, (int)p.wp_bytes, 0x00020000);
@@ -232,11 +233,17 @@
     __builtin_amdgcn_sched_barrier(0);
 #pragma unroll
     for (int j = 0; j < NT; ++j) {
+      constexpr bool FT = NT == 7 && WP == 2 && !F16;
+      if (FT && j == NT - 1 && !(DBG & 1) && !fold) {
+#pragma unroll
+        for (int i = 0; i < PT; ++i)
+          if (i < ptc) acc[j][i] = __builtin_amdgcn_mfma_f32_16x16x32_bf16(wl[j], ah[i], acc[j][i], 0, 0, 0);
+      }
 #pragma unroll
       for (int i = 0; i < PT; ++i) {
         if (i >= ptc) continue;
         if (!(DBG & 1)) {
-          if (WP == 2) acc[j][i] = __builtin_amdgcn_mfma_f32_16x16x32_bf16(wl[j], ah[i], acc[j][i], 0, 0, 0);
+          if (WP == 2 && !(FT && j == NT - 1)) acc[j][i] = __builtin_amdgcn_mfma_f32_16x16x32_bf16(wl[j], ah[i], acc[j][i], 0, 0, 0);
           if (AP == 2) acc[j][i] = __builtin_amdgcn_mfma_f32_16x16x32_bf16(wh[j], al[i], acc[j][i], 0, 0, 0);
           if (F16) acc[j][i] = __builtin_amdgcn_mfma_f32_16x16x32_f16(__builtin_bit_cast(xf16x8, wh[j]), __builtin_bit_cast(xf16x8, ah[i]), acc[j][i], 0, 0, 0);
           else acc[j][i] = __builtin_amdgcn_mfma_f32_16x16x32_bf16(wh[j], ah[i], acc[j][i], 0, 0, 0);
@@ -274,6 +281,18 @@
     return;
   }
   const int fq = kg * 4;
+  if (WP == 2 && fold) {
+    __builtin_amdgcn_sched_barrier(0);
+#pragma unroll
+    for (int i = 0; i < PT; ++i)
+#pragma unroll
+      for (int e = 0; e < 4; ++e) {
+        const float a = acc[NT - 1][i][e];
+        const float up = __builtin_bit_cast(float, __builtin_amdgcn_ds_bpermute(((lane + 32) & 63) * 4, __builtin_bit_cast(int, a)));
+        acc[NT - 1][i][e] = fq + e < fold ? a + up : 0.f;
+      }
+    __builtin_amdgcn_sched_barrier(0);
+  }
   float bv[NT][4];
   {
     const __amdgpu_buffer_rsrc_t brs =
@@ -472,6 +491,8 @@
 static int launch_xhalo64c(const XHalo64Plan& h, const XIgemmParams& p, hipStream_t stream) {
   WCMC_REQUIRE(h.nt == NT && h.nb == NB && h.pt == PT && h.pxst == PXST && h.ap == AP && h.wp == WP && h.f16 == F16, WCMC_ERR_LAUNCH,
                "conv2d_igemm_bf16x3(halo, 64 pixels per wave): no instance for the plan");
+  WCMC_REQUIRE(!p.fold || (NT == 7 && WP == 2 && !F16 && p.fold == p.Cout % 16 && p.fold <= 8 && (p.Np / 16) % NT == 0), WCMC_ERR_BAD_ARG,
+               "conv2d_igemm_fold_bf16x3: a folded pack needs a two-plane weight instance whose last cout tile holds 1..8 rows");
   static LdsAttr attr;
   if (set_max_lds(reinterpret_cast<const void*>(&conv_halo64_bf16x3_kernel<NT, NB, PT, 0, PXST, AP, WP, F16>), h.lds, attr) != hipSuccess) return WCMC_ERR_LAUNCH;
   const dim3 grid((unsigned)(p.N * (p.tilesX * p.tilesY + (PT == 4 ? p.stripX * p.stripY : 0))), (unsigned)((p.Np / 16 + NT - 1) / NT));
diff --git a/wcmc_amd/csrc/conv_bf16x3.hip b/wcmc_amd/csrc/conv_bf16x3.hip
--- a/wcmc_amd/csrc/conv_bf16x3.hip
+++ b/wcmc_amd/csrc/conv_bf16x3.hip
@@ -266,10 +266,12 @@
 }
 
 __global__ void pack_weight_split_kernel(const float* __restrict__ w, u16* __restrict__ wp, int Cout, int Cin,
-                                         int ks, int mode, int rows, int Np, int CS, int Ks, int Kt, int nslabs, int CSl, int f16) {
+                                         int ks, int mode, int rows, int Np, int CS, int Ks, int Kt, int nslabs, int CSl, int f16, int fold) {
   const int64_t idx = (int64_t)blockIdx.x * blockDim.x + threadIdx.x;
   if (idx >= (int64_t)Np * Kt) return;
-  const int n = (int)(idx / Kt), k = (int)(idx - (int64_t)n * Kt);
+  const int n0 = (int)(idx / Kt), k = (int)(idx - (int64_t)n0 * Kt);
+  const bool folded = fold && n0 >= rows - fold + 8 && n0 < rows + 8;
+  const int n = folded ? n0 - 8 : n0;
   int slab = k / Ks;
   if (slab > nslabs - 1) slab = nslabs - 1;
   const int kk = k - slab * Ks;
@@ -286,8 +288,9 @@
   u16 hi, lo;
   split1(v, hi, lo);
   if (f16) { hi = f2h_sat(v); lo = 0; }
-  wp[((int64_t)n * 2) * Kt + k] = hi;
-  wp[((int64_t)n * 2 + 1) * Kt + k] = lo;
+  if (folded) { hi = lo; lo = 0; }
+  wp[((int64_t)n0 * 2) * Kt + k] = hi;
+  wp[((int64_t)n0 * 2 + 1) * Kt + k] = lo;
 }
 
 int x_env_on(const char* name) {
@@ -373,7 +376,7 @@
   return q;
 }
 constexpr int XPACK_MAX = 32;
-struct XPackEntry { const float* w; u16* wp; int Cout, Cin, mode, rows, Np, CS, Ks, Kt, nslabs, CSl; unsigned block0; int f16; };
+struct XPackEntry { const float* w; u16* wp; int Cout, Cin, mode, rows, Np, CS, Ks, Kt, nslabs, CSl; unsigned block0; int f16, fold; };
 struct XPackTable { XPackEntry e[XPACK_MAX]; int n, ks; };
 __global__ __launch_bounds__(256) void pack_weight_split_multi_kernel(XPackTable t) {
   int k = 0;
@@ -383,7 +386,9 @@
   const XPackEntry& q = t.e[k];
   const int64_t idx = (int64_t)(blockIdx.x - q.block0) * blockDim.x + threadIdx.x;
   if (idx >= (int64_t)q.Np * q.Kt) return;
-  const int n = (int)(idx / q.Kt), kk0 = (int)(idx - (int64_t)n * q.Kt);
+  const int n0 = (int)(idx / q.Kt), kk0 = (int)(idx - (int64_t)n0 * q.Kt);
+  const bool folded = q.fold && n0 >= q.rows - q.fold + 8 && n0 < q.rows + 8;
+  const int n = folded ? n0 - 8 : n0;
   int slab = kk0 / q.Ks;
   if (slab > q.nslabs - 1) slab = q.nslabs - 1;
   const int kk = kk0 - slab * q.Ks;
@@ -400,8 +405,9 @@
   u16 hi, lo;
   split1(v, hi, lo);
   if (q.f16) { hi = f2h_sat(v); lo = 0; }
-  q.wp[((int64_t)n * 2) * q.Kt + kk0] = hi;
-  q.wp[((int64_t)n * 2 + 1) * q.Kt + kk0] = lo;
+  if (folded) { hi = lo; lo = 0; }
+  q.wp[((int64_t)n0 * 2) * q.Kt + kk0] = hi;
+  q.wp[((int64_t)n0 * 2 + 1) * q.Kt + kk0] = lo;
 }
 
 static int x_colsum_rows(int N, int Ho, int Wo) {
@@ -635,23 +641,28 @@
   return check_launch("split_dy_colsum_bf16");
 }
 
-static inline int x_mode_ap(int mode) { return mode >= 2 ? 1 : 2; }
-static inline bool x_mode_fwd(int mode) { return mode == 0 || mode == 3 || mode == 4; }
+static inline bool x_mode_ok(int mode) { return (mode >= 0 && mode <= 4) || (mode >= WCMC_PACK_FOLD && mode <= WCMC_PACK_FOLD + 2); }
+static inline int x_mode_base(int mode) { return mode & ~WCMC_PACK_FOLD; }
+static inline int x_mode_fold(int mode, int rows) { return (mode & WCMC_PACK_FOLD) ? rows % 16 : 0; }
+static inline bool x_fold_rows_ok(int mode, int rows) { return !(mode & WCMC_PACK_FOLD) || (rows % 16 >= 1 && rows % 16 <= 8); }
+static inline int x_mode_ap(int mode) { return x_mode_base(mode) >= 2 ? 1 : 2; }
+static inline bool x_mode_fwd(int mode) { const int b = x_mode_base(mode); return b == 0 || b == 3 || b == 4; }
 extern "C" size_t wcmc_conv2d_packed_elems_bf16x3(int rows, int kchan, int ks, int mode) {
-  if (rows <= 0 || kchan <= 0 || ks <= 0 || mode < 0 || mode > 4) return 0;
+  if (rows <= 0 || kchan <= 0 || ks <= 0 || !x_mode_ok(mode) || !x_fold_rows_ok(mode, rows)) return 0;
   return (size_t)round_up(rows, 16) * 2 * x_plan_k(kchan, ks, x_mode_ap(mode), rows).Kt;
 }
 
 extern "C" int wcmc_conv2d_pack_weight_bf16x3(const float* w, void* wp, int Cout, int Cin, int ks, int mode,
                                               void* stream) {
-  WCMC_REQUIRE(w && wp && Cout > 0 && Cin > 0 && ks > 0 && mode >= 0 && mode <= 4, WCMC_ERR_BAD_ARG,
+  WCMC_REQUIRE(w && wp && Cout > 0 && Cin > 0 && ks > 0 && x_mode_ok(mode), WCMC_ERR_BAD_ARG,
                "conv2d_pack_weight_bf16x3: bad argument");
   const int rows = x_mode_fwd(mode) ? Cout : Cin, kchan = x_mode_fwd(mode) ? Cin : Cout;
+  WCMC_REQUIRE(x_fold_rows_ok(mode, rows), WCMC_ERR_BAD_ARG, "conv2d_pack_weight_bf16x3: a folded mode needs 1 <= rows %% 16 <= 8 (rows = %d)", rows);
   const int Np = round_up(rows, 16);
   const XKPlan q = x_plan_k(kchan, ks, x_mode_ap(mode), rows);
   const int64_t total = (int64_t)Np * q.Kt;
   hipLaunchKernelGGL(pack_weight_split_kernel, dim3((unsigned)ceil_div64(total, 256)), dim3(256), 0,
-                     (hipStream_t)stream, w, (u16*)wp, Cout, Cin, ks, x_mode_fwd(mode) ? 0 : 1, rows, Np, q.CS, q.Ks, q.Kt, q.nslabs, q.CSl, mode == 4 ? 1 : 0);
+                     (hipStream_t)stream, w, (u16*)wp, Cout, Cin, ks, x_mode_fwd(mode) ? 0 : 1, rows, Np, q.CS, q.Ks, q.Kt, q.nslabs, q.CSl, mode == 4 ? 1 : 0, x_mode_fold(mode, rows));
   return check_launch("conv2d_pack_weight_bf16x3");
 }
 
@@ -663,12 +674,14 @@
   t.n = n_entries; t.ks = ks;
   unsigned blocks = 0;
   for (int i = 0; i < n_entries; ++i) {
-    WCMC_REQUIRE(w[i] && wp[i] && Cout[i] > 0 && Cin[i] > 0 && mode[i] >= 0 && mode[i] <= 4, WCMC_ERR_BAD_ARG,
+    WCMC_REQUIRE(w[i] && wp[i] && Cout[i] > 0 && Cin[i] > 0 && x_mode_ok(mode[i]) &&
+                     x_fold_rows_ok(mode[i], x_mode_fwd(mode[i]) ? Cout[i] : Cin[i]), WCMC_ERR_BAD_ARG,
                  "conv2d_pack_chain_bf16x3: bad entry %d", i);
     XPackEntry& e = t.e[i];
     e.w = w[i]; e.wp = (u16*)wp[i]; e.Cout = Cout[i]; e.Cin = Cin[i]; e.mode = x_mode_fwd(mode[i]) ? 0 : 1;
     e.f16 = mode[i] == 4 ? 1 : 0;
     e.rows = x_mode_fwd(mode[i]) ? Cout[i] : Cin[i];
+    e.fold = x_mode_fold(mode[i], e.rows);
     const int kchan = x_mode_fwd(mode[i]) ? Cin[i] : Cout[i];
     e.Np = round_up(e.rows, 16);
     const XKPlan q = x_plan_k(kchan, ks, x_mode_ap(mode[i]), e.rows);
@@ -843,13 +856,30 @@
   return 0;
 }
 
-extern "C" int wcmc_conv2d_igemm_bf16x3(const void* x_split, int N, int H, int W, int Cin, const void* wp,
-                                        const float* bias, float* y, int64_t ysn, int64_t ysh, int64_t ysw,
-                                        void* y_split, int Cout, int ks, int pad, int act, float slope,
-                                        const void* gate_split, int gate_act, float gate_slope,
-                                        float* colsum_partial, const void* gate_mask, void* mask_out,
-                                        int terms, void* stream) {
-  const char* who = "conv2d_igemm_bf16x3";
+static int x_fold_rows(const XConvPlan& c, const XIgemmParams& p) {
+  if (c.family != XConvPlan::HALO64 || c.h64.nt != 7 || c.h64.wp != 2 || c.h64.f16) return 0;
+  const int r = p.Cout % 16;
+  return (r >= 1 && r <= 8 && (p.Np / 16) % c.h64.nt == 0) ? r : 0;
+}
+extern "C" int wcmc_conv2d_fold_supported(int N, int H, int W, int Cin, int Cout, int ks, int pad, int terms, int orientation) {
+  if (N <= 0 || H <= 0 || W <= 0 || Cin <= 0 || Cout <= 0 || ks <= 0 || pad < 0 || terms < 1 || terms > 3 || ks - 1 - pad < 0) return 0;
+  const int gin = orientation ? Cout : Cin, gout = orientation ? Cin : Cout, gpad = orientation ? ks - 1 - pad : pad;
+  if (H + 2 * gpad - ks + 1 <= 0 || W + 2 * gpad - ks + 1 <= 0) return 0;
+  XIgemmParams p;
+  if (x_igemm_shape(p, "conv2d_fold_supported", N, H, W, gin, gout, ks, gpad, terms, true, 0, 0, 0, false, false)) return 0;
+  static const u16 given = 0;
+  p.ys = const_cast<u16*>(&given);
+  XConvPlan c;
+  if (x_plan_conv(p, &c)) return 0;
+  return x_fold_rows(c, p) ? 1 : 0;
+}
+
+static int x_igemm_entry(const char* who, bool folded, const void* x_split, int N, int H, int W, int Cin, const void* wp,
+                         const float* bias, float* y, int64_t ysn, int64_t ysh, int64_t ysw,
+                         void* y_split, int Cout, int ks, int pad, int act, float slope,
+                         const void* gate_split, int gate_act, float gate_slope,
+                         float* colsum_partial, const void* gate_mask, void* mask_out,
+                         int terms, void* stream) {
   WCMC_REQUIRE(x_split && wp, WCMC_ERR_BAD_ARG, "%s: bad argument", who);
   WCMC_REQUIRE(!colsum_partial || y_split, WCMC_ERR_BAD_ARG,
                "conv2d_igemm_bf16x3: column sums are produced with the split output only");
@@ -880,7 +910,29 @@
 #endif
   XConvPlan c;
   if (const int rc = x_plan_conv(p, &c)) return rc;
+  if (folded) {
+    p.fold = x_fold_rows(c, p);
+    WCMC_REQUIRE(p.fold != 0, WCMC_ERR_BAD_ARG, "%s: no folded launch for this shape (ask wcmc_conv2d_fold_supported)", who);
+  }
   return x_launch_conv(c, p, (hipStream_t)stream);
+}
+extern "C" int wcmc_conv2d_igemm_bf16x3(const void* x_split, int N, int H, int W, int Cin, const void* wp,
+                                        const float* bias, float* y, int64_t ysn, int64_t ysh, int64_t ysw,
+                                        void* y_split, int Cout, int ks, int pad, int act, float slope,
+                                        const void* gate_split, int gate_act, float gate_slope,
+                                        float* colsum_partial, const void* gate_mask, void* mask_out,
+                                        int terms, void* stream) {
+  return x_igemm_entry("conv2d_igemm_bf16x3", false, x_split, N, H, W, Cin, wp, bias, y, ysn, ysh, ysw, y_split, Cout, ks, pad, act, slope,
+                       gate_split, gate_act, gate_slope, colsum_partial, gate_mask, mask_out, terms, stream);
+}
+extern "C" int wcmc_conv2d_igemm_fold_bf16x3(const void* x_split, int N, int H, int W, int Cin, const void* wp,
+                                             const float* bias, float* y, int64_t ysn, int64_t ysh, int64_t ysw,
+                                             void* y_split, int Cout, int ks, int pad, int act, float slope,
+                                             const void* gate_split, int gate_act, float gate_slope,
+                                             float* colsum_partial, const void* gate_mask, void* mask_out,
+                                             int terms, void* stream) {
+  return x_igemm_entry("conv2d_igemm_fold_bf16x3", true, x_split, N, H, W, Cin, wp, bias, y, ysn, ysh, ysw, y_split, Cout, ks, pad, act, slope,
+                       gate_split, gate_act, gate_slope, colsum_partial, gate_mask, mask_out, terms, stream);
 }
 
 extern "C" int wcmc_conv2d_out_f16(const void* x_f16, int N, int H, int W, int Cin, const void* wp_f16, const float* bias, float* y,
diff --git a/wcmc_amd/ops/__init__.py b/wcmc_amd/ops/__init__.py
--- a/wcmc_amd/ops/__init__.py
+++ b/wcmc_amd/ops/__init__.py
@@ -27,6 +27,8 @@
 FUSE_FINAL = os.environ.get("WCMC_FUSE_FINAL", "1") != "0"
 
 SAVE_FINAL_HIDDEN = True
+
+FOLD_LAST_TILE = "off"
 
 TERMS_BY_KS = {}
 
@@ -67,6 +69,14 @@
     return TERMS_BY_KS.get((ks, cin), TERMS_BY_KS.get(ks, (wgrad_terms(), dgrad_terms())))
 
 
+def fold_last_tile(dgrad):
+    v = FOLD_LAST_TILE
+    v = "all" if v is True else "off" if v is False else v
+    if v not in ("all", "dgrad", "off"):
+        raise ValueError("ops.FOLD_LAST_TILE must be \"all\", \"dgrad\" or \"off\", not %r" % (v,))
+    return v == "all" or (v == "dgrad" and dgrad)
+
+
 def out_layer_terms(ks, act):
     if PRECISION == "bf16x321h" and ks == 5 and act == "linear":
         return "h"
@@ -87,7 +97,7 @@
                           _SppMean, spp_mean, _CatBroadcast, cat_broadcast, _PBufferCat, pbuffer_cat, _SampleCat,
                           sample_features_cat)
 from .conv_split import (_split_empty, split_raw, split_from_nchw_raw, presplit_shared, split_gated_raw, split_dy_colsum_raw,
-                         unsplit_debug, _dgrad_mode, _pack_x, _fwd_pack_mode, PACK_MAX_ENTRIES, _pack_chains_x, _pack_chain_x,
+                         unsplit_debug, _dgrad_mode, _pack_x, _fwd_pack_mode, PACK_FOLD, PACK_MAX_ENTRIES, _pack_chains_x, _pack_chain_x,
                          _chain_out_terms, conv2d_x_raw, conv2d_out_f16_raw, conv1x1_pair_x_raw, colsum_finish_raw,
                          conv2d_wgrad_x_raw, _chainx_forward, _chainx_backward, _ConvChainX, _split_shared, _ChainSppMeanX,
                          _CatBroadcastChainX, _CatUpsampleChainX, conv_chain)
diff --git a/wcmc_amd/ops/conv_split.py b/wcmc_amd/ops/conv_split.py
--- a/wcmc_amd/ops/conv_split.py
+++ b/wcmc_amd/ops/conv_split.py
@@ -65,9 +65,12 @@
     return 2 if (_sw.dgrad_terms() if terms is None else terms) == 2 else 1
 
 
+PACK_FOLD = 8
+
+
 def _pack_x(weight, mode):
     cout, cin, ks, _ = weight.shape
-    rows, kch = (cout, cin) if mode in (0, 3, 4) else (cin, cout)
+    rows, kch = (cout, cin) if (mode & ~PACK_FOLD) in (0, 3, 4) else (cin, cout)
     wp = torch.empty(lib().wcmc_conv2d_packed_elems_bf16x3(rows, kch, ks, mode), device=weight.device, dtype=torch.int16)
     w = weight.detach()
     if not w.is_contiguous():
@@ -86,7 +89,7 @@
 PACK_MAX_ENTRIES = 32
 
 
-def _pack_chains_x(chains, ks):
+def _pack_chains_x(chains, ks, folds=None):
     assert sum(2 * len(w) for w, _ in chains) <= PACK_MAX_ENTRIES
     dev = chains[0][0][0].device
     ws, outs, couts, cins, modes, keep, res = [], [], [], [], [], [], []
@@ -101,12 +104,14 @@
             keep.append(w)
             cout, cin = w.shape[0], w.shape[1]
             pair = []
-            for mode in (_fwd_pack_mode(out_terms) if li == n - 1 else 0, dmode):
-                rows, kch = (cout, cin) if mode in (0, 3, 4) else (cin, cout)
+            fold = folds[len(res)][li] if folds is not None else (False, False)
+            lmodes = ((_fwd_pack_mode(out_terms) if li == n - 1 else 0) | (PACK_FOLD if fold[0] else 0), dmode | (PACK_FOLD if fold[1] else 0))
+            for mode in lmodes:
+                rows, kch = (cout, cin) if (mode & ~PACK_FOLD) in (0, 3, 4) else (cin, cout)
                 wp = torch.empty(lib().wcmc_conv2d_packed_elems_bf16x3(rows, kch, ks, mode), device=dev, dtype=torch.int16)
                 ws.append(w.data_ptr()); outs.append(wp.data_ptr()); couts.append(cout); cins.append(cin); modes.append(mode)
                 pair.append(wp)
-            per.append((pair[0], pair[1], (_fwd_pack_mode(out_terms) if li == n - 1 else 0, dmode)))
+            per.append((pair[0], pair[1], lmodes))
         res.append(per)
     m = len(ws)
     arr_p, arr_i = ctypes.c_void_p * m, ctypes.c_int * m
@@ -115,8 +120,8 @@
     return res
 
 
-def _pack_chain_x(weights, ks, out_terms=3):
-    return [(a, b) for a, b, _ in _pack_chains_x([(weights, out_terms)], ks)[0]]
+def _pack_chain_x(weights, ks, out_terms=3, folds=None):
+    return [(a, b) for a, b, _ in _pack_chains_x([(weights, out_terms)], ks, [folds] if folds is not None else None)[0]]
 
 
 def _chain_out_terms(ks, act_last, cin_last, cout_last, pair):
@@ -127,7 +132,7 @@
 
 
 def conv2d_x_raw(xs, dims, wp, bias, cout, ks, pad, act, out_split, gate=None, gate_act="linear", colsum=False,
-                 gate_mask=None, mask_out=False, terms=3, out=None):
+                 gate_mask=None, mask_out=False, terms=3, out=None, fold=False):
     n, cin, h, w = dims
     ho, wo = h + 2 * pad - ks + 1, w + 2 * pad - ks + 1
     dev = xs.device
@@ -144,9 +149,10 @@
     if mask_out:
         mask = torch.empty(n * ho * wo * ((cout + 7) // 8), device=dev, dtype=torch.uint8)
     with _timed_conv(dims, cout, ks, pad, terms, yf, gate is not None):
-        check(lib().wcmc_conv2d_igemm_bf16x3(_ptr(xs), n, h, w, cin, _ptr(wp), _ptr(bias), *yv, _ptr(ysp), cout,
-                                             ks, pad, ACT[act], LEAKY_SLOPE, _ptr(gate), ACT[gate_act], LEAKY_SLOPE,
-                                             _ptr(part), _ptr(gate_mask), _ptr(mask), terms, _stream()), "conv2d_igemm_bf16x3")
+        entry = lib().wcmc_conv2d_igemm_fold_bf16x3 if fold else lib().wcmc_conv2d_igemm_bf16x3
+        check(entry(_ptr(xs), n, h, w, cin, _ptr(wp), _ptr(bias), *yv, _ptr(ysp), cout,
+                    ks, pad, ACT[act], LEAKY_SLOPE, _ptr(gate), ACT[gate_act], LEAKY_SLOPE,
+                    _ptr(part), _ptr(gate_mask), _ptr(mask), terms, _stream()), "conv2d_igemm_fold_bf16x3" if fold else "conv2d_igemm_bf16x3")
     out = ysp if out_split else yf
     ret = (out,) + ((part,) if colsum else ()) + ((mask,) if mask_out else ())
     return ret if len(ret) > 1 else out
@@ -233,9 +239,22 @@
                                               params[2 * nl - 2].shape[0]))
     ctx.terms = _sw.chain_terms(ks, dims0[1])
     oterms = _chain_out_terms(ks, acts[-1], params[2 * nl - 2].shape[1], params[2 * nl - 2].shape[0], pair)
-    packs = _pack_chain_x([params[2 * l] for l in range(nl)], ks, oterms) if 2 * nl <= PACK_MAX_ENTRIES else None
+    fold_f, fold_d = [False] * nl, [False] * nl
+    if ks == 5 and (_sw.fold_last_tile(False) or _sw.fold_last_tile(True)):
+        step = ks - 1 - 2 * pad
+        for l in range(nl):
+            cout_l, cin_l = params[2 * l].shape[:2]
+            hl, wl_ = dims0[2] - l * step, dims0[3] - l * step
+            if _sw.fold_last_tile(False) and (l < nl - 1 or oterms == 3):
+                fold_f[l] = bool(lib().wcmc_conv2d_fold_supported(n, hl, wl_, cin_l, cout_l, ks, pad, 3, 0))
+            if _sw.fold_last_tile(True) and l > 0:
+                fold_d[l] = bool(lib().wcmc_conv2d_fold_supported(n, hl - step, wl_ - step, cin_l, cout_l, ks, pad, ctx.terms[1], 1))
+    ctx.fold_d = fold_d
+    packs = (_pack_chain_x([params[2 * l] for l in range(nl)], ks, oterms, list(zip(fold_f, fold_d)))
+             if 2 * nl <= PACK_MAX_ENTRIES else None)
     ctx.wp1 = [pk[1] for pk in packs] if packs is not None else None
-    pack0 = (lambda l: packs[l][0]) if packs is not None else (lambda l: _pack_x(params[2 * l], _fwd_pack_mode(oterms) if l == nl - 1 else 0))
+    pack0 = (lambda l: packs[l][0]) if packs is not None else (
+        lambda l: _pack_x(params[2 * l], (_fwd_pack_mode(oterms) if l == nl - 1 else 0) | (PACK_FOLD if fold_f[l] else 0)))
     for l in range(nl):
         wt, b = params[2 * l], params[2 * l + 1]
         cout = wt.shape[0]
@@ -257,7 +276,7 @@
             out = conv2d_out_f16_raw(xs[l], dims[l], wp, b.detach(), cout, ks, pad)
         else:
             out = conv2d_x_raw(xs[l], dims[l], wp, b.detach(), cout, ks, pad, acts[l], out_split=hidden, mask_out=hidden,
-                               terms=3 if hidden else oterms)
+                               terms=3 if hidden else oterms, fold=fold_f[l])
         hh, ww = dims[l][2] + 2 * pad - ks + 1, dims[l][3] + 2 * pad - ks + 1
         dims.append((n, cout, hh, ww))
         if hidden:
@@ -304,7 +323,8 @@
     bptrs = getattr(ctx, "bias_ptrs", None) or [0] * nl
     sink_of = lambda l: (ws[l].data_ptr() if isinstance(ws[l], torch.nn.Parameter) else 0, bptrs[l])
     flushed = [_flushed_by_consumer(w) for w in ws]
-    pack1 = (lambda l: wp1[l]) if wp1 is not None else (lambda l: _pack_x(ws[l], _dgrad_mode(dterms)))
+    fold_d = getattr(ctx, "fold_d", None) or [False] * nl
+    pack1 = (lambda l: wp1[l]) if wp1 is not None else (lambda l: _pack_x(ws[l], _dgrad_mode(dterms) | (PACK_FOLD if fold_d[l] else 0)))
     for l in range(nl - 1, -1, -1):
         wt = ws[l]
         cout = wt.shape[0]
@@ -329,7 +349,8 @@
         elif l > 0:
             wpt = pack1(l)
             dys, part = conv2d_x_raw(dys, dims[l + 1], wpt, None, wt.shape[1], ks, ks - 1 - pad, "linear",
-                                     out_split=True, gate_act=acts[l - 1], colsum=True, terms=dterms, gate_mask=masks[l - 1])
+                                     out_split=True, gate_act=acts[l - 1], colsum=True, terms=dterms, gate_mask=masks[l - 1],
+                                     fold=fold_d[l])
         elif need_dx and dx is None:
             sub = getattr(ctx, "dx_channels", None)
             if sub is not None and (sub[1] + 7) // 8 * 8 - sub[0] // 8 * 8 <= wt.shape[1] // 2:
```
